# wuji3/visiondk

Hardware: NVIDIA H100
Metric: embeddings/sec (ConvNeXt-B 224^2 faceX ArcFace train step) (higher is better)
Workload: dtype bf16

## Files before the change

visiondk_b200/csrc/convnext.cu:

```cuda
#include "vdk_host.h"
#include "vdk_ptx.cuh"

#include <cstdlib>
#include "convnext_internal.h"

namespace vdk {

__device__ __forceinline__ float warp_sum(float v) {
#pragma unroll
  for (int off = 16; off > 0; off >>= 1) v += __shfl_xor_sync(0xffffffffu, v, off);
  return v;
}

__global__ void __launch_bounds__(256) stem_patchify_kernel(const float* __restrict__ x, int B, int H, int W,
                                                            __nv_bfloat16* __restrict__ out) {
  const int PH = H / 4, PW = W / 4;
  const int64_t total = static_cast<int64_t>(B) * PH * PW * 12;
  for (int64_t t = static_cast<int64_t>(blockIdx.x) * blockDim.x + threadIdx.x; t < total;
       t += static_cast<int64_t>(gridDim.x) * blockDim.x) {
    const int ck = static_cast<int>(t % 12);
    const int64_t patch = t / 12;
    const int c = ck >> 2, kh = ck & 3;
    const int pw = static_cast<int>(patch % PW);
    const int ph = static_cast<int>((patch / PW) % PH);
// ... 246 lines not shown
  const bool active = has_c && warp < TH && oy0 + warp < H;
  float2 acc[kDwTW][2];
#pragma unroll
  for (int p = 0; p < kDwTW; ++p) {
    acc[p][0] = make_float2(bc.x, bc.y);
    acc[p][1] = make_float2(bc.z, bc.w);
  }
  mbar_wait(bar, 0);
  if (active) {
    const uint8_t* tbase = smem + cl * 2;
#pragma unroll 1
    for (int dy = 0; dy < 7; ++dy) {
      float2 wlo[7], whi[7];
      const float* wrow = wsm + dy * (7 * chunk) + cl;
#pragma unroll
      for (int dx = 0; dx < 7; ++dx) {
        const float4 t = *reinterpret_cast<const float4*>(wrow + dx * chunk);
        wlo[dx] = make_float2(t.x, t.y);
        whi[dx] = make_float2(t.z, t.w);
      }
      const uint8_t* rowp = tbase + (warp + dy) * (box_w * pix_stride);
#pragma unroll
      for (int ix = 0; ix < box_w; ++ix) {
        const uint2 t = *reinterpret_cast<const uint2*>(rowp + ix * pix_stride);
        const float2 a = make_float2(__uint_as_float(t.x << 16), __uint_as_float(t.x & 0xffff0000u));
        const float2 c = make_float2(__uint_as_float(t.y << 16), __uint_as_float(t.y & 0xffff0000u));
#pragma unroll
        for (int p = 0; p < kDwTW; ++p) {
          const int dx = ix - p;
          if (dx >= 0 && dx < 7) {
            acc[p][0] = ffma2(a, wlo[dx], acc[p][0]);
            acc[p][1] = ffma2(c, whi[dx], acc[p][1]);
          }
        }
      }
    }
  }
  if (MODE == 1) {
    if (active) {
#pragma unroll
      for (int p = 0; p < kDwTW; ++p) {
        const int ox = ox0 + p;
        if (ox >= W) continue;
        const int64_t off = ((static_cast<int64_t>(b) * H + oy0 + warp) * W + ox) * C + c0;
        float o0 = acc[p][0].x, o1 = acc[p][0].y, o2 = acc[p][1].x, o3 = acc[p][1].y;
        if (addend) {
          const uint2 t = __ldg(reinterpret_cast<const uint2*>(addend + off));
          const float2 a = __bfloat1622float2(*reinterpret_cast<const __nv_bfloat162*>(&t.x));
          const float2 c = __bfloat1622float2(*reinterpret_cast<const __nv_bfloat162*>(&t.y));
          o0 += a.x; o1 += a.y; o2 += c.x; o3 += c.y;
        }
        __nv_bfloat162 lo = __floats2bfloat162_rn(o0, o1), hi = __floats2bfloat162_rn(o2, o3);
        uint2 t;
        t.x = *reinterpret_cast<uint32_t*>(&lo);
        t.y = *reinterpret_cast<uint32_t*>(&hi);
        *reinterpret_cast<uint2*>(y + off) = t;
      }
    }
    return;
  }
  float mean[kDwTW], rstd[kDwTW];
  const float inv_chunk = 1.0f / static_cast<float>(chunk), inv_c = 1.0f / static_cast<float>(C);
#pragma unroll
  for (int p = 0; p < kDwTW; ++p) {
    const float s = warp_sum(active ? (acc[p][0].x + acc[p][0].y) + (acc[p][1].x + acc[p][1].y) : 0.f);
    mean[p] = s * inv_chunk;
  }
#pragma unroll
  for (int p = 0; p < kDwTW; ++p) {
    float q = 0.f;
    if (active) {
      const float d0 = acc[p][0].x - mean[p], d1 = acc[p][0].y - mean[p];
      const float d2 = acc[p][1].x - mean[p], d3 = acc[p][1].y - mean[p];
      q = fmaf(d0, d0, fmaf(d1, d1, fmaf(d2, d2, d3 * d3)));
    }
    rstd[p] = warp_sum(q);
  }
  if (nchunks == 1) {
#pragma unroll
    for (int p = 0; p < kDwTW; ++p) rstd[p] = rsqrtf(rstd[p] * inv_c + eps);
  } else {
    float2 mine = make_float2(0.f, 0.f);
#pragma unroll
    for (int p = 0; p < kDwTW; ++p)
      if (lane == p) mine = make_float2(mean[p], rstd[p]);
    if (lane < kDwTW && warp < 7) part[warp * 8 + lane] = mine;
    cluster_arrive();
    cluster_wait();
    const float inv_n = 1.0f / static_cast<float>(nchunks);
#pragma unroll
    for (int p = 0; p < kDwTW; ++p) {
      float2 r = make_float2(0.f, 0.f);
      if (lane < nchunks) r = ld_dsmem_f2(part + warp * 8 + p, static_cast<uint32_t>(lane));
      const float m = warp_sum(r.x) * inv_n;
      const float d = r.x - m;
      const float m2 = warp_sum(lane < nchunks ? fmaf(static_cast<float>(chunk) * d, d, r.y) : 0.f);
      mean[p] = m;
      rstd[p] = rsqrtf(m2 * inv_c + eps);
    }
    cluster_arrive();
  }
  if (active) {
#pragma unroll
    for (int p = 0; p < kDwTW; ++p) {
      const int ox = ox0 + p;
      if (ox >= W) continue;
      const int64_t pix = (static_cast<int64_t>(b) * H + oy0 + warp) * W + ox;
      if (rstd_out != nullptr && lane == 0 && ck == 0) rstd_out[pix] = rstd[p];
      __nv_bfloat16* dst = y + pix * C + c0;
      __nv_bfloat162 lo = __floats2bfloat162_rn((acc[p][0].x - mean[p]) * rstd[p] * g4.x + b4.x,
                                                (acc[p][0].y - mean[p]) * rstd[p] * g4.y + b4.y);
      __nv_bfloat162 hi = __floats2bfloat162_rn((acc[p][1].x - mean[p]) * rstd[p] * g4.z + b4.z,
                                                (acc[p][1].y - mean[p]) * rstd[p] * g4.w + b4.w);
      uint2 t;
      t.x = *reinterpret_cast<uint32_t*>(&lo);
      t.y = *reinterpret_cast<uint32_t*>(&hi);
      *reinterpret_cast<uint2*>(dst) = t;
    }
  }
  if (nchunks > 1) cluster_wait();
}

template <int MODE, int CHUNK, int TH>
__global__ void __launch_bounds__((TH + 1) * 32, TH == 7 ? 2 : 1)
dwconv7_pipe_kernel(const __grid_constant__ CUtensorMap map_x, int B, int H, int W, int C, int nchunks, int n_tiles,
                    const float* __restrict__ w49, const float* __restrict__ bias, const float* __restrict__ ln_w,
                    const float* __restrict__ ln_b, float eps, __nv_bfloat16* __restrict__ y, float* __restrict__ rstd_out,
                    const __nv_bfloat16* __restrict__ addend) {
  extern __shared__ uint8_t dwp_smem_raw[];
  uint8_t* smem = dwp_smem_raw + ((128u - (smem_u32(dwp_smem_raw) & 127u)) & 127u);
  constexpr int box_w = kDwTW + 6, box_h = TH + 6;
  constexpr int tile_bytes = box_h * box_w * CHUNK * 2;
  constexpr int tile_stride = (tile_bytes + 127) & ~127;
  float* wsm = reinterpret_cast<float*>(smem + 2 * tile_stride);
  float2* part = reinterpret_cast<float2*>(wsm + 49 * CHUNK);
  uint64_t* full_bar = reinterpret_cast<uint64_t*>(part + 2 * TH * 8);
  uint64_t* empty_bar = full_bar + 2;

  const int warp = threadIdx.x >> 5, lane = threadIdx.x & 31;
  const int ck = blockIdx.x % nchunks;
  const int group = blockIdx.x / nchunks, n_groups = gridDim.x / nchunks;
  const int tiles_w = (W + kDwTW - 1) / kDwTW, tiles_h = (H + TH - 1) / TH;
  const int n_my = group < n_tiles ? (n_tiles - group + n_groups - 1) / n_groups : 0;
  const bool clustered = MODE == 0 && nchunks > 1;

  if (threadIdx.x == 0) {
    prefetch_tensormap(&map_x);
    for (int i = 0; i < 2; ++i) {
      mbar_init(&full_bar[i], 1);
      mbar_init(&empty_bar[i], TH);
    }
    fence_mbar_init();
  }
  for (int i = threadIdx.x; i < 49 * (CHUNK / 4); i += blockDim.x) {
    const int t = i / (CHUNK / 4), q = i - t * (CHUNK / 4);
    *reinterpret_cast<float4*>(wsm + t * CHUNK + q * 4) = __ldg(reinterpret_cast<const float4*>(w49 + t * C + ck * CHUNK + q * 4));
  }
  __syncthreads();

  auto tile_coords = [&](int it, int& b, int& oy0, int& ox0) {
    int t = group + it * n_groups;
    const int tw = t % tiles_w;
    t /= tiles_w;
    const int th = t % tiles_h;
    b = t / tiles_h;
    oy0 = th * TH;
    ox0 = tw * kDwTW;
  };

  if (warp == TH) {
    if (lane == 0 && n_my > 0) {
      int b, oy0, ox0;
      tile_coords(0, b, oy0, ox0);
      mbar_arrive_expect_tx(&full_bar[0], tile_bytes);
      tma_load_4d(smem, &map_x, &full_bar[0], ck * CHUNK, ox0 - 3, oy0 - 3, b);
    }
    for (int it = 0; it < n_my; ++it) {
      if (lane == 0 && it + 1 < n_my) {
        const int j = it + 1, buf = j & 1;
        mbar_wait_relaxed(&empty_bar[buf], ((j >> 1) & 1) ^ 1);
        int b, oy0, ox0;
        tile_coords(j, b, oy0, ox0);
        mbar_arrive_expect_tx(&full_bar[buf], tile_bytes);
        tma_load_4d(smem + buf * tile_stride, &map_x, &full_bar[buf], ck * CHUNK, ox0 - 3, oy0 - 3, b);
      }
      if (clustered) {
        __syncwarp();
        cluster_arrive();
        cluster_wait();
      }
    }
    if (clustered) {
      __syncwarp();
      cluster_arrive();
      cluster_wait();
    }
    return;
  }

  const int cl = lane * 4;
  const bool has_c = cl < CHUNK;
  const int c0 = ck * CHUNK + cl;
  float4 bc = make_float4(0.f, 0.f, 0.f, 0.f), g4 = bc, b4 = bc;
  if (has_c && MODE == 0) {
    bc = __ldg(reinterpret_cast<const float4*>(bias + c0));
    g4 = __ldg(reinterpret_cast<const float4*>(ln_w + c0));
    b4 = __ldg(reinterpret_cast<const float4*>(ln_b + c0));
  }
  constexpr int pix_stride = CHUNK * 2;
  const float inv_chunk = 1.0f / static_cast<float>(CHUNK), inv_c = 1.0f / static_cast<float>(C);

  auto conv_row = [&](const uint8_t* tile, float2 (&acc)[kDwTW][2]) {
#pragma unroll
    for (int p = 0; p < kDwTW; ++p) {
      acc[p][0] = make_float2(bc.x, bc.y);
      acc[p][1] = make_float2(bc.z, bc.w);
    }
    const uint8_t* tbase = tile + cl * 2;
#pragma unroll 1
    for (int dy = 0; dy < 7; ++dy) {
      float2 wlo[7], whi[7];
      const float* wrow = wsm + dy * (7 * CHUNK) + cl;
#pragma unroll
      for (int dx = 0; dx < 7; ++dx) {
        const float4 t = *reinterpret_cast<const float4*>(wrow + dx * CHUNK);
        wlo[dx] = make_float2(t.x, t.y);
        whi[dx] = make_float2(t.z, t.w);
      }
      const uint8_t* rowp = tbase + (warp + dy) * (box_w * pix_stride);
#pragma unroll
      for (int ix = 0; ix < box_w; ++ix) {
        const uint2 t = *reinterpret_cast<const uint2*>(rowp + ix * pix_stride);
        const float2 a = make_float2(__uint_as_float(t.x << 16), __uint_as_float(t.x & 0xffff0000u));
        const float2 c = make_float2(__uint_as_float(t.y << 16), __uint_as_float(t.y & 0xffff0000u));
#pragma unroll
        for (int p = 0; p < kDwTW; ++p) {
          const int dx = ix - p;
          if (dx >= 0 && dx < 7) {
            acc[p][0] = ffma2(a, wlo[dx], acc[p][0]);
            acc[p][1] = ffma2(c, whi[dx], acc[p][1]);
          }
        }
      }
    }
  };

  if (MODE == 1) {
    for (int it = 0; it < n_my; ++it) {
      const int buf = it & 1;
      int b, oy0, ox0;
      tile_coords(it, b, oy0, ox0);
      const bool active = has_c && oy0 + warp < H;
      float2 acc[kDwTW][2];
      mbar_wait(&full_bar[buf], (it >> 1) & 1);
      if (active) conv_row(smem + buf * tile_stride, acc);
      __syncwarp();
      if (lane == 0) mbar_arrive(&empty_bar[buf]);
      if (active) {
#pragma unroll
        for (int p = 0; p < kDwTW; ++p) {
          const int ox = ox0 + p;
          if (ox >= W) continue;
          const int64_t off = ((static_cast<int64_t>(b) * H + oy0 + warp) * W + ox) * C + c0;
          float o0 = acc[p][0].x, o1 = acc[p][0].y, o2 = acc[p][1].x, o3 = acc[p][1].y;
          if (addend) {
            const uint2 t = __ldg(reinterpret_cast<const uint2*>(addend + off));
            const float2 a = __bfloat1622float2(*reinterpret_cast<const __nv_bfloat162*>(&t.x));
            const float2 c = __bfloat1622float2(*reinterpret_cast<const __nv_bfloat162*>(&t.y));
            o0 += a.x; o1 += a.y; o2 += c.x; o3 += c.y;
          }
          __nv_bfloat162 lo = __floats2bfloat162_rn(o0, o1), hi = __floats2bfloat162_rn(o2, o3);
          uint2 t;
          t.x = *reinterpret_cast<uint32_t*>(&lo);
          t.y = *reinterpret_cast<uint32_t*>(&hi);
          *reinterpret_cast<uint2*>(y + off) = t;
        }
      }
    }
    return;
  }

  float2 acc[kDwTW][2];
  float mean[kDwTW], m2[kDwTW];
  int pb = 0, poy0 = 0, pox0 = 0;
  bool pactive = false;

  auto local_stats = [&](bool active, int parity) {
#pragma unroll
    for (int p = 0; p < kDwTW; ++p)
      mean[p] = warp_sum(active ? (acc[p][0].x + acc[p][0].y) + (acc[p][1].x + acc[p][1].y) : 0.f) * inv_chunk;
#pragma unroll
    for (int p = 0; p < kDwTW; ++p) {
      float q = 0.f;
      if (active) {
        const float d0 = acc[p][0].x - mean[p], d1 = acc[p][0].y - mean[p];
        const float d2 = acc[p][1].x - mean[p], d3 = acc[p][1].y - mean[p];
        q = fmaf(d0, d0, fmaf(d1, d1, fmaf(d2, d2, d3 * d3)));
      }
      m2[p] = warp_sum(q);
    }
    if (clustered) {
      float2 mine = make_float2(0.f, 0.f);
#pragma unroll
      for (int p = 0; p < kDwTW; ++p)
        if (lane == p) mine = make_float2(mean[p], m2[p]);
      if (lane < kDwTW) part[(parity * TH + warp) * 8 + lane] = mine;
    }
  };

  auto finish = [&](int parity) {
    float rstd[kDwTW];
    if (clustered) {
      float2 r[kDwTW];
#pragma unroll
      for (int p = 0; p < kDwTW; ++p) {
        r[p] = make_float2(0.f, 0.f);
        if (lane < nchunks) r[p] = ld_dsmem_f2(part + (parity * TH + warp) * 8 + p, static_cast<uint32_t>(lane));
      }
      const float inv_n = 1.0f / static_cast<float>(nchunks);
#pragma unroll
      for (int p = 0; p < kDwTW; ++p) {
        const float m = warp_sum(r[p].x) * inv_n;
        const float d = r[p].x - m;
        const float q = warp_sum(lane < nchunks ? fmaf(static_cast<float>(CHUNK) * d, d, r[p].y) : 0.f);
        mean[p] = m;
        rstd[p] = rsqrtf(q * inv_c + eps);
      }
    } else {
#pragma unroll
      for (int p = 0; p < kDwTW; ++p) rstd[p] = rsqrtf(m2[p] * inv_c + eps);
    }
    if (pactive) {
#pragma unroll
      for (int p = 0; p < kDwTW; ++p) {
        const int ox = pox0 + p;
        if (ox >= W) continue;
        const int64_t pix = (static_cast<int64_t>(pb) * H + poy0 + warp) * W + ox;
        if (rstd_out != nullptr && lane == 0 && ck == 0) rstd_out[pix] = rstd[p];
        __nv_bfloat16* dst = y + pix * C + c0;
        __nv_bfloat162 lo = __floats2bfloat162_rn((acc[p][0].x - mean[p]) * rstd[p] * g4.x + b4.x,
                                                  (acc[p][0].y - mean[p]) * rstd[p] * g4.y + b4.y);
        __nv_bfloat162 hi = __floats2bfloat162_rn((acc[p][1].x - mean[p]) * rstd[p] * g4.z + b4.z,
                                                  (acc[p][1].y - mean[p]) * rstd[p] * g4.w + b4.w);
        uint2 t;
        t.x = *reinterpret_cast<uint32_t*>(&lo);
        t.y = *reinterpret_cast<uint32_t*>(&hi);
        *reinterpret_cast<uint2*>(dst) = t;
      }
    }
  };

  for (int it = 0; it < n_my; ++it) {
    const int buf = it & 1;
    int b, oy0, ox0;
    tile_coords(it, b, oy0, ox0);
    const bool active = has_c && oy0 + warp < H;
    float2 nxt[kDwTW][2];
    mbar_wait(&full_bar[buf], (it >> 1) & 1);
    if (active) conv_row(smem + buf * tile_stride, nxt);
    __syncwarp();
    if (lane == 0) mbar_arrive(&empty_bar[buf]);
    if (it > 0) {
      if (clustered) cluster_wait();
      finish((it - 1) & 1);
    }
#pragma unroll
    for (int p = 0; p < kDwTW; ++p) {
      acc[p][0] = nxt[p][0];
      acc[p][1] = nxt[p][1];
    }
    pb = b; poy0 = oy0; pox0 = ox0; pactive = active;
    local_stats(active, buf);
    if (clustered) cluster_arrive();
  }
  if (n_my > 0) {
    if (clustered) cluster_wait();
    finish((n_my - 1) & 1);
  }
  if (clustered) {
    cluster_arrive();
    cluster_wait();
  }
}

template <int LPP>
__global__ void __launch_bounds__(256)
ln_patchify_kernel(const __nv_bfloat16* __restrict__ x, int B, int H, int W, int C, const float* __restrict__ ln_w,
                   const float* __restrict__ ln_b, float eps, int patch , __nv_bfloat16* __restrict__ out,
                   float* __restrict__ rstd_out) {
  constexpr int kPPW = 32 / LPP;
  constexpr int kMaxIter = 8;
  const int lane = threadIdx.x & 31;
  const int sub = lane % LPP;
  const int64_t warp_id = (static_cast<int64_t>(blockIdx.x) * blockDim.x + threadIdx.x) >> 5;
  const int64_t pix = warp_id * kPPW + lane / LPP;
  const int64_t npix = static_cast<int64_t>(B) * H * W;
  const bool ok = pix < npix;
  const __nv_bfloat16* src = x + (ok ? pix : 0) * C;
  const int iters = (C + LPP * 8 - 1) / (LPP * 8);
  float v[kMaxIter][8];
  float s = 0.f;
#pragma unroll
  for (int i = 0; i < kMaxIter; ++i) {
    if (i < iters) {
      const int c = (sub + i * LPP) * 8;
      uint4 t = make_uint4(0, 0, 0, 0);
      if (ok && c < C) t = *reinterpret_cast<const uint4*>(src + c);
      const float2 a0 = __bfloat1622float2(*reinterpret_cast<const __nv_bfloat162*>(&t.x));
      const float2 a1 = __bfloat1622float2(*reinterpret_cast<const __nv_bfloat162*>(&t.y));
      const float2 a2 = __bfloat1622float2(*reinterpret_cast<const __nv_bfloat162*>(&t.z));
      const float2 a3 = __bfloat1622float2(*reinterpret_cast<const __nv_bfloat162*>(&t.w));
      v[i][0] = a0.x; v[i][1] = a0.y; v[i][2] = a1.x; v[i][3] = a1.y;
      v[i][4] = a2.x; v[i][5] = a2.y; v[i][6] = a3.x; v[i][7] = a3.y;
#pragma unroll
      for (int j = 0; j < 8; ++j) s += v[i][j];
    }
  }
#pragma unroll
  for (int off = LPP / 2; off > 0; off >>= 1) s += __shfl_xor_sync(0xffffffffu, s, off);
  const float mean = s / static_cast<float>(C);
  float q = 0.f;
#pragma unroll
  for (int i = 0; i < kMaxIter; ++i) {
    if (i < iters && (sub + i * LPP) * 8 < C) {
#pragma unroll
      for (int j = 0; j < 8; ++j) {
        const float d = v[i][j] - mean;
        q = fmaf(d, d, q);
      }
    }
  }
#pragma unroll
  for (int off = LPP / 2; off > 0; off >>= 1) q += __shfl_xor_sync(0xffffffffu, q, off);
  const float rstd = rsqrtf(q / static_cast<float>(C) + eps);
  if (!ok) return;
  if (rstd_out != nullptr && sub == 0) rstd_out[pix] = rstd;
  int64_t orow;
  int ocol0;
  if (patch == 2) {
    const int xw = static_cast<int>(pix % W);
    const int yh = static_cast<int>((pix / W) % H);
    const int b = static_cast<int>(pix / (static_cast<int64_t>(W) * H));
    orow = (static_cast<int64_t>(b) * (H / 2) + (yh >> 1)) * (W / 2) + (xw >> 1);
    ocol0 = ((yh & 1) * 2 + (xw & 1)) * C;
  } else {
    orow = pix;
    ocol0 = 0;
  }
  __nv_bfloat16* dst = out + orow * (static_cast<int64_t>(C) * patch * patch) + ocol0;
#pragma unroll
  for (int i = 0; i < kMaxIter; ++i) {
    const int c = (sub + i * LPP) * 8;
    if (i < iters && c < C) {
      const float4 g0 = __ldg(reinterpret_cast<const float4*>(ln_w + c)), g1 = __ldg(reinterpret_cast<const float4*>(ln_w + c + 4));
      const float4 b0 = __ldg(reinterpret_cast<const float4*>(ln_b + c)), b1 = __ldg(reinterpret_cast<const float4*>(ln_b + c + 4));
      __nv_bfloat162 o0 = __floats2bfloat162_rn((v[i][0] - mean) * rstd * g0.x + b0.x, (v[i][1] - mean) * rstd * g0.y + b0.y);
      __nv_bfloat162 o1 = __floats2bfloat162_rn((v[i][2] - mean) * rstd * g0.z + b0.z, (v[i][3] - mean) * rstd * g0.w + b0.w);
      __nv_bfloat162 o2 = __floats2bfloat162_rn((v[i][4] - mean) * rstd * g1.x + b1.x, (v[i][5] - mean) * rstd * g1.y + b1.y);
      __nv_bfloat162 o3 = __floats2bfloat162_rn((v[i][6] - mean) * rstd * g1.z + b1.z, (v[i][7] - mean) * rstd * g1.w + b1.w);
      uint4 t;
      t.x = *reinterpret_cast<uint32_t*>(&o0); t.y = *reinterpret_cast<uint32_t*>(&o1);
      t.z = *reinterpret_cast<uint32_t*>(&o2); t.w = *reinterpret_cast<uint32_t*>(&o3);
      *reinterpret_cast<uint4*>(dst + c) = t;
    }
  }
}

int launch_ln_patchify(const __nv_bfloat16* x, int B, int H, int W, int C, const float* ln_w, const float* ln_b, float eps,
                       int patch, __nv_bfloat16* out, float* rstd_out, cudaStream_t s) {
  VDK_REQUIRE(C % 8 == 0 && C <= 2048, "layernorm_patchify: C must be a multiple of 8, <= 2048 (got %d)", C);
  const int64_t npix = static_cast<int64_t>(B) * H * W;
  const int vecs = C / 8;
  if (vecs <= 8) {
    const int64_t warps = (npix + 3) / 4;
    ln_patchify_kernel<8><<<static_cast<unsigned>((warps * 32 + 255) / 256), 256, 0, s>>>(x, B, H, W, C, ln_w, ln_b, eps, patch, out, rstd_out);
  } else if (vecs <= 16) {
    const int64_t warps = (npix + 1) / 2;
    ln_patchify_kernel<16><<<static_cast<unsigned>((warps * 32 + 255) / 256), 256, 0, s>>>(x, B, H, W, C, ln_w, ln_b, eps, patch, out, rstd_out);
  } else {
    ln_patchify_kernel<32><<<static_cast<unsigned>((npix * 32 + 255) / 256), 256, 0, s>>>(x, B, H, W, C, ln_w, ln_b, eps, patch, out, rstd_out);
  }
  VDK_CUDA_OK(cudaGetLastError());
  return VDK_OK;
}

__global__ void __launch_bounds__(256)
neck_finalize_kernel(const float* __restrict__ acc, int n_slabs, size_t slab_stride, int B, int F,
                     const float* __restrict__ bias, int l2norm, float* __restrict__ out) {
  const int lane = threadIdx.x & 31;
  const int row = (blockIdx.x * blockDim.x + threadIdx.x) >> 5;
  if (row >= B) return;
  double ss = 0.0;
  for (int i = lane; i < F; i += 32) {
    float v = bias[i];
    for (int sl = 0; sl < n_slabs; ++sl) v += acc[sl * slab_stride + static_cast<size_t>(row) * F + i];
    out[static_cast<size_t>(row) * F + i] = v;
    ss = fma(static_cast<double>(v), static_cast<double>(v), ss);
  }
#pragma unroll
  for (int off = 16; off > 0; off >>= 1) ss += __shfl_xor_sync(0xffffffffu, ss, off);
  const float denom = l2norm ? fmaxf(static_cast<float>(sqrt(ss)), 1e-12f) : 1.0f;
  if (l2norm)
    for (int i = lane; i < F; i += 32) out[static_cast<size_t>(row) * F + i] = __fdiv_rn(out[static_cast<size_t>(row) * F + i], denom);
}

int launch_neck_finalize(const float* slabs, int n_slabs, size_t slab_stride, int B, int F, const float* bias, int l2norm,
                         float* out, cudaStream_t s) {
  neck_finalize_kernel<<<(B * 32 + 255) / 256, 256, 0, s>>>(slabs, n_slabs, slab_stride, B, F, bias, l2norm, out);
  VDK_CUDA_OK(cudaGetLastError());
  return VDK_OK;
}

int launch_neck(const __nv_bfloat16* feats, int batch, int Kn, int F, const void* neck_w, const float* neck_b, int l2_normalize,
                float* scratch, size_t scratch_bytes, float* embeddings, cudaStream_t s) {
  const int tiles = ((batch + 127) / 128) * ((F + 255) / 256);
  const size_t slab = static_cast<size_t>(batch) * F;
  int split = std::max(1, (2 * sm_count()) / std::max(1, tiles));
  split = static_cast<int>(std::min<size_t>(split, scratch_bytes / (slab * sizeof(float))));
  split = vdk_gemm_effective_splits(Kn, std::max(1, split));
  {
    vdk_gemm_desc g{};
    g.A = feats; g.B = neck_w; g.D = scratch;
    g.M = batch; g.N = F; g.K = Kn; g.lda = Kn; g.ldb = Kn; g.ldd = F;
    g.in_dtype = VDK_DTYPE_BF16; g.out_dtype = VDK_DTYPE_FP32; g.epilogue = VDK_EPI_NONE;
    g.split_k = split;
    g.split_stride = split > 1 ? static_cast<long long>(slab) : 0;
    const int rc = gemm_run(g, s);
    if (rc != VDK_OK) return rc;
  }
  neck_finalize_kernel<<<(batch * 32 + 255) / 256, 256, 0, s>>>(scratch, split, slab, batch, F, neck_b, l2_normalize, embeddings);
  VDK_CUDA_OK(cudaGetLastError());
  return VDK_OK;
}

static int check_net(const vdk_convnext_net* n) {
  VDK_REQUIRE(n, "vdk_convnext: null network");
  VDK_REQUIRE(n->image_size > 0 && n->image_size % 32 == 0, "vdk_convnext: image_size must be a multiple of 32");
  VDK_REQUIRE(n->feat_dim > 0 && n->feat_dim % 8 == 0, "vdk_convnext: feat_dim must be a multiple of 8");
  int nb = 0;
  for (int s = 0; s < 4; ++s) {
    VDK_REQUIRE(n->dims[s] > 0 && n->dims[s] % 8 == 0 && n->dims[s] <= 2048, "vdk_convnext: dims must be multiples of 8, <= 2048");
    VDK_REQUIRE(n->depths[s] >= 0, "vdk_convnext: bad depth");
    nb += n->depths[s];
  }
  VDK_REQUIRE(nb <= VDK_CONVNEXT_MAX_BLOCKS, "vdk_convnext: too many blocks (%d)", nb);
  VDK_REQUIRE(n->dims[0] <= 256, "vdk_convnext: stem width must be <= 256 (LayerNorm epilogue tile)");
  return VDK_OK;
}

}

using namespace vdk;

template <int TW, int MODE>
static int launch_dwconv_tw(const CUtensorMap& mx, int batch, int H, int W, int C, int TH, int box_c, const float* w49,
                            const float* bias, const float* ln_w, const float* ln_b, float eps, __nv_bfloat16* y,
                            float* rstd_out, const __nv_bfloat16* addend, cudaStream_t s) {
  const int tpg = ((C / 4) + 31) / 32 * 32;
  const int groups = std::max(1, std::min(512 / tpg, TH));
  const int n_chunks = C / box_c;
  const int smem = n_chunks * (((TH + 6) * (TW + 6) * box_c * 2 + 127) & ~127) + 16 * TW * 16 * 4 + 16 + 128;
  auto kern = dwconv7_ln_kernel<TW, MODE>;
  VDK_CUDA_OK(cudaFuncSetAttribute(kern, cudaFuncAttributeMaxDynamicSharedMemorySize, 227 * 1024));
  const unsigned grid = static_cast<unsigned>(batch) * ((H + TH - 1) / TH) * ((W + TW - 1) / TW);
  kern<<<grid, groups * tpg, smem, s>>>(mx, batch, H, W, C, TH, box_c, tpg, w49, bias, ln_w, ln_b, eps, y, rstd_out, addend);
  VDK_CUDA_OK(cudaGetLastError());
  return VDK_OK;
}


template <int MODE, int CHUNK, int TH>
static int launch_dwconv7_pipe_t(const __nv_bfloat16* x, int batch, int H, int W, int C, const float* w49, const float* bias,
                                 const float* ln_w, const float* ln_b, float eps, __nv_bfloat16* y, float* rstd_out,
                                 const __nv_bfloat16* addend, cudaStream_t s) {
  const int nchunks = C / CHUNK;
  constexpr int tile_stride = ((TH + 6) * (kDwTW + 6) * CHUNK * 2 + 127) & ~127;
  constexpr int smem = 2 * tile_stride + 49 * CHUNK * 4 + 2 * TH * 8 * 8 + 4 * 8 + 128;
  static_assert(smem <= 227 * 1024, "dwconv7_pipe shared memory budget");
  CUtensorMap mx;
  int rc = make_tma_nhwc_16bit(&mx, x, batch, H, W, C, TH + 6, kDwTW + 6, CHUNK);
  if (rc != VDK_OK) return rc;
  auto kern = dwconv7_pipe_kernel<MODE, CHUNK, TH>;
  const int cluster = (MODE == 0) ? nchunks : 1;
  struct Fit { int clusters; };
  static Fit fit[17] = {};
  cudaLaunchConfig_t cfg{};
  cfg.blockDim = dim3((TH + 1) * 32);
  cfg.dynamicSmemBytes = smem;
  cfg.stream = s;
  cudaLaunchAttribute attr[1];
  attr[0].id = cudaLaunchAttributeClusterDimension;
  attr[0].val.clusterDim.x = cluster;
  attr[0].val.clusterDim.y = 1;
  attr[0].val.clusterDim.z = 1;
  cfg.attrs = attr;
  cfg.numAttrs = 1;
  if (fit[cluster].clusters == 0) {
    VDK_CUDA_OK(cudaFuncSetAttribute(kern, cudaFuncAttributeMaxDynamicSharedMemorySize, smem));
    if (cluster > 8) VDK_CUDA_OK(cudaFuncSetAttribute(kern, cudaFuncAttributeNonPortableClusterSizeAllowed, 1));
    cfg.gridDim = dim3(cluster * sm_count());
    int n = 0;
    if (cudaOccupancyMaxActiveClusters(&n, kern, &cfg) != cudaSuccess || n <= 0) {
      cudaGetLastError();
      fit[cluster].clusters = -1;
    } else {
      fit[cluster].clusters = n;
    }
  }
  if (fit[cluster].clusters < 0) return VDK_ERR_WORKSPACE;
  const int n_tiles = batch * ((H + TH - 1) / TH) * ((W + kDwTW - 1) / kDwTW);
  const int groups = std::min(n_tiles, fit[cluster].clusters);
  cfg.gridDim = dim3(static_cast<unsigned>(groups) * nchunks);
  if (MODE == 1) {
    const int slots = fit[cluster].clusters;
    const int g = std::max(1, std::min(n_tiles, slots / nchunks));
    cfg.gridDim = dim3(static_cast<unsigned>(g) * nchunks);
  }
  VDK_CUDA_OK(cudaLaunchKernelEx(&cfg, kern, mx, batch, H, W, C, nchunks, n_tiles, w49, bias, ln_w, ln_b, eps, y, rstd_out, addend));
  return VDK_OK;
}

static int launch_dwconv7_pipe(int mode, const __nv_bfloat16* x, int batch, int H, int W, int C, int chunk, const float* w49,
                               const float* bias, const float* ln_w, const float* ln_b, float eps, __nv_bfloat16* y, float* rstd_out,
                               const __nv_bfloat16* addend, cudaStream_t s) {
  const bool tall = H > 7;
#define VDK_DWP(MODEV, CHV)                                                                                                           \
  return tall ? launch_dwconv7_pipe_t<MODEV, CHV, 14>(x, batch, H, W, C, w49, bias, ln_w, ln_b, eps, y, rstd_out, addend, s)          \
              : launch_dwconv7_pipe_t<MODEV, CHV, 7>(x, batch, H, W, C, w49, bias, ln_w, ln_b, eps, y, rstd_out, addend, s)
  if (mode == 0) {
    if (chunk == 128) { VDK_DWP(0, 128); }
    if (chunk == 96) { VDK_DWP(0, 96); }
    VDK_DWP(0, 64);
  }
  if (chunk == 128) { VDK_DWP(1, 128); }
  if (chunk == 96) { VDK_DWP(1, 96); }
  VDK_DWP(1, 64);
#undef VDK_DWP
}

int vdk::launch_dwconv7(int mode, const __nv_bfloat16* x, int batch, int H, int W, int C, const float* w49, const float* bias,
                          const float* ln_w, const float* ln_b, float eps, __nv_bfloat16* y, float* rstd_out,
                          const __nv_bfloat16* addend, cudaStream_t s) {
  VDK_REQUIRE(C % 8 == 0 && C <= 2048, "dwconv7: C must be a multiple of 8, <= 2048 (got %d)", C);
  const double dw_elems = static_cast<double>(batch) * H * W * C;
  ProfScope prof(kProfDepthwise, 2.0 * 49.0 * dw_elems, 2.0 * dw_elems * (addend ? 3.0 : 2.0), s);
  {
    int chunk = 0;
    if (C % 128 == 0) chunk = 128;
    else if (C % 96 == 0) chunk = 96;
    else if (C % 64 == 0) chunk = 64;
    static const bool use_pipe = [] {
      const char* e = getenv("VDK_DWCONV_PIPE");
      return e ? atoi(e) != 0 : true;
    }();
    if (use_pipe && chunk > 0 && C / chunk <= 16) {
      const int rc = launch_dwconv7_pipe(mode, x, batch, H, W, C, chunk, w49, bias, ln_w, ln_b, eps, y, rstd_out, addend, s);
      if (rc != VDK_ERR_WORKSPACE) return rc;
    }
    if (chunk > 0 && C / chunk <= 16) {
      const int nchunks = C / chunk;
      const int TH = std::min(7, H);
      CUtensorMap mx;
      int rc = make_tma_nhwc_16bit(&mx, x, batch, H, W, C, TH + 6, kDwTW + 6, chunk);
      if (rc != VDK_OK) return rc;
      const int smem = (((TH + 6) * (kDwTW + 6) * chunk * 2 + 127) & ~127) + 49 * chunk * 4 + 7 * 8 * 8 + 16 + 128;
      const unsigned grid = static_cast<unsigned>(batch) * ((H + TH - 1) / TH) * ((W + kDwTW - 1) / kDwTW) * nchunks;
      cudaLaunchConfig_t cfg{};
      cfg.gridDim = dim3(grid);
      cfg.blockDim = dim3(32 * TH);
      cfg.dynamicSmemBytes = smem;
      cfg.stream = s;
      cudaLaunchAttribute attr[1];
      attr[0].id = cudaLaunchAttributeClusterDimension;
      attr[0].val.clusterDim.x = (mode == 0) ? nchunks : 1;
      attr[0].val.clusterDim.y = 1;
      attr[0].val.clusterDim.z = 1;
      cfg.attrs = attr;
      cfg.numAttrs = 1;
#define VDK_DWC(MODEV, CHV)                                                                                              \
  do {                                                                                                                   \
    auto kern = dwconv7_chunk_kernel<MODEV, CHV>;                                                                        \
    VDK_CUDA_OK(cudaFuncSetAttribute(kern, cudaFuncAttributeMaxDynamicSharedMemorySize, 80 * 1024));                     \
    if (MODEV == 0 && nchunks > 8) VDK_CUDA_OK(cudaFuncSetAttribute(kern, cudaFuncAttributeNonPortableClusterSizeAllowed, 1)); \
    VDK_CUDA_OK(cudaLaunchKernelEx(&cfg, kern, mx, batch, H, W, C, TH, nchunks, w49, bias, ln_w, ln_b, eps, y, rstd_out, addend)); \
  } while (0)
      if (mode == 0) {
        if (chunk == 128) VDK_DWC(0, 128);
        else if (chunk == 96) VDK_DWC(0, 96);
        else VDK_DWC(0, 64);
      } else {
        if (chunk == 128) VDK_DWC(1, 128);
        else if (chunk == 96) VDK_DWC(1, 96);
        else VDK_DWC(1, 64);
      }
#undef VDK_DWC
      return VDK_OK;
    }
  }
  int box_c = std::min(C, 256);
  while (C % box_c != 0 || box_c % 8 != 0) --box_c;
  int T = 7;
  while (T > 2 && (T + 6) * (T + 6) * C * 2 > 200 * 1024) T = (T == 7) ? 4 : 2;
  VDK_REQUIRE((T + 6) * (T + 6) * C * 2 <= 200 * 1024, "dwconv7: C too large for the shared-memory halo (%d)", C);
  const int TH = std::min(T, H);
  CUtensorMap mx;
  int rc = make_tma_nhwc_16bit(&mx, x, batch, H, W, C, TH + 6, T + 6, box_c);
  if (rc != VDK_OK) return rc;
#define VDK_DW(TWV)                                                                                                    \
  return mode == 0 ? launch_dwconv_tw<TWV, 0>(mx, batch, H, W, C, TH, box_c, w49, bias, ln_w, ln_b, eps, y, rstd_out, addend, s) \
                   : launch_dwconv_tw<TWV, 1>(mx, batch, H, W, C, TH, box_c, w49, bias, ln_w, ln_b, eps, y, rstd_out, addend, s)
  if (T == 7) { VDK_DW(7); }
  if (T == 4) { VDK_DW(4); }
  VDK_DW(2);
#undef VDK_DW
}

static int launch_dwconv7_ln(const __nv_bfloat16* x, int batch, int H, int W, int C, const float* w49, const float* bias,
                             const float* ln_w, const float* ln_b, float eps, __nv_bfloat16* y, cudaStream_t s) {
  return launch_dwconv7(0, x, batch, H, W, C, w49, bias, ln_w, ln_b, eps, y, nullptr, nullptr, s);
}

extern "C" int vdk_dwconv7_ln(const void* x, int batch, int H, int W, int C, const float* w49, const float* bias,
                              const float* ln_w, const float* ln_b, float eps, void* y, void* stream) {
  VDK_REQUIRE(x && y && w49 && bias && ln_w && ln_b, "vdk_dwconv7_ln: null operand");
  VDK_REQUIRE(batch > 0 && H > 0 && W > 0 && C > 0 && C % 8 == 0, "vdk_dwconv7_ln: bad shape (C must be a multiple of 8)");
  return launch_dwconv7_ln(reinterpret_cast<const __nv_bfloat16*>(x), batch, H, W, C, w49, bias, ln_w, ln_b, eps,
                           reinterpret_cast<__nv_bfloat16*>(y), reinterpret_cast<cudaStream_t>(stream));
}

extern "C" int vdk_layernorm_patchify(const void* x, int batch, int H, int W, int C, const float* ln_w,
                                      const float* ln_b, float eps, int patch, void* out, void* stream) {
  VDK_REQUIRE(x && out && ln_w && ln_b, "vdk_layernorm_patchify: null operand");
  VDK_REQUIRE(batch > 0 && H > 0 && W > 0 && C > 0 && C % 8 == 0 && C <= 2048, "vdk_layernorm_patchify: bad shape");
  VDK_REQUIRE(patch == 1 || (patch == 2 && H % 2 == 0 && W % 2 == 0), "vdk_layernorm_patchify: patch must be 1 or 2");
  return launch_ln_patchify(reinterpret_cast<const __nv_bfloat16*>(x), batch, H, W, C, ln_w, ln_b, eps, patch,
                            reinterpret_cast<__nv_bfloat16*>(out), nullptr, reinterpret_cast<cudaStream_t>(stream));
}

extern "C" size_t vdk_convnext_workspace_bytes(const vdk_convnext_net* net, int batch) {
  if (!net || batch <= 0) return 0;
  const size_t hw0 = static_cast<size_t>(net->image_size / 4) * (net->image_size / 4);
  size_t max_mc = 0, max_m4c = 0;
  size_t hw = hw0;
  for (int s = 0; s < 4; ++s) {
    if (s > 0) hw /= 4;
    const size_t m = static_cast<size_t>(batch) * hw;
    max_mc = std::max(max_mc, m * net->dims[s]);
    max_m4c = std::max(max_m4c, m * net->dims[s] * 4);
  }
  const size_t patches = static_cast<size_t>(batch) * hw0 * 48;
  return up256(max_mc * 2) * 2 + up256(std::max(max_m4c, patches) * 2) + up256(static_cast<size_t>(batch) * net->feat_dim * 4) + 1024;
}

extern "C" int vdk_convnext_forward(const vdk_convnext_net* net, const float* images, int batch, int l2_normalize,
                                    float* embeddings, void* workspace, size_t workspace_bytes, void* stream) {
  int rc = check_net(net);
  if (rc != VDK_OK) return rc;
  VDK_REQUIRE(images && embeddings && batch > 0, "vdk_convnext_forward: null image/embedding buffer");
  VDK_REQUIRE(workspace && workspace_bytes >= vdk_convnext_workspace_bytes(net, batch),
              "vdk_convnext_forward: workspace too small");
  VDK_REQUIRE((reinterpret_cast<uintptr_t>(workspace) & 255) == 0 && (reinterpret_cast<uintptr_t>(images) & 15) == 0,
              "vdk_convnext_forward: workspace must be 256-byte and images 16-byte aligned");
  cudaStream_t s = reinterpret_cast<cudaStream_t>(stream);
  const int S = net->image_size;
  const size_t hw0 = static_cast<size_t>(S / 4) * (S / 4);
  size_t max_mc = 0, max_m4c = 0, hwt = hw0;
  for (int st = 0; st < 4; ++st) {
    if (st > 0) hwt /= 4;
    max_mc = std::max(max_mc, static_cast<size_t>(batch) * hwt * net->dims[st]);
    max_m4c = std::max(max_m4c, static_cast<size_t>(batch) * hwt * net->dims[st] * 4);
// ... 60 lines not shown
```

visiondk_b200/csrc/convnext_train.cu:

```cuda
#include "vdk_host.h"
#include "vdk_ptx.cuh"
#include "convnext_internal.h"
#include "train_gemm.h"

#include <vector>

namespace vdk {

static size_t al(size_t v) { return (v + 255) & ~static_cast<size_t>(255); }

static bool ln_bwd_fuses(int C) { return C == 128 || C == 256 || C == 512 || C == 1024; }

struct StageDims {
  int H, W, C;
  size_t M;
};

struct TrainLayout {
  StageDims st[4];
  int depth[4];
  int n_blocks;
  size_t p0, z0, rstd0;
  size_t xs[4][VDK_CONVNEXT_MAX_BLOCKS + 1];
  size_t y[VDK_CONVNEXT_MAX_BLOCKS], rstd[VDK_CONVNEXT_MAX_BLOCKS];
  size_t hpre[VDK_CONVNEXT_MAX_BLOCKS], hpost[VDK_CONVNEXT_MAX_BLOCKS];
  size_t patch[4], prstd[4];
  size_t f, frstd, fn, bn2_mean, bn2_rstd, z, zslab, bn1_mean, bn1_rstd;
  size_t dxa, dxb, dy, dconv, G, sdo, dw49, gwc, gwneck, dz, dzb, dfn, wslab;
  size_t total;
};

static void make_layout(const vdk_convnext_net* net, int batch, TrainLayout* L) {
  size_t off = 0;
  auto take = [&](size_t bytes) { size_t o = off; off += al(bytes); return o; };
  int H = net->image_size / 4, W = H;
  L->n_blocks = 0;
  for (int s = 0; s < 4; ++s) {
    if (s > 0) { H /= 2; W /= 2; }
    L->st[s] = {H, W, net->dims[s], static_cast<size_t>(batch) * H * W};
    L->depth[s] = net->depths[s];
    L->n_blocks += net->depths[s];
  }
  const size_t M0 = L->st[0].M;
  L->p0 = take(M0 * 48 * 2);
  L->z0 = take(M0 * net->dims[0] * 2);
  L->rstd0 = take(M0 * 4);
  int k = 0;
  size_t max_mc = 0, max_cc4 = 0;
  for (int s = 0; s < 4; ++s) {
    const size_t M = L->st[s].M, C = L->st[s].C;
    max_mc = std::max(max_mc, M * C);
    max_cc4 = std::max(max_cc4, C * 4 * C);
    if (s > 0) {
      L->patch[s] = take(M * 4 * L->st[s - 1].C * 2);
      L->prstd[s] = take(L->st[s - 1].M * 4);
      max_cc4 = std::max(max_cc4, C * 4 * static_cast<size_t>(L->st[s - 1].C));
    }
    for (int j = 0; j <= L->depth[s]; ++j) L->xs[s][j] = take(M * C * 2);
    for (int j = 0; j < L->depth[s]; ++j, ++k) {
      L->y[k] = take(M * C * 2);
      L->rstd[k] = take(M * 4);
      L->hpre[k] = take(M * 4 * C * 2);
      L->hpost[k] = take(M * 4 * C * 2);
    }
  }
  const size_t M3 = L->st[3].M, C3 = L->st[3].C, F = net->feat_dim, Kn = (M3 / batch) * C3;
  L->f = take(M3 * C3 * 2);
  L->frstd = take(M3 * 4);
  L->fn = take(M3 * C3 * 2);
  L->bn2_mean = take(C3 * 4);
  L->bn2_rstd = take(C3 * 4);
  L->z = take(static_cast<size_t>(batch) * F * 4);
  L->zslab = take(static_cast<size_t>(batch) * F * 4 * 160);
  L->bn1_mean = take(F * 4);
  L->bn1_rstd = take(F * 4);
  L->dxa = take(max_mc * 2);
  L->dxb = take(max_mc * 2);
  L->dy = take(std::max(max_mc * 2, static_cast<size_t>(2) * 4096 * sm_count() * 4));
  L->dconv = take(max_mc * 2);
  L->G = take(max_cc4 * 4);
  L->sdo = take(static_cast<size_t>(L->n_blocks) * 2048 * 4);
  L->dw49 = take(static_cast<size_t>(L->n_blocks) * 49 * 2048 * 4);
  L->gwc = take(max_cc4 * 4);
  L->gwneck = take(F * Kn * 4);
  L->dz = take(static_cast<size_t>(batch) * F * 4);
  L->dzb = take(static_cast<size_t>(batch) * F * 2);
  L->dfn = take(M3 * C3 * 2);
  size_t slab = wgrad_slab_bytes(net->dims[0], 48, M0);
  for (int s = 0; s < 4; ++s) {
    const int C = L->st[s].C;
    slab = std::max(slab, wgrad_slab_bytes(C, 4 * C, L->st[s].M));
    slab = std::max(slab, wgrad_slab_bytes(4 * C, C, L->st[s].M));
    if (s > 0) slab = std::max(slab, wgrad_slab_bytes(C, 4 * L->st[s - 1].C, L->st[s].M));
  }
  L->wslab = take(slab);
  L->total = off + 256;
}

__global__ void slab_reduce_bias_kernel(const float* __restrict__ slabs, int n_slabs, size_t stride, const float* __restrict__ bias,
                                        int rows, int cols, float* __restrict__ out) {
  const int i = blockIdx.x * blockDim.x + threadIdx.x;
  if (i >= rows * cols) return;
  float v = bias ? bias[i % cols] : 0.f;
  for (int s = 0; s < n_slabs; ++s) v += slabs[s * stride + i];
  out[i] = v;
}
int launch_slab_reduce_bias(const float* slabs, int n_slabs, size_t stride, const float* bias, int rows, int cols, float* out,
                            cudaStream_t s) {
  slab_reduce_bias_kernel<<<(rows * cols + 255) / 256, 256, 0, s>>>(slabs, n_slabs, stride, bias, rows, cols, out);
  VDK_CUDA_OK(cudaGetLastError());
  return VDK_OK;
}
__global__ void __launch_bounds__(256)
slab_reduce_kernel(const float* __restrict__ slabs, int n_slabs, size_t stride, int64_t n4, float* __restrict__ dst,
                   int accumulate) {
  __shared__ float4 part[8][32];
  const int col = threadIdx.x & 31, grp = threadIdx.x >> 5;
  const int64_t i = static_cast<int64_t>(blockIdx.x) * 32 + col;
  float4 acc = make_float4(0.f, 0.f, 0.f, 0.f);
  if (i < n4) {
#pragma unroll 4
    for (int s = grp; s < n_slabs; s += 8) {
      const float4 v = __ldg(reinterpret_cast<const float4*>(slabs + static_cast<size_t>(s) * stride) + i);
      acc.x += v.x; acc.y += v.y; acc.z += v.z; acc.w += v.w;
    }
  }
  part[grp][col] = acc;
  __syncthreads();
  if (grp == 0 && i < n4) {
    float4 t = part[0][col];
#pragma unroll
    for (int g = 1; g < 8; ++g) {
      const float4 v = part[g][col];
      t.x += v.x; t.y += v.y; t.z += v.z; t.w += v.w;
    }
    float4* o = reinterpret_cast<float4*>(dst) + i;
    if (accumulate) {
      const float4 d = *o;
      t.x += d.x; t.y += d.y; t.z += d.z; t.w += d.w;
    }
    *o = t;
  }
}
int launch_slab_reduce(const float* slabs, int n_slabs, size_t stride, int64_t n4, float* dst, int accumulate, cudaStream_t s) {
  slab_reduce_kernel<<<static_cast<unsigned>((n4 + 31) / 32), 256, 0, s>>>(slabs, n_slabs, stride, n4, dst, accumulate);
  VDK_CUDA_OK(cudaGetLastError());
  return VDK_OK;
}
__global__ void col_sum_f32_small_kernel(const float* __restrict__ x, int rows, int cols, float* __restrict__ out) {
  const int c = blockIdx.x * blockDim.x + threadIdx.x;
  if (c >= cols) return;
  float s = 0.f;
  for (int r = 0; r < rows; ++r) s += x[static_cast<size_t>(r) * cols + c];
  out[c] += s;
}
int launch_col_sum_f32_small(const float* x, int rows, int cols, float* out, cudaStream_t s) {
  col_sum_f32_small_kernel<<<(cols + 255) / 256, 256, 0, s>>>(x, rows, cols, out);
  VDK_CUDA_OK(cudaGetLastError());
  return VDK_OK;
}
__global__ void stem_patchify_train_kernel(const float* __restrict__ x, int B, int H, int W, __nv_bfloat16* __restrict__ out) {
  const int PH = H / 4, PW = W / 4;
  const int64_t total = static_cast<int64_t>(B) * PH * PW * 12;
  for (int64_t t = static_cast<int64_t>(blockIdx.x) * blockDim.x + threadIdx.x; t < total;
       t += static_cast<int64_t>(gridDim.x) * blockDim.x) {
    const int ck = static_cast<int>(t % 12);
    const int64_t patch = t / 12;
    const int c = ck >> 2, kh = ck & 3;
    const int pw = static_cast<int>(patch % PW);
    const int ph = static_cast<int>((patch / PW) % PH);
    const int b = static_cast<int>(patch / (static_cast<int64_t>(PW) * PH));
    const float4 v = *reinterpret_cast<const float4*>(x + ((static_cast<int64_t>(b) * 3 + c) * H + (ph * 4 + kh)) * W + pw * 4);
    __nv_bfloat162 lo = __floats2bfloat162_rn(v.x, v.y), hi = __floats2bfloat162_rn(v.z, v.w);
    uint2 o;
    o.x = *reinterpret_cast<uint32_t*>(&lo);
    o.y = *reinterpret_cast<uint32_t*>(&hi);
    *reinterpret_cast<uint2*>(out + patch * 48 + ck * 4) = o;
  }
}

}

using namespace vdk;

extern "C" size_t vdk_convnext_train_workspace_bytes(const vdk_convnext_net* net, int batch) {
  if (!net || batch <= 0) return 0;
  TrainLayout L;
  make_layout(net, batch, &L);
  return L.total;
}

constexpr int kPackTab = 32;
struct PackTab {
  const float* src[kPackTab];
  void* dst[kPackTab];
  void* dst2[kPackTab];
  const float* scale[kPackTab];
};

__global__ void __launch_bounds__(256)
pack_cast_kernel(PackTab t, int64_t n, int cols) {
  const float* __restrict__ src = t.src[blockIdx.y];
  __nv_bfloat16* __restrict__ dst = reinterpret_cast<__nv_bfloat16*>(t.dst[blockIdx.y]);
  __nv_bfloat16* __restrict__ dst2 = reinterpret_cast<__nv_bfloat16*>(t.dst2[blockIdx.y]);
  const float* __restrict__ sc = t.scale[blockIdx.y];
  for (int64_t i = (static_cast<int64_t>(blockIdx.x) * blockDim.x + threadIdx.x) * 4; i < n;
       i += static_cast<int64_t>(gridDim.x) * blockDim.x * 4) {
    const float4 v = __ldg(reinterpret_cast<const float4*>(src + i));
    if (dst2 != nullptr) {
      __nv_bfloat162 lo = __floats2bfloat162_rn(v.x, v.y), hi = __floats2bfloat162_rn(v.z, v.w);
      uint2 o;
      o.x = *reinterpret_cast<uint32_t*>(&lo);
      o.y = *reinterpret_cast<uint32_t*>(&hi);
      *reinterpret_cast<uint2*>(dst2 + i) = o;
    }
    const float m = sc ? sc[i / cols] : 1.f;
    __nv_bfloat162 lo = __floats2bfloat162_rn(v.x * m, v.y * m), hi = __floats2bfloat162_rn(v.z * m, v.w * m);
    uint2 o;
    o.x = *reinterpret_cast<uint32_t*>(&lo);
    o.y = *reinterpret_cast<uint32_t*>(&hi);
    *reinterpret_cast<uint2*>(dst + i) = o;
  }
}
__global__ void __launch_bounds__(256)
pack_taps_kernel(PackTab t, int C) {
  const float* __restrict__ src = t.src[blockIdx.y];
  float* __restrict__ dst = reinterpret_cast<float*>(t.dst[blockIdx.y]);
  float* __restrict__ dst2 = reinterpret_cast<float*>(t.dst2[blockIdx.y]);
  const int i = blockIdx.x * blockDim.x + threadIdx.x;
  if (i >= 49 * C) return;
  const int tap = i / C, c = i - tap * C;
  const float v = src[c * 49 + tap];
  if (dst != nullptr) dst[i] = v;
  if (dst2 != nullptr) dst2[(48 - tap) * C + c] = v;
}

__global__ void __launch_bounds__(256)
unpack_taps_grad_kernel(PackTab t, int C) {
  const float* __restrict__ src = t.src[blockIdx.y];
  float* __restrict__ dst = reinterpret_cast<float*>(t.dst[blockIdx.y]);
  const int i = blockIdx.x * blockDim.x + threadIdx.x;
  if (i >= 49 * C) return;
  const int tap = i / C, c = i - tap * C;
  dst[c * 49 + tap] += src[i];
}

static int pack_impl(const vdk_convnext_tensors* p, const vdk_convnext_net* net, bool taps_and_weights, bool flip, cudaStream_t s) {
  auto bf = [](const void* q) { return const_cast<void*>(q); };
  int k0 = 0;
  for (int st = 0; st < 4; ++st) {
    const int C = net->dims[st], depth = net->depths[st];
    for (int j0 = 0; j0 < depth; j0 += kPackTab) {
      const int nb = std::min(kPackTab, depth - j0);
      PackTab fc1{}, fc2{}, taps{};
      bool any_flip = false;
      for (int j = 0; j < nb; ++j) {
        const vdk_convnext_block_tensors* b = &p->blocks[k0 + j0 + j];
        const vdk_convnext_block* o = &net->blocks[k0 + j0 + j];
        fc1.src[j] = b->fc1_w; fc1.dst[j] = bf(o->fc1_w);
        fc2.src[j] = b->fc2_w;
        if (o->fc2_wg) { fc2.dst[j] = bf(o->fc2_wg); fc2.dst2[j] = bf(o->fc2_w); fc2.scale[j] = b->gamma; }
        else { fc2.dst[j] = bf(o->fc2_w); }
        taps.src[j] = b->dw_w;
        taps.dst[j] = taps_and_weights ? bf(o->dw_w) : nullptr;
        taps.dst2[j] = (flip && o->dw_w_flip) ? bf(o->dw_w_flip) : nullptr;
        any_flip = any_flip || taps.dst2[j] != nullptr;
      }
      const int64_t n = static_cast<int64_t>(4) * C * C;
      const unsigned gx = static_cast<unsigned>(std::max<int64_t>(1, std::min<int64_t>((n / 4 + 255) / 256, 256)));
      if (taps_and_weights) {
        pack_cast_kernel<<<dim3(gx, nb), 256, 0, s>>>(fc1, n, 4 * C);
        pack_cast_kernel<<<dim3(gx, nb), 256, 0, s>>>(fc2, n, 4 * C);
      }
      if (taps_and_weights || any_flip) pack_taps_kernel<<<dim3((49 * C + 255) / 256, nb), 256, 0, s>>>(taps, C);
    }
    k0 += depth;
  }
  VDK_CUDA_OK(cudaGetLastError());
  return VDK_OK;
}

extern "C" int vdk_convnext_pack(const vdk_convnext_tensors* p, vdk_convnext_net* net, void* stream) {
  VDK_REQUIRE(p && net, "vdk_convnext_pack: null argument");
  cudaStream_t s = reinterpret_cast<cudaStream_t>(stream);
  const int C0 = net->dims[0];
  auto bf = [](const void* q) { return reinterpret_cast<__nv_bfloat16*>(const_cast<void*>(q)); };
  for (int st = 0; st < 4; ++st)
    VDK_REQUIRE(net->dims[st] % 4 == 0, "vdk_convnext_pack: channel counts must be multiples of 4");
  RC(launch_cast_bf16(p->stem_w, static_cast<int64_t>(C0) * 48, bf(net->stem_w), s));
  for (int st = 1; st < 4; ++st) {
    RC(launch_permute021(p->down[st].conv_w, net->dims[st], net->dims[st - 1], 4, nullptr, bf(net->down[st].conv_w), nullptr, 0, s));
  }
  RC(pack_impl(p, net, true, true, s));
  const int C3 = net->dims[3], hw = (net->image_size / 32) * (net->image_size / 32);
  RC(launch_permute021(p->lin_w, net->feat_dim, C3, hw, nullptr, bf(net->neck_w), nullptr, 0, s));
  return VDK_OK;
}

extern "C" int vdk_convnext_train_forward(const vdk_convnext_net* net, const vdk_convnext_tensors* p, const float* images,
                                          int batch, float bn_momentum, float* out_feats, void* workspace,
                                          size_t workspace_bytes, void* stream) {
  VDK_REQUIRE(net && p && images && out_feats && batch > 1, "vdk_convnext_train_forward: bad arguments (batch must be > 1)");
  TrainLayout L;
  make_layout(net, batch, &L);
  VDK_REQUIRE(workspace && workspace_bytes >= L.total && (reinterpret_cast<uintptr_t>(workspace) & 255) == 0,
              "vdk_convnext_train_forward: workspace too small or misaligned");
  cudaStream_t s = reinterpret_cast<cudaStream_t>(stream);
  uint8_t* ws = reinterpret_cast<uint8_t*>(workspace);
  auto B16 = [&](size_t off) { return reinterpret_cast<__nv_bfloat16*>(ws + off); };
  auto F32 = [&](size_t off) { return reinterpret_cast<float*>(ws + off); };
  const Gemm G{s};
  const int S = net->image_size;

  {
    const int M0 = static_cast<int>(L.st[0].M), C0 = L.st[0].C;
    const int64_t total = static_cast<int64_t>(M0) * 12;
    stem_patchify_train_kernel<<<static_cast<int>(std::min<int64_t>((total + 255) / 256, 132 * 16)), 256, 0, s>>>(images, batch, S, S,
                                                                                                             B16(L.p0));
    VDK_CUDA_OK(cudaGetLastError());
    RC(G.run(B16(L.p0), net->stem_w, B16(L.z0), M0, C0, 48, 48, 48, C0, VDK_EPI_NONE, net->stem_b, nullptr, nullptr, 0,
             VDK_DTYPE_BF16, 1, 0, 0, 0));
    RC(launch_ln_patchify(B16(L.z0), batch, L.st[0].H, L.st[0].W, C0, net->stem_ln_w, net->stem_ln_b, 1e-6f, 1, B16(L.xs[0][0]),
                          F32(L.rstd0), s));
  }
  int k = 0;
  for (int st = 0; st < 4; ++st) {
    const int H = L.st[st].H, W = L.st[st].W, C = L.st[st].C, M = static_cast<int>(L.st[st].M);
    if (st > 0) {
      const vdk_convnext_down* d = &net->down[st];
      const int Cin = L.st[st - 1].C;
      RC(launch_ln_patchify(B16(L.xs[st - 1][L.depth[st - 1]]), batch, L.st[st - 1].H, L.st[st - 1].W, Cin, d->ln_w, d->ln_b, 1e-6f,
                            2, B16(L.patch[st]), F32(L.prstd[st]), s));
      RC(G.run(B16(L.patch[st]), d->conv_w, B16(L.xs[st][0]), M, C, 4 * Cin, 4 * Cin, 4 * Cin, C, VDK_EPI_NONE, d->conv_b, nullptr,
               nullptr, 0, VDK_DTYPE_BF16, 1, 0, 0, 0));
    }
    for (int j = 0; j < L.depth[st]; ++j, ++k) {
      const vdk_convnext_block* b = &net->blocks[k];
      RC(launch_dwconv7(0, B16(L.xs[st][j]), batch, H, W, C, b->dw_w, b->dw_b, b->ln_w, b->ln_b, 1e-6f, B16(L.y[k]), F32(L.rstd[k]),
                        nullptr, s));
      RC(G.run(B16(L.y[k]), b->fc1_w, B16(L.hpost[k]), M, 4 * C, C, C, C, 4 * C, VDK_EPI_GELU, b->fc1_b, nullptr, nullptr, 0,
               VDK_DTYPE_BF16, 1, 0, 0, 0, B16(L.hpre[k])));
      RC(G.run(B16(L.hpost[k]), b->fc2_w, B16(L.xs[st][j + 1]), M, C, 4 * C, 4 * C, 4 * C, C, VDK_EPI_SCALE_RESIDUAL, b->fc2_b,
               b->gamma, B16(L.xs[st][j]), C, VDK_DTYPE_BF16, 1, 0, 0, 0));
    }
  }
  {
    const int H = L.st[3].H, W = L.st[3].W, C3 = L.st[3].C, M3 = static_cast<int>(L.st[3].M), F = net->feat_dim;
    const int Kn = H * W * C3;
    RC(launch_ln_patchify(B16(L.xs[3][L.depth[3]]), batch, H, W, C3, net->head_ln_w, net->head_ln_b, 1e-6f, 1, B16(L.f),
                          F32(L.frstd), s));
    RC(launch_bn_fwd_bf16(B16(L.f), M3, C3, p->bn2_w, p->bn2_b, 1e-5f, bn_momentum, B16(L.fn), F32(L.bn2_mean), F32(L.bn2_rstd),
                          p->bn2_running_mean, p->bn2_running_var, s));
    const int tiles = ((batch + 127) / 128) * ((F + 255) / 256);
    int split = std::max(1, std::min(160, (2 * sm_count()) / std::max(1, tiles)));
    split = vdk_gemm_effective_splits(Kn, split);
    const size_t slab = static_cast<size_t>(batch) * F;
    RC(G.run(B16(L.fn), net->neck_w, F32(L.zslab), batch, F, Kn, Kn, Kn, F, VDK_EPI_NONE, nullptr, nullptr, nullptr, 0,
             VDK_DTYPE_FP32, split, split > 1 ? static_cast<long long>(slab) : 0, 0, 0));
    RC(launch_slab_reduce_bias(F32(L.zslab), split, slab, p->lin_b, batch, F, F32(L.z), s));
    RC(launch_bn_fwd_f32(F32(L.z), batch, F, p->bn1_w, p->bn1_b, 1e-5f, bn_momentum, out_feats, F32(L.bn1_mean), F32(L.bn1_rstd),
                         p->bn1_running_mean, p->bn1_running_var, s));
  }
  return VDK_OK;
}

extern "C" int vdk_convnext_train_backward_units(const vdk_convnext_net* net) {
  if (!net) return 0;
  int n = 1 + 4;
  for (int st = 0; st < 4; ++st) n += net->depths[st];
  return n;
}

static int backward_range(const vdk_convnext_net* net, const vdk_convnext_tensors* p, const vdk_convnext_tensors* g,
                          const float* d_feats, int batch, void* workspace, size_t workspace_bytes, void* stream, int u_begin,
                          int u_end) {
  VDK_REQUIRE(net && p && g && d_feats && batch > 1, "vdk_convnext_train_backward: bad arguments");
  VDK_REQUIRE(u_begin >= 0 && u_begin < u_end && u_end <= vdk_convnext_train_backward_units(net),
              "vdk_convnext_train_backward: bad unit range [%d, %d)", u_begin, u_end);
  int u = 0;
  auto active = [&](int unit) { return unit >= u_begin && unit < u_end; };
  TrainLayout L;
  make_layout(net, batch, &L);
  VDK_REQUIRE(workspace && workspace_bytes >= L.total, "vdk_convnext_train_backward: workspace too small");
  cudaStream_t s = reinterpret_cast<cudaStream_t>(stream);
  uint8_t* ws = reinterpret_cast<uint8_t*>(workspace);
  auto B16 = [&](size_t off) { return reinterpret_cast<__nv_bfloat16*>(ws + off); };
  auto F32 = [&](size_t off) { return reinterpret_cast<float*>(ws + off); };
  const Gemm G{s};
  const int F = net->feat_dim;

  const int H3 = L.st[3].H, W3 = L.st[3].W, C3 = L.st[3].C, M3 = static_cast<int>(L.st[3].M), Kn = H3 * W3 * C3;
  if (active(u++)) {
    VDK_CUDA_OK(cudaMemsetAsync(F32(L.sdo), 0, static_cast<size_t>(L.n_blocks) * 2048 * 4, s));
    VDK_CUDA_OK(cudaMemsetAsync(F32(L.dw49), 0, static_cast<size_t>(L.n_blocks) * 49 * 2048 * 4, s));
    RC(launch_bn_bwd_f32(d_feats, F32(L.z), batch, F, p->bn1_w, F32(L.bn1_mean), F32(L.bn1_rstd), F32(L.dz), g->bn1_w, g->bn1_b, s));
    RC(launch_col_sum_f32_small(F32(L.dz), batch, F, g->lin_b, s));
    RC(launch_cast_bf16(F32(L.dz), static_cast<int64_t>(batch) * F, B16(L.dzb), s));
    RC(G.run(B16(L.dzb), B16(L.fn), F32(L.gwneck), F, Kn, batch, F, Kn, Kn, VDK_EPI_NONE, nullptr, nullptr, nullptr, 0,
             VDK_DTYPE_FP32, 1, 0, 1, 1));
    RC(launch_permute021(F32(L.gwneck), F, H3 * W3, C3, nullptr, nullptr, g->lin_w, 1, s));
    RC(G.run(B16(L.dzb), net->neck_w, B16(L.dfn), batch, Kn, F, F, Kn, Kn, VDK_EPI_NONE, nullptr, nullptr, nullptr, 0,
             VDK_DTYPE_BF16, 1, 0, 0, 1));
    RC(launch_bn_bwd_bf16(B16(L.dfn), B16(L.f), M3, C3, p->bn2_w, F32(L.bn2_mean), F32(L.bn2_rstd), B16(L.dy), g->bn2_w, g->bn2_b, s));
    RC(launch_ln_bwd(B16(L.dy), B16(L.f), F32(L.frstd), batch, H3, W3, C3, net->head_ln_w, net->head_ln_b, 1, B16(L.dxa), nullptr,
                     g->head_ln_w, g->head_ln_b, s));
  }
  size_t dx = L.dxa, dx_other = L.dxb;
  int k = L.n_blocks;
  for (int st = 3; st >= 0; --st) {
    const int H = L.st[st].H, W = L.st[st].W, C = L.st[st].C, M = static_cast<int>(L.st[st].M);
    int k_done_lo = -1, k_done_hi = -1;
    for (int j = L.depth[st] - 1; j >= 0; --j) {
      --k;
      if (!active(u++)) {
        std::swap(dx, dx_other);
        continue;
      }
      if (k_done_hi < 0) k_done_hi = k;
      k_done_lo = k;
      const vdk_convnext_block* b = &net->blocks[k];
      const vdk_convnext_block_tensors* pb = &p->blocks[k];
      const vdk_convnext_block_tensors* gb = &g->blocks[k];
      float* sdo = F32(L.sdo) + static_cast<size_t>(k) * 2048;
      RC(G.wgrad(B16(dx), B16(L.hpost[k]), F32(L.G), C, 4 * C, M, C, 4 * C, F32(L.wslab), false, sdo));
      RC(launch_layerscale_finalize(F32(L.G), pb->fc2_w, pb->fc2_b, pb->gamma, sdo, C, 4 * C, gb->fc2_w, gb->gamma, gb->fc2_b, s));
      RC(G.run(B16(dx), b->fc2_wg, B16(L.hpost[k]), M, 4 * C, C, C, 4 * C, 4 * C, VDK_EPI_MUL_GELU_GRAD, nullptr, nullptr,
               B16(L.hpre[k]), 4 * C, VDK_DTYPE_BF16, 1, 0, 0, 1));
      __nv_bfloat16* dh = B16(L.hpost[k]);
      RC(G.wgrad(dh, B16(L.y[k]), gb->fc1_w, 4 * C, C, M, 4 * C, C, F32(L.wslab), true, gb->fc1_b));
      if (ln_bwd_fuses(C)) {
        RC(G.ln_bwd(dh, b->fc1_w, B16(L.dconv), M, C, 4 * C, B16(L.y[k]), F32(L.rstd[k]), b->ln_w, b->ln_b, C, 0, gb->ln_w, gb->ln_b,
                    F32(L.dy)));
      } else {
        RC(G.run(dh, b->fc1_w, B16(L.dy), M, C, 4 * C, 4 * C, C, C, VDK_EPI_NONE, nullptr, nullptr, nullptr, 0, VDK_DTYPE_BF16, 1, 0, 0, 1));
        RC(launch_ln_bwd(B16(L.dy), B16(L.y[k]), F32(L.rstd[k]), batch, H, W, C, b->ln_w, b->ln_b, 1, B16(L.dconv), nullptr, gb->ln_w,
                         gb->ln_b, s));
      }
      RC(launch_dwconv7_wgrad(B16(L.xs[st][j]), B16(L.dconv), batch, H, W, C, F32(L.dw49) + static_cast<size_t>(k) * 49 * 2048, gb->dw_b, s));
      RC(launch_dwconv7(1, B16(L.dconv), batch, H, W, C, b->dw_w_flip, nullptr, nullptr, nullptr, 0.f, B16(dx_other), nullptr,
                        B16(dx), s));
      std::swap(dx, dx_other);
    }
    for (int k0 = k_done_lo; k_done_lo >= 0 && k0 <= k_done_hi; k0 += kPackTab) {
      const int nb = std::min(kPackTab, k_done_hi - k0 + 1);
      PackTab tab{};
      for (int j = 0; j < nb; ++j) {
        tab.src[j] = F32(L.dw49) + static_cast<size_t>(k0 + j) * 49 * 2048;
        tab.dst[j] = g->blocks[k0 + j].dw_w;
      }
      unpack_taps_grad_kernel<<<dim3((49 * C + 255) / 256, nb), 256, 0, s>>>(tab, C);
    }
    VDK_CUDA_OK(cudaGetLastError());
    if (st > 0 && !active(u++)) {
      std::swap(dx, dx_other);
    } else if (st > 0) {
      const vdk_convnext_down* d = &net->down[st];
      const vdk_convnext_down_tensors* gd = &g->down[st];
      const int Cin = L.st[st - 1].C;
      RC(G.wgrad(B16(dx), B16(L.patch[st]), F32(L.gwc), C, 4 * Cin, M, C, 4 * Cin, F32(L.wslab), false, gd->conv_b));
      RC(launch_permute021(F32(L.gwc), C, 4, Cin, nullptr, nullptr, gd->conv_w, 1, s));
      if (ln_bwd_fuses(Cin)) {
        RC(G.ln_bwd(B16(dx), d->conv_w, B16(dx_other), M, 4 * Cin, C, B16(L.patch[st]), F32(L.prstd[st]), d->ln_w, d->ln_b, Cin,
                    L.st[st].W, gd->ln_w, gd->ln_b, F32(L.dy)));
      } else {
        RC(G.run(B16(dx), d->conv_w, B16(L.dy), M, 4 * Cin, C, C, 4 * Cin, 4 * Cin, VDK_EPI_NONE, nullptr, nullptr, nullptr, 0,
                 VDK_DTYPE_BF16, 1, 0, 0, 1));
        RC(launch_ln_bwd(B16(L.dy), B16(L.patch[st]), F32(L.prstd[st]), batch, L.st[st - 1].H, L.st[st - 1].W, Cin, d->ln_w, d->ln_b,
                         2, B16(dx_other), nullptr, gd->ln_w, gd->ln_b, s));
      }
      std::swap(dx, dx_other);
    }
  }
  if (active(u++)) {
    const int M0 = static_cast<int>(L.st[0].M), C0 = L.st[0].C;
    RC(launch_ln_bwd(B16(dx), B16(L.xs[0][0]), F32(L.rstd0), batch, L.st[0].H, L.st[0].W, C0, net->stem_ln_w, net->stem_ln_b, 1,
                     B16(L.dy), nullptr, g->stem_ln_w, g->stem_ln_b, s));
    RC(G.wgrad(B16(L.dy), B16(L.p0), g->stem_w, C0, 48, M0, C0, 48, F32(L.wslab), true, g->stem_b));
  }
  return VDK_OK;
}

extern "C" int vdk_convnext_train_backward(const vdk_convnext_net* net, const vdk_convnext_tensors* p,
                                           const vdk_convnext_tensors* g, const float* d_feats, int batch, void* workspace,
                                           size_t workspace_bytes, void* stream) {
  VDK_REQUIRE(net, "vdk_convnext_train_backward: null net");
  return backward_range(net, p, g, d_feats, batch, workspace, workspace_bytes, stream, 0, vdk_convnext_train_backward_units(net));
}

extern "C" int vdk_convnext_train_backward_range(const vdk_convnext_net* net, const vdk_convnext_tensors* p,
                                                 const vdk_convnext_tensors* g, const float* d_feats, int batch, void* workspace,
                                                 size_t workspace_bytes, void* stream, int unit_begin, int unit_end) {
  VDK_REQUIRE(net, "vdk_convnext_train_backward_range: null net");
  return backward_range(net, p, g, d_feats, batch, workspace, workspace_bytes, stream, unit_begin, unit_end);
}
```

visiondk_b200/csrc/gemm.cu:

```cuda
#include "vdk_host.h"
#include "vdk_ptx.cuh"

#include <algorithm>
#include <cstdlib>

#include "train_gemm.h"

namespace vdk {

constexpr int kBM = 128;
constexpr int kBK = 64;
constexpr int kGemmThreads = 384;
constexpr int kBoxBytes = 64 * 128;
constexpr int kGemmPlain = 0;
constexpr int kConvDense = 1;
constexpr int kConvIm2col = 2;
constexpr int kConvGrouped = 3;
constexpr int kConvExDense = 4;
constexpr int kConvExIm2col = 5;
constexpr int kConvGroupedEx = 6;
constexpr int kGemmLnBwd = 7;

struct GemmParams {
  int M, N, K;
// ... 255 lines not shown
        t2[h] = fmaf(g1, h1, t2[h]);
        v[2 * jj] = h == 0 ? d.x * h0 : fmaf(d.x, h0, v[2 * jj]);
        v[2 * jj + 1] = h == 0 ? d.y * h1 : fmaf(d.y, h1, v[2 * jj + 1]);
      }
    }
    const int gi = sc * 64 / G;
#pragma unroll
    for (int gg = 0; gg < kGroups; ++gg)
      if (gg == gi)
#pragma unroll
        for (int h = 0; h < 2; ++h) {
          s1[gg][h] += t1[h];
          s2[gg][h] += t2[h];
        }
    halve_columns(v, lane);
    colp[sc][0] += v[0];
    colp[sc][1] += v[1];
#pragma unroll
    for (int jj = 0; jj < 8; ++jj)
#pragma unroll
      for (int e = 0; e < 2; ++e) v[2 * jj + e] = acc[4 * (sc * 8 + jj) + e] + acc[4 * (sc * 8 + jj) + 2 + e];
    halve_columns(v, lane);
    colp[sc][2] += v[0];
    colp[sc][3] += v[1];
  }
  const float inv_g = 1.0f / static_cast<float>(G);
#pragma unroll
  for (int gi = 0; gi < kGroups; ++gi) {
    if (gi * G >= BN) break;
#pragma unroll
    for (int h = 0; h < 2; ++h) {
      s1[gi][h] += __shfl_xor_sync(0xffffffffu, s1[gi][h], 1);
      s1[gi][h] += __shfl_xor_sync(0xffffffffu, s1[gi][h], 2);
      s2[gi][h] += __shfl_xor_sync(0xffffffffu, s2[gi][h], 1);
      s2[gi][h] += __shfl_xor_sync(0xffffffffu, s2[gi][h], 2);
    }
  }
  if (p.ln_cluster > 1) {
    const uint32_t rank = cluster_ctarank();
    if (leader) mbar_arrive_expect_tx(xbar, p.ln_cluster * 64 * 8);
    if ((lane & 3) == 0)
      for (int r = 0; r < p.ln_cluster; ++r)
#pragma unroll
        for (int h = 0; h < 2; ++h)
          st_async_f2(smem_u32(xch + (rank * 64 + frow + 8 * h) * 8), smem_u32(xbar), r, s1[0][h], s2[0][h]);
    mbar_wait<true>(xbar, xphase);
#pragma unroll
    for (int h = 0; h < 2; ++h) {
      float a = 0.f, b = 0.f;
      for (int r = 0; r < p.ln_cluster; ++r) {
        const float2 t = *reinterpret_cast<const float2*>(xch + (r * 64 + frow + 8 * h) * 8);
        a += t.x;
        b += t.y;
      }
      s1[0][h] = a;
      s2[0][h] = b;
    }
  }
#pragma unroll
  for (int gi = 0; gi < kGroups; ++gi)
#pragma unroll
    for (int h = 0; h < 2; ++h) {
      s1[gi][h] *= inv_g;
      s2[gi][h] *= inv_g;
    }
  __nv_bfloat16* dst = reinterpret_cast<__nv_bfloat16*>(p.D);
#pragma unroll
  for (int sc = 0; sc < BN / 64; ++sc) {
    uint8_t* boxp = ring + sc * kBoxBytes;
    const uint32_t box = smem_u32(boxp);
    const int gi = sc * 64 / G;
    float m1[2], m2[2], r[2];
#pragma unroll
    for (int h = 0; h < 2; ++h) {
      m1[h] = s1[0][h]; m2[h] = s2[0][h]; r[h] = rs[0][h];
#pragma unroll
      for (int gg = 1; gg < kGroups; ++gg)
        if (gg == gi) { m1[h] = s1[gg][h]; m2[h] = s2[gg][h]; r[h] = rs[gg][h]; }
    }
#pragma unroll
    for (int q = 0; q < 4; ++q) {
      const uint32_t addr = box + box_off(mrow, 2 * q + mcb);
      uint32_t rin[4], rq[4];
      ldmatrix_x4(rin, addr);
#pragma unroll
      for (int i = 0; i < 4; ++i) {
        const int j = sc * 8 + 2 * q + (i >> 1), h = i & 1, c = j * 8 + fcol;
        const float2 yv = unpack2(rin[i], VDK_DTYPE_BF16);
        const float2 w = *reinterpret_cast<const float2*>(par + c);
        const float2 iw = *reinterpret_cast<const float2*>(par + BN + c);
        const float2 b = *reinterpret_cast<const float2*>(par + 2 * BN + c);
        const float h0 = (yv.x - b.x) * iw.x, h1 = (yv.y - b.y) * iw.y;
        const float o0 = r[h] * (acc[4 * j + 2 * h] * w.x - m1[h] - h0 * m2[h]);
        const float o1 = r[h] * (acc[4 * j + 2 * h + 1] * w.y - m1[h] - h1 * m2[h]);
        rq[i] = pack2(o0, o1, VDK_DTYPE_BF16);
      }
      stmatrix_x4(addr, rq);
    }
    __syncwarp();
#pragma unroll
    for (int it = 0; it < 4; ++it) {
      const int row = wl * 16 + it * 4 + (lane >> 3), chunk = lane & 7, m = wrow0 + row;
      if (m < p.M) {
        const int n = n0 + sc * 64 + chunk * 8, qg = n / G;
        const long long off = p.ln_wo == 0 ? static_cast<long long>(m) * p.ldd + n : ln_pixel(p, m, qg) * G + (n - qg * G);
        *reinterpret_cast<uint4*>(dst + off) = *reinterpret_cast<const uint4*>(boxp + box_off(row, chunk));
      }
    }
  }
}

template <int BN, bool kBf16, int kTA, int kTB, int kMode>
__global__ void __launch_bounds__(kGemmThreads, 1)
gemm_tn_kernel(const __grid_constant__ CUtensorMap map_a, const __grid_constant__ CUtensorMap map_b,
               const __grid_constant__ CUtensorMap map_d, const __grid_constant__ CUtensorMap map_aux,
               const __grid_constant__ CUtensorMap map_r, const GemmParams p) {
  using Cfg = GemmCfg<BN>;
  constexpr int kStages = Cfg::kStages;
  constexpr int kRing = Cfg::kRing;
  extern __shared__ uint8_t smem_raw[];
  uint8_t* smem = smem_raw + ((1024u - (smem_u32(smem_raw) & 1023u)) & 1023u);
  uint8_t* ring_all = smem + kStages * Cfg::kStageBytes;
  float* par_all = reinterpret_cast<float*>(ring_all + Cfg::kRingBytes);
  uint64_t* full_bar = reinterpret_cast<uint64_t*>(par_all + 2 * Cfg::kParFloats);
  uint64_t* empty_bar = full_bar + kStages;
  uint64_t* res_bar = empty_bar + kStages;
  constexpr bool kColSums = kTA && kMode == kGemmPlain;
  const bool col_sums = kColSums && p.partial_out && p.split_stride > 0 && p.col_sums != nullptr;
  constexpr bool kConvEx = kMode == kConvExDense || kMode == kConvExIm2col;


  if (threadIdx.x == 0) {
    prefetch_tensormap(&map_a);
    prefetch_tensormap(&map_b);
    prefetch_tensormap(&map_d);
    if (p.aux != nullptr) prefetch_tensormap(&map_aux);
    if (kMode == kGemmLnBwd || p.epilogue == VDK_EPI_SCALE_RESIDUAL || p.epilogue == VDK_EPI_MUL_GELU_GRAD ||
        (kMode != kGemmPlain && p.epilogue == VDK_EPI_RESIDUAL_RELU) || (kConvEx && p.epilogue == VDK_EPI_SILU_RESIDUAL))
      prefetch_tensormap(&map_r);
    for (int i = 0; i < kStages; ++i) {
      mbar_init(&full_bar[i], 1);
      mbar_init(&empty_bar[i], col_sums ? 10 : 8);
    }
    mbar_init(&res_bar[0], 1);
    mbar_init(&res_bar[1], 1);
    if constexpr (kMode == kGemmLnBwd)
      for (int i = 0; i < 4; ++i) mbar_init(reinterpret_cast<uint64_t*>(reinterpret_cast<uint8_t*>(res_bar + 2) + kLnXchBytes) + i, 1);
    fence_mbar_init();
  }
  __syncthreads();
  if constexpr (kMode == kGemmLnBwd) {
    if (p.ln_cluster > 1) cluster_sync_all();
  }

  if (threadIdx.x < 128) {
    asm volatile("setmaxnreg.dec.sync.aligned.u32 40;");
    const int num_m = (p.M + kBM - 1) / kBM;
    const int num_n = (p.N + BN - 1) / BN;
    const int num_kb_total = (p.K + kBK - 1) / kBK;
    const int kb_per_split = (num_kb_total + p.split_k - 1) / p.split_k;
    const int num_tiles = num_m * num_n * p.split_k;
    if (threadIdx.x == 0) {
      int stage = 0;
      uint32_t phase = 0;
      for (int tile = blockIdx.x; tile < num_tiles; tile += gridDim.x) {
        const int mn = tile % (num_m * num_n), split = tile / (num_m * num_n);
        const int m0 = (mn / num_n) * kBM;
        const int n0 = (mn % num_n) * BN;
        const int kb0 = split * kb_per_split;
        const int kb1 = min(kb0 + kb_per_split, num_kb_total);
        int cw = 0, ch = 0, cn = 0;
        if constexpr (kMode == kConvIm2col || kMode == kConvGrouped || kMode == kConvGroupedEx) {
          cn = m0 / p.cv_howo;
          const int r = m0 - cn * p.cv_howo, ho = r / p.cv_wo;
          ch = ho * p.cv_stride - p.cv_pad;
          cw = (r - ho * p.cv_wo) * p.cv_stride - p.cv_pad;
        } else if constexpr (kMode == kConvExIm2col) {
          cn = m0 / p.cv_howo;
          const int r = m0 - cn * p.cv_howo, ho = r / p.cv_wo;
          ch = ho * p.cv_stride - (p.cv_pad & 0xff);
          cw = (r - ho * p.cv_wo) * p.cv_stride - (p.cv_pad >> 8);
        }
        for (int kb = kb0; kb < kb1; ++kb) {
          mbar_wait_relaxed<true>(&empty_bar[stage], phase ^ 1);
          uint8_t* sa = smem + stage * Cfg::kStageBytes;
          uint8_t* sb = sa + Cfg::kStageA;
          mbar_arrive_expect_tx(&full_bar[stage], Cfg::kStageBytes);
          if constexpr (kMode == kConvIm2col || kMode == kConvExIm2col) {
            const int tap = kb / p.cv_cpb, c0 = (kb - tap * p.cv_cpb) * kBK, dy = tap / p.cv_kw;
            tma_load_im2col_4d(sa, &map_a, &full_bar[stage], c0, cw, ch, cn, static_cast<uint16_t>(tap - dy * p.cv_kw),
                               static_cast<uint16_t>(dy), kEvictNormal);
          } else if constexpr (kMode == kConvGrouped) {
            const int tap = kb >> 1, c0 = n0 + (kb & 1) * kBK, dy = tap / p.cv_kw;
            tma_load_im2col_4d(sa, &map_a, &full_bar[stage], c0, cw, ch, cn, static_cast<uint16_t>(tap - dy * p.cv_kw),
                               static_cast<uint16_t>(dy), kEvictNormal);
          } else if constexpr (kMode == kConvGroupedEx) {
            const int tap = kb / p.cv_cpb, dy = tap / p.cv_kw;
            const int c0 = ((n0 / p.cv_cg_out * p.cv_cg_in) & ~7) + (kb - tap * p.cv_cpb) * kBK;
            tma_load_im2col_4d(sa, &map_a, &full_bar[stage], c0, cw, ch, cn, static_cast<uint16_t>(tap - dy * p.cv_kw),
                               static_cast<uint16_t>(dy), kEvictNormal);
          } else if (kTA) {
#pragma unroll
            for (int j = 0; j < kBM / 64; ++j) tma_load_2d(sa + j * 8192, &map_a, &full_bar[stage], m0 + j * 64, kb * kBK, kEvictNormal);
          } else {
            tma_load_2d(sa, &map_a, &full_bar[stage], kb * kBK, m0, kEvictNormal);
          }
          if (kTB) {
#pragma unroll
            for (int j = 0; j < BN / 64; ++j) tma_load_2d(sb + j * 8192, &map_b, &full_bar[stage], n0 + j * 64, kb * kBK, kEvictLast);
          } else {
            tma_load_2d(sb, &map_b, &full_bar[stage], kb * kBK, n0, kEvictLast);
          }
          if (++stage == kStages) {
            stage = 0;
            phase ^= 1;
          }
        }
      }
    } else if (col_sums && threadIdx.x >= 32 && threadIdx.x < 96) {
      const int j = (threadIdx.x >> 5) - 1, lane = threadIdx.x & 31;
      const int piece = lane & 15, r0 = lane >> 4;
      uint32_t off[4];
#pragma unroll
      for (int q = 0; q < 4; ++q)
        off[q] = j * 8192 + r0 * 128 + q * 256 + (((((piece >> 1) ^ r0) << 4)) ^ (q << 5)) + (piece & 1) * 8;
      int stage = 0;
      uint32_t phase = 0;
      for (int tile = blockIdx.x; tile < num_tiles; tile += gridDim.x) {
        const int mn = tile % (num_m * num_n), split = tile / (num_m * num_n);
        const int m0 = (mn / num_n) * kBM;
        const bool mine = (mn % num_n) == 0;
        const int kb0 = split * kb_per_split;
        const int kb1 = min(kb0 + kb_per_split, num_kb_total);
        float s[4] = {0.f, 0.f, 0.f, 0.f};
        for (int kb = kb0; kb < kb1; ++kb) {
          mbar_wait<true>(&full_bar[stage], phase);
          if (mine) {
            const uint8_t* sa = smem + stage * Cfg::kStageBytes;
#pragma unroll
            for (int i0 = 0; i0 < 32; i0 += 4) {
              uint2 v[4];
#pragma unroll
              for (int q = 0; q < 4; ++q) v[q] = *reinterpret_cast<const uint2*>(sa + off[q] + i0 * 256);
#pragma unroll
              for (int q = 0; q < 4; ++q) {
                const uint32_t w[2] = {v[q].x, v[q].y};
#pragma unroll
                for (int e = 0; e < 2; ++e) {
                  if constexpr (kBf16) {
                    s[2 * e] += __uint_as_float(w[e] << 16);
                    s[2 * e + 1] += __uint_as_float(w[e] & 0xffff0000u);
                  } else {
                    const float2 f = unpack2(w[e], VDK_DTYPE_FP16);
                    s[2 * e] += f.x;
                    s[2 * e + 1] += f.y;
                  }
                }
              }
            }
          }
          __syncwarp();
          if (lane == 0) mbar_arrive(&empty_bar[stage]);
          if (++stage == kStages) {
            stage = 0;
            phase ^= 1;
          }
        }
        if (mine) {
#pragma unroll
          for (int e = 0; e < 4; ++e) s[e] += __shfl_xor_sync(0xffffffffu, s[e], 16);
          const int m = m0 + j * 64 + piece * 4;
          if (lane < 16 && m < p.M)
            *reinterpret_cast<float4*>(p.col_sums + static_cast<size_t>(split) * p.M + m) = make_float4(s[0], s[1], s[2], s[3]);
        }
      }
    }
  } else {
    asm volatile("setmaxnreg.inc.sync.aligned.u32 232;");
    const int num_m = (p.M + kBM - 1) / kBM;
    const int num_n = (p.N + BN - 1) / BN;
    const int num_kb_total = (p.K + kBK - 1) / kBK;
    const int kb_per_split = (num_kb_total + p.split_k - 1) / p.split_k;
    const int num_tiles = num_m * num_n * p.split_k;
    const int ct = threadIdx.x - 128;
    const int cg = ct >> 7;
    const int wl = (ct >> 5) & 3, lane = ct & 31;
    const int fcol = (lane & 3) * 2;
    const int frow = wl * 16 + (lane >> 2);
    const int mrow = wl * 16 + ((lane >> 3) & 1) * 8 + (lane & 7);
    const int mcb = lane >> 4;
    const bool leader = (ct & 127) == 0;
    const uint32_t bar_id = 2 + cg;
    uint8_t* ring = ring_all + cg * kRing * kBoxBytes;
    float* par = par_all + cg * Cfg::kParFloats;
    const bool f32 = p.out_dtype == VDK_DTYPE_FP32;
    const int box_cols = f32 ? 32 : 64;
    const bool has_res = kMode == kGemmLnBwd || p.epilogue == VDK_EPI_SCALE_RESIDUAL || p.epilogue == VDK_EPI_MUL_GELU_GRAD ||
                         (kMode != kGemmPlain && p.epilogue == VDK_EPI_RESIDUAL_RELU) ||
                         (kConvEx && p.epilogue == VDK_EPI_SILU_RESIDUAL);
    const bool reduce = p.partial_out && p.split_stride == 0;
    int slot = 0;
    uint32_t res_phase = 0;
    int stage = 0;
    uint32_t phase = 0;
    float acc[BN / 2];
    float colp[BN / 64][4] = {};
// ... 103 lines not shown
          sum += __shfl_xor_sync(0xffffffffu, sum, 1);
          sum += __shfl_xor_sync(0xffffffffu, sum, 2);
          const float mean = sum / static_cast<float>(p.N);
          float sq = 0.f;
#pragma unroll
          for (int j = 0; j < BN / 8; ++j) {
            if (j * 8 >= p.N) break;
            const float d0 = acc[4 * j + 2 * r] - mean;
            sq = fmaf(d0, d0, sq);
            const float d1 = acc[4 * j + 2 * r + 1] - mean;
            sq = fmaf(d1, d1, sq);
          }
          sq += __shfl_xor_sync(0xffffffffu, sq, 1);
          sq += __shfl_xor_sync(0xffffffffu, sq, 2);
          ln_mean[r] = mean;
          ln_rstd[r] = rsqrtf(sq / static_cast<float>(p.N) + p.ln_eps);
        }
      }
      if (npre > 0) {
        mbar_wait<true>(&res_bar[cg], res_phase);
        res_phase ^= 1;
      }
      const int dz = (p.partial_out && p.split_stride > 0) ? split : 0;
      int box_i = 0;
#pragma unroll
      for (int sc = 0; sc < BN / 64; ++sc) {
        if (n0 + sc * 64 >= p.N) continue;
        if (f32) {
#pragma unroll
          for (int hb = 0; hb < 2; ++hb) {
            const int bcol = n0 + sc * 64 + hb * 32;
            if (bcol >= p.N) continue;
            uint8_t* box = ring + slot * kBoxBytes;
            if (has_res && box_i >= npre) {
              if (leader) {
                mbar_arrive_expect_tx(&res_bar[cg], kBoxBytes);
                tma_load_3d(box, &map_r, &res_bar[cg], bcol, wrow0, 0);
              }
              mbar_wait<true>(&res_bar[cg], res_phase);
              res_phase ^= 1;
            }
#pragma unroll
            for (int q = 0; q < 4; ++q) {
              const int j = sc * 8 + hb * 4 + q;
#pragma unroll
              for (int h = 0; h < 2; ++h) {
                const int r = frow + 8 * h;
                float2* dst = reinterpret_cast<float2*>(box + box_off(r, 2 * q + (fcol >> 2)) + (fcol & 2) * 4);
                float x0 = acc[4 * j + 2 * h], x1 = acc[4 * j + 2 * h + 1];
                if (!p.partial_out) epi_pair<BN, kMode>(p, x0, x1, par, j * 8 + fcol, ln_mean[h], ln_rstd[h], has_res ? *dst : make_float2(0.f, 0.f));
                *dst = make_float2(x0, x1);
              }
            }
            epi_publish<kRing>(&map_d, box, slot, leader, bar_id, bcol, wrow0, dz, reduce);
            ++box_i;
          }
        } else {
          const int bcol = n0 + sc * 64;
          uint8_t* box = ring + slot * kBoxBytes;
          if (p.aux != nullptr) {
#pragma unroll
            for (int q = 0; q < 4; ++q) {
              uint32_t rq[4];
#pragma unroll
              for (int i = 0; i < 4; ++i) {
                const int j = sc * 8 + 2 * q + (i >> 1), h = i & 1;
                float& x0 = acc[4 * j + 2 * h];
                float& x1 = acc[4 * j + 2 * h + 1];
                if (p.bias != nullptr) {
                  const float2 b = *reinterpret_cast<const float2*>(par + j * 8 + fcol);
                  x0 += b.x;
                  x1 += b.y;
                }
                rq[i] = pack2(x0, x1, p.out_dtype);
                const float2 a = unpack2(rq[i], p.out_dtype);
                x0 = a.x;
                x1 = a.y;
              }
              stmatrix_x4(smem_u32(box) + box_off(mrow, 2 * q + mcb), rq);
            }
            epi_publish<kRing>(&map_aux, box, slot, leader, bar_id, bcol, wrow0, 0, false);
            box = ring + slot * kBoxBytes;
#pragma unroll
            for (int q = 0; q < 4; ++q) {
              uint32_t rq[4];
#pragma unroll
              for (int i = 0; i < 4; ++i) {
                const int j = sc * 8 + 2 * q + (i >> 1), h = i & 1;
                float x0 = acc[4 * j + 2 * h], x1 = acc[4 * j + 2 * h + 1];
                gelu_pair(x0, x1);
                rq[i] = pack2(x0, x1, p.out_dtype);
              }
              stmatrix_x4(smem_u32(box) + box_off(mrow, 2 * q + mcb), rq);
            }
          } else {
#pragma unroll
            for (int q = 0; q < 4; ++q) {
              const uint32_t addr = smem_u32(box) + box_off(mrow, 2 * q + mcb);
              uint32_t rin[4] = {0u, 0u, 0u, 0u}, rq[4];
              if (has_res) ldmatrix_x4(rin, addr);
#pragma unroll
              for (int i = 0; i < 4; ++i) {
                const int j = sc * 8 + 2 * q + (i >> 1), h = i & 1;
                float x0 = acc[4 * j + 2 * h], x1 = acc[4 * j + 2 * h + 1];
                epi_pair<BN, kMode>(p, x0, x1, par, j * 8 + fcol, ln_mean[h], ln_rstd[h], unpack2(rin[i], p.out_dtype));
                rq[i] = pack2(x0, x1, p.out_dtype);
              }
              stmatrix_x4(addr, rq);
            }
          }
          epi_publish<kRing>(&map_d, box, slot, leader, bar_id, bcol, wrow0, 0, false);
          ++box_i;
        }
      }
    }
    if (leader) tma_store_wait<0>();
    if constexpr (kMode == kGemmLnBwd) {
      named_bar_sync(4, 256);
      float* part = reinterpret_cast<float*>(smem);
      const int warp = ct >> 5, jj = ((lane >> 4) & 1) * 4 + ((lane >> 3) & 1) * 2 + ((lane >> 2) & 1);
#pragma unroll
      for (int sc = 0; sc < BN / 64; ++sc)
#pragma unroll
        for (int i = 0; i < 4; ++i) part[(warp * 2 + (i >> 1)) * BN + sc * 64 + jj * 8 + fcol + (i & 1)] = colp[sc][i];
      named_bar_sync(4, 256);
      const int n0 = (blockIdx.x % num_n) * BN;
      float* row = p.ln_slab + static_cast<size_t>(blockIdx.x / num_n) * 2 * p.N;
      for (int t = ct; t < 2 * BN; t += 256) {
        const int q = t / BN, c = t - q * BN;
        float sum = 0.f;
#pragma unroll
        for (int w8 = 0; w8 < 8; ++w8) sum += part[(w8 * 2 + q) * BN + c];
        const int n = n0 + c, grp = n / p.ln_group;
        row[(grp * 2 + q) * p.ln_group + n - grp * p.ln_group] = sum;
      }
    }
  }
  if constexpr (kMode == kGemmLnBwd) {
    if (p.ln_cluster > 1) cluster_sync_all();
  }
}

template <int BN, bool kBf16, int kTA, int kTB, int kMode = kGemmPlain>
static int launch_gemm(const CUtensorMap* maps, const GemmParams& p, cudaStream_t stream) {
  constexpr int kSmem = GemmCfg<BN>::kSmemBytes;
  auto kern = gemm_tn_kernel<BN, kBf16, kTA, kTB, kMode>;
  static bool attr_set = false;
  if (!attr_set) {
    VDK_CUDA_OK(cudaFuncSetAttribute(kern, cudaFuncAttributeMaxDynamicSharedMemorySize, kSmem));
    attr_set = true;
  }
  const int num_tiles = ((p.M + kBM - 1) / kBM) * ((p.N + BN - 1) / BN) * p.split_k;
  const int grid = num_tiles < sm_count() ? num_tiles : sm_count();
  kern<<<grid, kGemmThreads, kSmem, stream>>>(maps[0], maps[1], maps[2], maps[3], maps[4], p);
  VDK_CUDA_OK(cudaGetLastError());
  return VDK_OK;
}

template <int BN, bool kBf16>
static int launch_gemm_major(const CUtensorMap* maps, const GemmParams& p, bool ta, bool tb, cudaStream_t s) {
  if (ta) return tb ? launch_gemm<BN, kBf16, 1, 1>(maps, p, s) : launch_gemm<BN, kBf16, 1, 0>(maps, p, s);
  return tb ? launch_gemm<BN, kBf16, 0, 1>(maps, p, s) : launch_gemm<BN, kBf16, 0, 0>(maps, p, s);
}

}

namespace vdk {

template <int BN>
static int launch_gemm_ln_bwd(const CUtensorMap* maps, const GemmParams& p, int cluster, cudaStream_t s, int* grid_out) {
  constexpr int kSmem = GemmCfg<BN>::kSmemBytes + kLnSmemBytes;
  static_assert(kSmem <= 227 * 1024, "LN-backward GEMM shared memory budget");
  auto kern = gemm_tn_kernel<BN, true, 0, 1, kGemmLnBwd>;
  static int fit[5] = {};
  cudaLaunchConfig_t cfg{};
  cfg.blockDim = dim3(kGemmThreads);
  cfg.dynamicSmemBytes = kSmem;
  cfg.stream = s;
  cudaLaunchAttribute attr[1];
  attr[0].id = cudaLaunchAttributeClusterDimension;
  attr[0].val.clusterDim.x = cluster;
  attr[0].val.clusterDim.y = 1;
  attr[0].val.clusterDim.z = 1;
  cfg.attrs = attr;
  cfg.numAttrs = 1;
  if (fit[cluster] == 0) {
    VDK_CUDA_OK(cudaFuncSetAttribute(kern, cudaFuncAttributeMaxDynamicSharedMemorySize, kSmem));
    int n = sm_count() / cluster;
    if (cluster > 1) {
      cfg.gridDim = dim3(cluster * sm_count());
      VDK_CUDA_OK(cudaOccupancyMaxActiveClusters(&n, kern, &cfg));
    }
    VDK_REQUIRE(n > 0, "vdk_gemm: no cluster of %d LN-backward GEMM CTAs fits on the device", cluster);
    fit[cluster] = n * cluster;
  }
  const int num_n = p.N / BN, num_tiles = ((p.M + kBM - 1) / kBM) * num_n;
  const int grid = std::min(num_tiles, fit[cluster] - fit[cluster] % num_n);
  cfg.gridDim = dim3(grid);
  VDK_CUDA_OK(cudaLaunchKernelEx(&cfg, kern, maps[0], maps[1], maps[2], maps[3], maps[4], p));
  *grid_out = grid;
  return VDK_OK;
}

static int gemm_ln_bwd_run(const vdk_gemm_desc& g, cudaStream_t s) {
  const int G = g.ln_group;
  VDK_REQUIRE(g.in_dtype == VDK_DTYPE_BF16 && g.out_dtype == VDK_DTYPE_BF16 && !g.trans_a && g.trans_b && g.split_k <= 1 &&
                  !g.bias && !g.aux_out && !g.a_col_sums,
              "vdk_gemm: LN_BWD needs bf16 in and out, trans_b only, no split-K, bias or auxiliary output");
  VDK_REQUIRE(g.gamma && g.beta && g.residual && g.ln_rstd && g.ln_dgamma && g.ln_dbeta && g.ln_slab,
              "vdk_gemm: LN_BWD needs gamma, beta, the saved output (residual), ln_rstd, ln_dgamma, ln_dbeta and ln_slab");
  const int BN = (g.N % 256 == 0) ? 256 : 128;
  VDK_REQUIRE(G > 0 && G % 128 == 0 && g.N % G == 0 && (BN % G == 0 || (G % BN == 0 && G / BN <= 4 && G / BN != 3)),
              "vdk_gemm: LN_BWD group %d must be 128, 256, 512 or 1024 and divide N=%d (tile width %d)", G, g.N, BN);
  VDK_REQUIRE(g.lda >= g.K && g.lda % 8 == 0 && g.ldb >= g.N && g.ldb % 8 == 0 && g.ldd >= g.N && g.ldd % 8 == 0 &&
                  (reinterpret_cast<uintptr_t>(g.D) & 15) == 0,
              "vdk_gemm: LN_BWD pitches must cover the rows and keep them 16-byte aligned");
  VDK_REQUIRE(g.ln_wo >= 0 && (g.ln_wo == 0 || (g.N == 4 * G && g.M % g.ln_wo == 0)),
              "vdk_gemm: LN_BWD patch rows need N = 4 ln_group and M a multiple of ln_wo");
  VDK_REQUIRE(g.ldr >= g.N && g.ldr % 8 == 0 && (reinterpret_cast<uintptr_t>(g.residual) & 15) == 0 &&
                  (reinterpret_cast<uintptr_t>(g.ln_slab) & 15) == 0,
              "vdk_gemm: LN_BWD saved-output rows and ln_slab must be 16-byte aligned");
  CUtensorMap maps[5];
  int rc = make_tma_2d_16bit(&maps[0], g.A, (uint64_t)g.M, (uint64_t)g.K, (uint64_t)g.lda, kBM, kBK);
  if (rc != VDK_OK) return rc;
  rc = make_tma_2d_16bit(&maps[1], g.B, (uint64_t)g.K, (uint64_t)g.N, (uint64_t)g.ldb, kBK, 64);
  if (rc != VDK_OK) return rc;
  rc = make_tma_epilogue_map(&maps[4], g.residual, 2, (uint64_t)g.M, (uint64_t)g.N, (uint64_t)g.ldr, 1, 0);
  if (rc != VDK_OK) return rc;
  maps[2] = maps[4];
  maps[3] = maps[4];
  GemmParams p{};
  p.M = g.M; p.N = g.N; p.K = g.K; p.D = g.D; p.ldd = g.ldd;
  p.gamma = g.gamma; p.beta = g.beta; p.residual = g.residual; p.ldr = g.ldr;
  p.out_dtype = VDK_DTYPE_BF16; p.epilogue = VDK_EPI_LN_BWD; p.split_k = 1;
  p.ln_slab = g.ln_slab; p.ln_rstd = g.ln_rstd; p.ln_group = G; p.ln_wo = g.ln_wo;
  p.ln_cluster = G > BN ? G / BN : 1;
  int grid = 0;
  {
    ProfScope prof(kProfGemm, 2.0 * g.M * g.N * g.K,
                   2.0 * (static_cast<double>(g.M) * g.K + static_cast<double>(g.N) * g.K) + 4.0 * g.M * g.N + 4.0 * g.M * (g.N / G), s);
    rc = BN == 256 ? launch_gemm_ln_bwd<256>(maps, p, p.ln_cluster, s, &grid) : launch_gemm_ln_bwd<128>(maps, p, p.ln_cluster, s, &grid);
    if (rc != VDK_OK) return rc;
  }
  const int n_part = grid / (g.N / BN) * (g.N / G);
  rc = launch_slab_reduce(g.ln_slab, n_part, static_cast<size_t>(2) * G, G / 4, g.ln_dgamma, 1, s);
  if (rc != VDK_OK) return rc;
  return launch_slab_reduce(g.ln_slab + G, n_part, static_cast<size_t>(2) * G, G / 4, g.ln_dbeta, 1, s);
}

int gemm_run(const vdk_gemm_desc& g, cudaStream_t s) {
  VDK_REQUIRE(g.A && g.B && g.D, "vdk_gemm: null operand");
  VDK_REQUIRE(g.M > 0 && g.N > 0 && g.K > 0, "vdk_gemm: empty problem M=%d N=%d K=%d", g.M, g.N, g.K);
  VDK_REQUIRE(g.in_dtype == VDK_DTYPE_BF16 || g.in_dtype == VDK_DTYPE_FP16, "vdk_gemm: in_dtype must be bf16/fp16");
  VDK_REQUIRE(g.out_dtype >= VDK_DTYPE_BF16 && g.out_dtype <= VDK_DTYPE_FP32, "vdk_gemm: bad out_dtype");
  VDK_REQUIRE(g.N % 8 == 0, "vdk_gemm: N must be a multiple of 8 (N=%d)", g.N);
  VDK_REQUIRE(g.lda >= (g.trans_a ? g.M : g.K) && g.ldb >= (g.trans_b ? g.N : g.K) && g.ldd >= g.N && g.lda % 8 == 0 &&
                  g.ldb % 8 == 0,
              "vdk_gemm: bad pitches");
  if (g.trans_a) VDK_REQUIRE(g.M % 8 == 0, "vdk_gemm: trans_a needs M to be a multiple of 8");
  const int dalign = g.out_dtype == VDK_DTYPE_FP32 ? 4 : 8;
  VDK_REQUIRE(g.ldd % dalign == 0, "vdk_gemm: ldd must keep rows 16-byte aligned");
  VDK_REQUIRE((reinterpret_cast<uintptr_t>(g.D) & 15) == 0, "vdk_gemm: D must be 16-byte aligned");
  if (g.epilogue == VDK_EPI_LN_BWD) return gemm_ln_bwd_run(g, s);
  VDK_REQUIRE(g.epilogue >= VDK_EPI_NONE && g.epilogue <= VDK_EPI_MUL_GELU_GRAD, "vdk_gemm: bad epilogue");
  if (g.epilogue == VDK_EPI_MUL_GELU_GRAD) {
    VDK_REQUIRE(g.residual && g.out_dtype != VDK_DTYPE_FP32 && g.split_k <= 1 && !g.bias,
                "vdk_gemm: MUL_GELU_GRAD needs the saved pre-activation in `residual`, a 16-bit output and no bias");
    VDK_REQUIRE(g.ldr >= g.N && g.ldr % 8 == 0 && (reinterpret_cast<uintptr_t>(g.residual) & 15) == 0,
                "vdk_gemm: pre-activation rows must be 16-byte aligned");
  }
  if (g.epilogue == VDK_EPI_SCALE_RESIDUAL) {
    VDK_REQUIRE(g.gamma && g.residual, "vdk_gemm: SCALE_RESIDUAL needs gamma and residual");
    VDK_REQUIRE(g.ldr >= g.N && g.ldr % dalign == 0 && (reinterpret_cast<uintptr_t>(g.residual) & 15) == 0,
                "vdk_gemm: residual must be 16-byte aligned rows");
  }
  if (g.epilogue == VDK_EPI_LAYERNORM) {
    VDK_REQUIRE(g.gamma && g.beta, "vdk_gemm: LAYERNORM needs gamma (weight) and beta (bias)");
    VDK_REQUIRE(g.N <= 256, "vdk_gemm: LAYERNORM epilogue needs the whole row in one tile (N <= 256, got %d)", g.N);
    VDK_REQUIRE((reinterpret_cast<uintptr_t>(g.beta) & 15) == 0, "vdk_gemm: beta must be 16-byte aligned");
  }
  if (g.bias) VDK_REQUIRE((reinterpret_cast<uintptr_t>(g.bias) & 15) == 0, "vdk_gemm: bias must be 16-byte aligned");
  if (g.gamma) VDK_REQUIRE((reinterpret_cast<uintptr_t>(g.gamma) & 15) == 0, "vdk_gemm: gamma must be 16-byte aligned");
  int split = g.split_k < 1 ? 1 : g.split_k;
  {
    const int kbt = (g.K + kBK - 1) / kBK;
    if (split > kbt) split = kbt;
    const int per = (kbt + split - 1) / split;
    split = (kbt + per - 1) / per;
  }
  if (g.split_stride != 0)
    VDK_REQUIRE(g.split_stride >= (long long)g.M * g.ldd && g.split_stride % 4 == 0, "vdk_gemm: split_stride must cover one [M,ldd] slab");
  if (g.split_k > 1)
    VDK_REQUIRE(g.out_dtype == VDK_DTYPE_FP32 && g.epilogue == VDK_EPI_NONE && !g.bias,
                "vdk_gemm: split_k > 1 needs fp32 output, no bias and no epilogue (partials are atomically added)");
  if (g.a_col_sums)
    VDK_REQUIRE(g.trans_a && g.split_k > 1 && g.split_stride != 0 && (reinterpret_cast<uintptr_t>(g.a_col_sums) & 15) == 0,
                "vdk_gemm: a_col_sums needs trans_a, split_k > 1 with split_stride > 0, and 16-byte alignment");

  bool wide = (g.N % 256 == 0) || g.N > 512;
  if (g.epilogue == VDK_EPI_LAYERNORM) wide = g.N > 128;
  const int BN = wide ? 256 : 128;
  CUtensorMap maps[5];
  CUtensorMap &ma = maps[0], &mb = maps[1], &md = maps[2], &maux = maps[3], &mr = maps[4];
  int rc = g.trans_a ? make_tma_2d_16bit(&ma, g.A, (uint64_t)g.K, (uint64_t)g.M, (uint64_t)g.lda, kBK, 64)
                     : make_tma_2d_16bit(&ma, g.A, (uint64_t)g.M, (uint64_t)g.K, (uint64_t)g.lda, kBM, kBK);
  if (rc != VDK_OK) return rc;
  rc = g.trans_b ? make_tma_2d_16bit(&mb, g.B, (uint64_t)g.K, (uint64_t)g.N, (uint64_t)g.ldb, kBK, 64)
                 : make_tma_2d_16bit(&mb, g.B, (uint64_t)g.N, (uint64_t)g.K, (uint64_t)g.ldb, BN, kBK);
  if (rc != VDK_OK) return rc;
  if (g.aux_out != nullptr) {
    VDK_REQUIRE(g.out_dtype != VDK_DTYPE_FP32 && g.split_k <= 1 && g.epilogue == VDK_EPI_GELU,
                "vdk_gemm: aux_out needs the GELU epilogue and a 16-bit output");
    VDK_REQUIRE((reinterpret_cast<uintptr_t>(g.aux_out) & 15) == 0, "vdk_gemm: aux_out must be 16-byte aligned");
  }
  const int osize = g.out_dtype == VDK_DTYPE_FP32 ? 4 : 2;
  const bool slabs = g.split_k > 1 && g.split_stride != 0;
  rc = make_tma_epilogue_map(&md, g.D, osize, (uint64_t)g.M, (uint64_t)g.N, (uint64_t)g.ldd, slabs ? (uint64_t)split : 1,
                             slabs ? (uint64_t)g.split_stride : 0);
  if (rc != VDK_OK) return rc;
  maux = md;
  mr = md;
  if (g.aux_out != nullptr) {
    rc = make_tma_epilogue_map(&maux, g.aux_out, 2, (uint64_t)g.M, (uint64_t)g.N, (uint64_t)g.ldd, 1, 0);
    if (rc != VDK_OK) return rc;
  }
  if (g.epilogue == VDK_EPI_SCALE_RESIDUAL || g.epilogue == VDK_EPI_MUL_GELU_GRAD) {
    rc = make_tma_epilogue_map(&mr, g.residual, osize, (uint64_t)g.M, (uint64_t)g.N, (uint64_t)g.ldr, 1, 0);
    if (rc != VDK_OK) return rc;
  }
  GemmParams p{g.M, g.N, g.K, g.D, g.ldd, g.bias, g.gamma, g.beta, g.residual, g.ldr, g.out_dtype, g.epilogue,
               g.ln_eps, split, g.split_k > 1 ? (long long)g.split_stride : 0ll, g.aux_out, (g.split_k > 1) ? 1 : 0};
  if (g.a_col_sums) p.col_sums = g.a_col_sums;
  const bool bf = g.in_dtype == VDK_DTYPE_BF16;
  const double osz = g.out_dtype == VDK_DTYPE_FP32 ? 4.0 : 2.0;
  ProfScope prof(kProfGemm, 2.0 * g.M * g.N * g.K,
                 2.0 * (static_cast<double>(g.M) * g.K + static_cast<double>(g.N) * g.K) + osz * g.M * g.N * (g.split_k > 1 ? split : 1) +
                     (g.aux_out ? 2.0 * g.M * g.N : 0.0) + (g.residual ? osz * g.M * g.N : 0.0),
                 s);
  const bool ta = g.trans_a != 0, tb = g.trans_b != 0;
  if (wide) return bf ? launch_gemm_major<256, true>(maps, p, ta, tb, s) : launch_gemm_major<256, false>(maps, p, ta, tb, s);
  return bf ? launch_gemm_major<128, true>(maps, p, ta, tb, s) : launch_gemm_major<128, false>(maps, p, ta, tb, s);
}

struct ConvArgs {
  const void* x;
  const void* w;
  const float* bias;
  const void* residual;
  void* y;
  int B, H, W, Cin, Cout, kernel, stride, epilogue;
  int pad_h[2], pad_w[2];
  bool ex;
};

static int conv_launch(const ConvArgs& c, cudaStream_t s) {
  const int Ho = (c.H + c.pad_h[0] + c.pad_h[1] - c.kernel) / c.stride + 1;
  const int Wo = (c.W + c.pad_w[0] + c.pad_w[1] - c.kernel) / c.stride + 1;
  const bool dense = c.kernel == 1 && c.stride == 1 && (c.pad_h[0] | c.pad_h[1] | c.pad_w[0] | c.pad_w[1]) == 0;
  const int Cinp = dense ? c.Cin : (c.Cin + kBK - 1) / kBK * kBK;
  const long long M = static_cast<long long>(c.B) * Ho * Wo;
  const long long K = static_cast<long long>(c.kernel) * c.kernel * Cinp;
  VDK_REQUIRE(M < (1ll << 31) && K < (1ll << 31), "vdk_conv2d: problem too large (M=%lld K=%lld)", M, K);
  const bool wide = (c.Cout % 256 == 0) || c.Cout > 512;
  CUtensorMap maps[5];
  int rc = dense ? make_tma_2d_16bit(&maps[0], c.x, (uint64_t)M, (uint64_t)c.Cin, (uint64_t)c.Cin, kBM, kBK)
         : c.ex  ? make_tma_im2col_16bit_pads(&maps[0], c.x, c.B, c.H, c.W, c.Cin, c.kernel, c.stride, c.pad_h, c.pad_w)
                 : make_tma_im2col_16bit(&maps[0], c.x, c.B, c.H, c.W, c.Cin, c.kernel, c.stride, c.pad_h[0]);
  if (rc != VDK_OK) return rc;
  rc = make_tma_2d_16bit(&maps[1], c.w, (uint64_t)c.Cout, (uint64_t)K, (uint64_t)K, wide ? 256 : 128, kBK);
  if (rc != VDK_OK) return rc;
  rc = make_tma_epilogue_map(&maps[2], c.y, 2, (uint64_t)M, (uint64_t)c.Cout, (uint64_t)c.Cout, 1, 0);
  if (rc != VDK_OK) return rc;
  maps[3] = maps[2];
  maps[4] = maps[2];
  if (c.residual != nullptr) {
    rc = make_tma_epilogue_map(&maps[4], c.residual, 2, (uint64_t)M, (uint64_t)c.Cout, (uint64_t)c.Cout, 1, 0);
    if (rc != VDK_OK) return rc;
  }
  GemmParams p{};
  p.M = static_cast<int>(M); p.N = c.Cout; p.K = static_cast<int>(K);
  p.D = c.y; p.ldd = c.Cout; p.bias = c.bias; p.residual = c.residual; p.ldr = c.Cout;
  p.out_dtype = VDK_DTYPE_BF16; p.epilogue = c.epilogue; p.split_k = 1;
  p.cv_cpb = Cinp / kBK; p.cv_kw = c.kernel; p.cv_stride = c.stride;
  p.cv_pad = c.ex ? (c.pad_h[0] | c.pad_w[0] << 8) : c.pad_h[0];
  p.cv_wo = Wo; p.cv_howo = Ho * Wo;
  ProfScope prof(kProfGemm, 2.0 * M * c.Cout * K,
                 2.0 * (static_cast<double>(c.B) * c.H * c.W * c.Cin + static_cast<double>(c.Cout) * K + M * c.Cout) +
                     (c.residual ? 2.0 * M * c.Cout : 0.0),
                 s);
  if (c.ex) {
    if (dense) return wide ? launch_gemm<256, true, 0, 0, kConvExDense>(maps, p, s) : launch_gemm<128, true, 0, 0, kConvExDense>(maps, p, s);
    return wide ? launch_gemm<256, true, 0, 0, kConvExIm2col>(maps, p, s) : launch_gemm<128, true, 0, 0, kConvExIm2col>(maps, p, s);
  }
  if (dense) return wide ? launch_gemm<256, true, 0, 0, kConvDense>(maps, p, s) : launch_gemm<128, true, 0, 0, kConvDense>(maps, p, s);
  return wide ? launch_gemm<256, true, 0, 0, kConvIm2col>(maps, p, s) : launch_gemm<128, true, 0, 0, kConvIm2col>(maps, p, s);
}

int conv_run(const vdk_conv_desc& c, cudaStream_t s) {
  VDK_REQUIRE(c.x && c.w && c.y, "vdk_conv2d: null operand");
  VDK_REQUIRE(c.B > 0 && c.H > 0 && c.W > 0, "vdk_conv2d: empty input B=%d H=%d W=%d", c.B, c.H, c.W);
// ... 201 lines not shown
```

visiondk_b200/csrc/train_gemm.h:

```cpp
#pragma once
#include <algorithm>

#include "vdk_host.h"

namespace vdk {

int launch_slab_reduce(const float* slabs, int n_slabs, size_t stride, int64_t n4, float* dst, int accumulate, cudaStream_t s);
int launch_slab_reduce_bias(const float* slabs, int n_slabs, size_t stride, const float* bias, int rows, int cols, float* out,
                            cudaStream_t s);
int launch_col_sum_f32_small(const float* x, int rows, int cols, float* out, cudaStream_t s);

inline int wgrad_splits(int M, int N, size_t K) {
  const int tiles = ((M + 127) / 128) * ((N + 255) / 256);
  const int want = std::max(2, (2 * sm_count()) / std::max(1, tiles));
  return vdk_gemm_effective_splits(static_cast<int>(K), want);
}
inline size_t wgrad_slab_bytes(int M, int N, size_t K) {
  return static_cast<size_t>(std::max(2, wgrad_splits(M, N, K))) * M * (static_cast<size_t>(N) + 1) * 4;
}

struct Gemm {
  cudaStream_t s;
  int run(const void* A, const void* B, void* D, int M, int N, int K, int lda, int ldb, int ldd, int epi, const float* bias,
          const float* gamma, const void* res, int ldr, int out_dtype, int split, long long stride, int ta, int tb,
          void* aux_out = nullptr, float* a_col_sums = nullptr) const {
    vdk_gemm_desc g{};
    g.A = A; g.B = B; g.D = D;
    g.M = M; g.N = N; g.K = K; g.lda = lda; g.ldb = ldb; g.ldd = ldd;
    g.in_dtype = VDK_DTYPE_BF16; g.out_dtype = out_dtype; g.epilogue = epi;
    g.bias = bias; g.gamma = gamma; g.residual = res; g.ldr = ldr;
    g.ln_eps = 1e-6f; g.split_k = split; g.split_stride = stride; g.trans_a = ta; g.trans_b = tb; g.aux_out = aux_out;
    g.a_col_sums = a_col_sums;
    return gemm_run(g, s);
  }
  int ln_bwd(const void* A, const void* B, void* D, int M, int N, int K, const void* y, const float* rstd, const float* ln_w,
             const float* ln_b, int group, int wo, float* dgamma, float* dbeta, float* slab) const {
    vdk_gemm_desc g{};
    g.A = A; g.B = B; g.D = D;
    g.M = M; g.N = N; g.K = K; g.lda = K; g.ldb = N; g.ldd = N;
    g.in_dtype = VDK_DTYPE_BF16; g.out_dtype = VDK_DTYPE_BF16; g.epilogue = VDK_EPI_LN_BWD;
    g.gamma = ln_w; g.beta = ln_b; g.residual = y; g.ldr = N;
    g.split_k = 1; g.trans_b = 1;
    g.ln_rstd = rstd; g.ln_dgamma = dgamma; g.ln_dbeta = dbeta; g.ln_slab = slab; g.ln_group = group; g.ln_wo = wo;
    return gemm_run(g, s);
  }
  int wgrad(const void* A, const void* B, float* D, int M, int N, int K, int lda, int ldb, float* slabs, bool accumulate,
            float* bias_grad = nullptr) const {
    VDK_REQUIRE((static_cast<size_t>(M) * N) % 4 == 0, "wgrad: M*N must be a multiple of 4");
    const int split = wgrad_splits(M, N, static_cast<size_t>(K));
    const size_t stride = static_cast<size_t>(M) * N;
    float* col_slabs = bias_grad ? slabs + static_cast<size_t>(split) * stride : nullptr;
    int rc = run(A, B, slabs, M, N, K, lda, ldb, N, VDK_EPI_NONE, nullptr, nullptr, nullptr, 0, VDK_DTYPE_FP32, std::max(2, split),
                 static_cast<long long>(stride), 1, 1, nullptr, col_slabs);
    if (rc != VDK_OK) return rc;
    rc = launch_slab_reduce(slabs, split, stride, static_cast<int64_t>(stride / 4), D, accumulate ? 1 : 0, s);
    if (rc != VDK_OK || !bias_grad) return rc;
    return launch_slab_reduce(col_slabs, split, static_cast<size_t>(M), M / 4, bias_grad, 1, s);
  }
};

#define RC(expr)                   \
  do {                             \
    int _rc = (expr);              \
    if (_rc != VDK_OK) return _rc; \
  } while (0)

}
```

visiondk_b200/csrc/train_ops.cu:

```cuda
#include "vdk_host.h"
#include "vdk_ptx.cuh"
#include "convnext_internal.h"

namespace vdk {

__device__ __forceinline__ float wsum(float v) {
#pragma unroll
  for (int off = 16; off > 0; off >>= 1) v += __shfl_xor_sync(0xffffffffu, v, off);
  return v;
}

__device__ __forceinline__ void unpack8(const uint4& t, float (&v)[8]) {
  const float2 a0 = __bfloat1622float2(*reinterpret_cast<const __nv_bfloat162*>(&t.x));
  const float2 a1 = __bfloat1622float2(*reinterpret_cast<const __nv_bfloat162*>(&t.y));
  const float2 a2 = __bfloat1622float2(*reinterpret_cast<const __nv_bfloat162*>(&t.z));
  const float2 a3 = __bfloat1622float2(*reinterpret_cast<const __nv_bfloat162*>(&t.w));
  v[0] = a0.x; v[1] = a0.y; v[2] = a1.x; v[3] = a1.y; v[4] = a2.x; v[5] = a2.y; v[6] = a3.x; v[7] = a3.y;
}
__device__ __forceinline__ uint4 pack8(const float (&v)[8]) {
  __nv_bfloat162 o0 = __floats2bfloat162_rn(v[0], v[1]), o1 = __floats2bfloat162_rn(v[2], v[3]);
  __nv_bfloat162 o2 = __floats2bfloat162_rn(v[4], v[5]), o3 = __floats2bfloat162_rn(v[6], v[7]);
  uint4 t;
  t.x = *reinterpret_cast<uint32_t*>(&o0); t.y = *reinterpret_cast<uint32_t*>(&o1);
  t.z = *reinterpret_cast<uint32_t*>(&o2); t.w = *reinterpret_cast<uint32_t*>(&o3);
  return t;
}


template <int LPP, int IT, int U>
__global__ void __launch_bounds__(256, IT >= 4 ? 1 : 2)
ln_bwd_kernel(const __nv_bfloat16* __restrict__ dy, const __nv_bfloat16* __restrict__ y, const float* __restrict__ rstd,
              int B, int H, int W, int C, const float* __restrict__ ln_w, const float* __restrict__ ln_b, int patch,
              __nv_bfloat16* __restrict__ dx, const __nv_bfloat16* __restrict__ addend, float* __restrict__ dgamma,
              float* __restrict__ dbeta) {
  constexpr int kPPW = 32 / LPP;
  extern __shared__ float ln_sm[];
  const int Cp = LPP * IT * 8;
  float* s_w = ln_sm;
  float* s_iw = s_w + Cp;
  float* s_b = s_iw + Cp;
  float* s_dg = s_b + Cp;
  float* s_db = s_dg + Cp;
  for (int c = threadIdx.x; c < Cp; c += 256) {
    float w = c < C ? ln_w[c] : 1.f;
    float iw = 0.f;
    if (w != 0.f) {
      if (fabsf(w) < 1e-12f) w = w < 0.f ? -1e-12f : 1e-12f;
      iw = 1.0f / w;
    }
    s_w[c] = w;
    s_iw[c] = iw;
    s_b[c] = c < C ? ln_b[c] : 0.f;
    s_dg[c] = 0.f;
    s_db[c] = 0.f;
  }
  __syncthreads();
  const int lane = threadIdx.x & 31, sub = lane % LPP;
  const int64_t npix = static_cast<int64_t>(B) * H * W;
  const int64_t nwarps = (static_cast<int64_t>(gridDim.x) * blockDim.x) >> 5;
  const int64_t warp_id = (static_cast<int64_t>(blockIdx.x) * blockDim.x + threadIdx.x) >> 5;
  const float inv_c = 1.0f / static_cast<float>(C);
  float gw[IT][8], gb[IT][8];
#pragma unroll
  for (int i = 0; i < IT; ++i)
#pragma unroll
    for (int j = 0; j < 8; ++j) { gw[i][j] = 0.f; gb[i][j] = 0.f; }

  for (int64_t base = warp_id * (kPPW * U); base < npix; base += nwarps * (kPPW * U)) {
    uint4 rdy[U][IT], ry[U][IT];
    int64_t pix[U], roff[U];
#pragma unroll
    for (int u = 0; u < U; ++u) {
      pix[u] = base + u * kPPW + lane / LPP;
      const bool ok = pix[u] < npix;
      int64_t orow = pix[u];
      int ocol0 = 0;
      if (patch == 2 && ok) {
        const int xw = static_cast<int>(pix[u] % W);
        const int yh = static_cast<int>((pix[u] / W) % H);
        const int b = static_cast<int>(pix[u] / (static_cast<int64_t>(W) * H));
        orow = (static_cast<int64_t>(b) * (H / 2) + (yh >> 1)) * (W / 2) + (xw >> 1);
        ocol0 = ((yh & 1) * 2 + (xw & 1)) * C;
      }
      roff[u] = orow * (static_cast<int64_t>(C) * patch * patch) + ocol0;
#pragma unroll
      for (int i = 0; i < IT; ++i) {
        const int c = (sub + i * LPP) * 8;
        rdy[u][i] = make_uint4(0, 0, 0, 0);
        ry[u][i] = make_uint4(0, 0, 0, 0);
        if (ok && c < C) {
          rdy[u][i] = __ldg(reinterpret_cast<const uint4*>(dy + roff[u] + c));
          ry[u][i] = __ldg(reinterpret_cast<const uint4*>(y + roff[u] + c));
        }
      }
    }
    float s1[U], s2[U];
#pragma unroll
    for (int u = 0; u < U; ++u) { s1[u] = 0.f; s2[u] = 0.f; }
#pragma unroll
    for (int i = 0; i < IT; ++i) {
      const int c = (sub + i * LPP) * 8;
      float w[8], iw[8], bb[8];
      *reinterpret_cast<float4*>(&w[0]) = *reinterpret_cast<const float4*>(s_w + c);
            *reinterpret_cast<float4*>(&w[4]) = *reinterpret_cast<const float4*>(s_w + c + 4);
      *reinterpret_cast<float4*>(&iw[0]) = *reinterpret_cast<const float4*>(s_iw + c);
            *reinterpret_cast<float4*>(&iw[4]) = *reinterpret_cast<const float4*>(s_iw + c + 4);
      *reinterpret_cast<float4*>(&bb[0]) = *reinterpret_cast<const float4*>(s_b + c);
            *reinterpret_cast<float4*>(&bb[4]) = *reinterpret_cast<const float4*>(s_b + c + 4);
#pragma unroll
      for (int u = 0; u < U; ++u) {
        const bool okc = pix[u] < npix && c < C;
        float vdy[8], vy[8];
        unpack8(rdy[u][i], vdy);
        unpack8(ry[u][i], vy);
#pragma unroll
        for (int j = 0; j < 8; ++j) {
          const float h = okc ? (vy[j] - bb[j]) * iw[j] : 0.f;
          const float g = vdy[j] * w[j];
          s1[u] += g;
          s2[u] = fmaf(g, h, s2[u]);
          gw[i][j] = fmaf(vdy[j], h, gw[i][j]);
          gb[i][j] += vdy[j];
        }
      }
    }
#pragma unroll
    for (int u = 0; u < U; ++u) {
#pragma unroll
      for (int off = LPP / 2; off > 0; off >>= 1) {
        s1[u] += __shfl_xor_sync(0xffffffffu, s1[u], off);
        s2[u] += __shfl_xor_sync(0xffffffffu, s2[u], off);
      }
    }
#pragma unroll
    for (int u = 0; u < U; ++u) {
      if (pix[u] < npix) {
        const float rs = rstd[pix[u]];
        const float m1 = s1[u] * inv_c, m2 = s2[u] * inv_c;
#pragma unroll
        for (int i = 0; i < IT; ++i) {
          const int c = (sub + i * LPP) * 8;
          if (c < C) {
            float w[8], iw[8], bb[8];
            *reinterpret_cast<float4*>(&w[0]) = *reinterpret_cast<const float4*>(s_w + c);
            *reinterpret_cast<float4*>(&w[4]) = *reinterpret_cast<const float4*>(s_w + c + 4);
            *reinterpret_cast<float4*>(&iw[0]) = *reinterpret_cast<const float4*>(s_iw + c);
            *reinterpret_cast<float4*>(&iw[4]) = *reinterpret_cast<const float4*>(s_iw + c + 4);
            *reinterpret_cast<float4*>(&bb[0]) = *reinterpret_cast<const float4*>(s_b + c);
            *reinterpret_cast<float4*>(&bb[4]) = *reinterpret_cast<const float4*>(s_b + c + 4);
            float vdy[8], vy[8], o[8];
            if constexpr (IT > 4) {
              asm volatile("" : "+r"(rdy[u][i].x), "+r"(rdy[u][i].y), "+r"(rdy[u][i].z), "+r"(rdy[u][i].w));
              asm volatile("" : "+r"(ry[u][i].x), "+r"(ry[u][i].y), "+r"(ry[u][i].z), "+r"(ry[u][i].w));
            }
            unpack8(rdy[u][i], vdy);
            unpack8(ry[u][i], vy);
#pragma unroll
            for (int j = 0; j < 8; ++j) {
              const float h = (vy[j] - bb[j]) * iw[j];
              o[j] = rs * (vdy[j] * w[j] - m1 - h * m2);
            }
            if (addend) {
              float a[8];
              unpack8(__ldg(reinterpret_cast<const uint4*>(addend + pix[u] * C + c)), a);
#pragma unroll
              for (int j = 0; j < 8; ++j) o[j] += a[j];
            }
            *reinterpret_cast<uint4*>(dx + pix[u] * C + c) = pack8(o);
          }
        }
      }
    }
  }
#pragma unroll
  for (int i = 0; i < IT; ++i) {
    const int c = (sub + i * LPP) * 8;
#pragma unroll
    for (int j = 0; j < 8; ++j) {
      float a = gw[i][j], b2 = gb[i][j];
#pragma unroll
      for (int off = LPP; off < 32; off <<= 1) {
        a += __shfl_xor_sync(0xffffffffu, a, off);
        b2 += __shfl_xor_sync(0xffffffffu, b2, off);
      }
      if (lane < LPP) {
        atomicAdd(s_dg + c + j, a);
        atomicAdd(s_db + c + j, b2);
      }
    }
  }
  __syncthreads();
  for (int c = threadIdx.x; c < C; c += 256) {
    atomicAdd(dgamma + c, s_dg[c]);
    atomicAdd(dbeta + c, s_db[c]);
  }
}

template <int LPP, int IT, int U>
static void ln_bwd_launch(const __nv_bfloat16* dy, const __nv_bfloat16* y, const float* rstd, int B, int H, int W, int C,
                          const float* ln_w, const float* ln_b, int patch, __nv_bfloat16* dx, const __nv_bfloat16* addend,
                          float* dgamma, float* dbeta, cudaStream_t s) {
  const int64_t npix = static_cast<int64_t>(B) * H * W;
  const int64_t pix_per_block_trip = 8 * (32 / LPP) * U;
  const int blocks = static_cast<int>(std::max<int64_t>(1, std::min<int64_t>((npix + pix_per_block_trip - 1) / pix_per_block_trip,
                                                                              sm_count() * (IT >= 4 ? 1 : 2))));
  const size_t smem = static_cast<size_t>(LPP) * IT * 8 * 5 * sizeof(float);
  ln_bwd_kernel<LPP, IT, U><<<blocks, 256, smem, s>>>(dy, y, rstd, B, H, W, C, ln_w, ln_b, patch, dx, addend, dgamma, dbeta);
}

int launch_ln_bwd(const __nv_bfloat16* dy, const __nv_bfloat16* y, const float* rstd, int B, int H, int W, int C,
                  const float* ln_w, const float* ln_b, int patch, __nv_bfloat16* dx, const __nv_bfloat16* addend,
                  float* dgamma, float* dbeta, cudaStream_t s) {
  VDK_REQUIRE(C % 8 == 0 && C <= 1536, "ln_bwd: C must be a multiple of 8, <= 1536 (got %d)", C);
  const int vecs = C / 8;
  if (vecs <= 8) ln_bwd_launch<8, 1, 4>(dy, y, rstd, B, H, W, C, ln_w, ln_b, patch, dx, addend, dgamma, dbeta, s);
  else if (vecs <= 16) ln_bwd_launch<16, 1, 4>(dy, y, rstd, B, H, W, C, ln_w, ln_b, patch, dx, addend, dgamma, dbeta, s);
  else if (vecs <= 32) ln_bwd_launch<32, 1, 4>(dy, y, rstd, B, H, W, C, ln_w, ln_b, patch, dx, addend, dgamma, dbeta, s);
  else if (vecs <= 64) ln_bwd_launch<32, 2, 2>(dy, y, rstd, B, H, W, C, ln_w, ln_b, patch, dx, addend, dgamma, dbeta, s);
  else if (vecs <= 96) ln_bwd_launch<32, 3, 1>(dy, y, rstd, B, H, W, C, ln_w, ln_b, patch, dx, addend, dgamma, dbeta, s);
  else if (vecs <= 128) ln_bwd_launch<32, 4, 1>(dy, y, rstd, B, H, W, C, ln_w, ln_b, patch, dx, addend, dgamma, dbeta, s);
  else ln_bwd_launch<32, 6, 1>(dy, y, rstd, B, H, W, C, ln_w, ln_b, patch, dx, addend, dgamma, dbeta, s);
  VDK_CUDA_OK(cudaGetLastError());
  return VDK_OK;
}

constexpr int kWgT = 14;
constexpr int kWgC = 64;
constexpr int kWgR = 7;

template <int TT>
__global__ void __launch_bounds__(224)
dwconv7_wgrad_kernel(const __grid_constant__ CUtensorMap map_x, const __grid_constant__ CUtensorMap map_g, int B, int H,
                     int W, int C, int T_rt, int ipc, float* __restrict__ dw49, float* __restrict__ dbias) {
  extern __shared__ uint8_t wg_raw[];
  uint8_t* smem = wg_raw + ((128u - (smem_u32(wg_raw) & 127u)) & 127u);
  const int T = TT > 0 ? TT : T_rt;
  const int halo = T + 6;
  const int nh = (T + kWgR - 1) / kWgR;
  const int planes = 7 * nh;
  const int x_bytes = halo * halo * kWgC * 2, g_bytes = T * T * kWgC * 2;
  const int red_bytes = (planes * 7 + nh) * kWgC * 4;
  const int first = ((x_bytes > red_bytes ? x_bytes : red_bytes) + 127) & ~127;
  uint8_t* sx = smem;
  float* red = reinterpret_cast<float*>(smem);
  uint8_t* sg = smem + first;
  uint64_t* bar = reinterpret_cast<uint64_t*>(sg + ((g_bytes + 127) & ~127));

  const int tiles_w = (W + T - 1) / T, tiles_h = (H + T - 1) / T;
  const int n_cc = (C + kWgC - 1) / kWgC;
  int bid = blockIdx.x;
  const int cc = bid % n_cc; bid /= n_cc;
  const int tw = bid % tiles_w; bid /= tiles_w;
  const int th = bid % tiles_h;
  const int b0 = (bid / tiles_h) * ipc;
  const int b1 = min(B, b0 + ipc);
  const int oy0 = th * T, ox0 = tw * T;

  if (threadIdx.x == 0) {
    prefetch_tensormap(&map_x);
    prefetch_tensormap(&map_g);
    mbar_init(bar, 1);
    fence_mbar_init();
  }
  __syncthreads();

  const int quad = threadIdx.x & 15, plane = threadIdx.x >> 4;
  const bool active = plane < planes;
  const int hh = plane / 7, dy = plane - hh * 7;
  const int px0 = hh * kWgR;
  float2 acc[7][2];
#pragma unroll
  for (int dx = 0; dx < 7; ++dx) {
    acc[dx][0] = make_float2(0.f, 0.f);
    acc[dx][1] = make_float2(0.f, 0.f);
  }
  float bsum[4] = {0.f, 0.f, 0.f, 0.f};

  uint32_t phase = 0;
  for (int b = b0; b < b1; ++b) {
    if (threadIdx.x == 0) {
      mbar_arrive_expect_tx(bar, x_bytes + g_bytes);
      tma_load_4d(sx, &map_x, bar, cc * kWgC, ox0 - 3, oy0 - 3, b);
      tma_load_4d(sg, &map_g, bar, cc * kWgC, ox0, oy0, b);
    }
    mbar_wait(bar, phase);
    phase ^= 1u;
    if (active) {
#pragma unroll 1
      for (int py = 0; py < T; ++py) {
        float2 g[kWgR][2], x[kWgR + 6][2];
        const uint8_t* gr = sg + ((py * T + px0) * kWgC + quad * 4) * 2;
#pragma unroll
        for (int r = 0; r < kWgR; ++r) {
          uint2 t = make_uint2(0u, 0u);
          if (TT > 0 || px0 + r < T) t = *reinterpret_cast<const uint2*>(gr + r * kWgC * 2);
          g[r][0] = make_float2(__uint_as_float(t.x << 16), __uint_as_float(t.x & 0xffff0000u));
          g[r][1] = make_float2(__uint_as_float(t.y << 16), __uint_as_float(t.y & 0xffff0000u));
        }
        const uint8_t* xr = sx + (((py + dy) * halo + px0) * kWgC + quad * 4) * 2;
#pragma unroll
        for (int i = 0; i < kWgR + 6; ++i) {
          uint2 t = make_uint2(0u, 0u);
          if (TT > 0 || px0 + i < halo) t = *reinterpret_cast<const uint2*>(xr + i * kWgC * 2);
          x[i][0] = make_float2(__uint_as_float(t.x << 16), __uint_as_float(t.x & 0xffff0000u));
          x[i][1] = make_float2(__uint_as_float(t.y << 16), __uint_as_float(t.y & 0xffff0000u));
        }
        if (dy == 0) {
#pragma unroll
          for (int r = 0; r < kWgR; ++r) {
            bsum[0] += g[r][0].x; bsum[1] += g[r][0].y; bsum[2] += g[r][1].x; bsum[3] += g[r][1].y;
          }
        }
#pragma unroll
        for (int r = 0; r < kWgR; ++r)
#pragma unroll
          for (int dx = 0; dx < 7; ++dx) {
            acc[dx][0] = ffma2(g[r][0], x[r + dx][0], acc[dx][0]);
            acc[dx][1] = ffma2(g[r][1], x[r + dx][1], acc[dx][1]);
          }
      }
    }
    __syncthreads();
  }

  if (active) {
#pragma unroll
    for (int dx = 0; dx < 7; ++dx)
      *reinterpret_cast<float4*>(red + (plane * 7 + dx) * kWgC + quad * 4) =
          make_float4(acc[dx][0].x, acc[dx][0].y, acc[dx][1].x, acc[dx][1].y);
    if (dy == 0) {
#pragma unroll
      for (int c = 0; c < 4; ++c) red[(planes * 7 + hh) * kWgC + quad * 4 + c] = bsum[c];
    }
  }
  __syncthreads();
  for (int o = threadIdx.x; o < 50 * kWgC; o += blockDim.x) {
    const int slot = o / kWgC, ch = o - slot * kWgC;
    if (cc * kWgC + ch >= C) continue;
    float s = 0.f;
    if (slot < 49) {
      const int sdy = slot / 7, sdx = slot - sdy * 7;
      for (int h2 = 0; h2 < nh; ++h2) s += red[((h2 * 7 + sdy) * 7 + sdx) * kWgC + ch];
      atomicAdd(dw49 + slot * C + cc * kWgC + ch, s);
    } else {
      for (int h2 = 0; h2 < nh; ++h2) s += red[(planes * 7 + h2) * kWgC + ch];
      atomicAdd(dbias + cc * kWgC + ch, s);
    }
  }
}

int launch_dwconv7_wgrad(const __nv_bfloat16* x, const __nv_bfloat16* dconv, int B, int H, int W, int C, float* dw49,
                         float* dbias, cudaStream_t s) {
  const double wg_elems = static_cast<double>(B) * H * W * C;
  ProfScope prof(kProfDepthwise, 2.0 * 49.0 * wg_elems, 2.0 * 2.0 * wg_elems, s);

  VDK_REQUIRE(C % 8 == 0, "dwconv7_wgrad: C must be a multiple of 8 (got %d)", C);
  const int T = std::min(kWgT, std::max(H, W));
  CUtensorMap mx, mg;
  int rc = make_tma_nhwc_16bit(&mx, x, B, H, W, C, T + 6, T + 6, kWgC);
  if (rc != VDK_OK) return rc;
  rc = make_tma_nhwc_16bit(&mg, dconv, B, H, W, C, T, T, kWgC);
  if (rc != VDK_OK) return rc;
  const int halo = T + 6, nh = (T + kWgR - 1) / kWgR, planes = 7 * nh;
  const int x_bytes = halo * halo * kWgC * 2, red_bytes = (planes * 7 + nh) * kWgC * 4;
  const int smem = ((std::max(x_bytes, red_bytes) + 127) & ~127) + ((T * T * kWgC * 2 + 127) & ~127) + 16 + 128;
  VDK_CUDA_OK(cudaFuncSetAttribute(dwconv7_wgrad_kernel<14>, cudaFuncAttributeMaxDynamicSharedMemorySize, 160 * 1024));
  VDK_CUDA_OK(cudaFuncSetAttribute(dwconv7_wgrad_kernel<7>, cudaFuncAttributeMaxDynamicSharedMemorySize, 160 * 1024));
  VDK_CUDA_OK(cudaFuncSetAttribute(dwconv7_wgrad_kernel<0>, cudaFuncAttributeMaxDynamicSharedMemorySize, 160 * 1024));
  const int64_t per_image = static_cast<int64_t>((H + T - 1) / T) * ((W + T - 1) / T) * ((C + kWgC - 1) / kWgC);
  const int ipc = static_cast<int>(std::max<int64_t>(1, std::min<int64_t>(16, (per_image * B) / (sm_count() * 4))));
  const unsigned grid = static_cast<unsigned>(((B + ipc - 1) / ipc) * per_image);
  const int threads = ((16 * planes + 31) / 32) * 32;
  if (T == 14) dwconv7_wgrad_kernel<14><<<grid, threads, smem, s>>>(mx, mg, B, H, W, C, T, ipc, dw49, dbias);
  else if (T == 7) dwconv7_wgrad_kernel<7><<<grid, threads, smem, s>>>(mx, mg, B, H, W, C, T, ipc, dw49, dbias);
  else dwconv7_wgrad_kernel<0><<<grid, threads, smem, s>>>(mx, mg, B, H, W, C, T, ipc, dw49, dbias);
  VDK_CUDA_OK(cudaGetLastError());
  return VDK_OK;
}

template <typename TIn, typename TOut>
__global__ void __launch_bounds__(256)
bn_train_fwd_kernel(const TIn* __restrict__ x, int R, int C, const float* __restrict__ weight, const float* __restrict__ bias,
                    float eps, float momentum, TOut* __restrict__ y, float* __restrict__ save_mean,
                    float* __restrict__ save_rstd, float* __restrict__ running_mean, float* __restrict__ running_var) {
  __shared__ float red[8][33];
  __shared__ float s_mean[32], s_rstd[32];
  const int lane = threadIdx.x & 31, warp = threadIdx.x >> 5;
  const int c = blockIdx.x * 32 + lane;
  const bool ok = c < C;
  float s = 0.f;
  if (ok) for (int r = warp; r < R; r += 8) s += static_cast<float>(x[static_cast<int64_t>(r) * C + c]);
  red[warp][lane] = s;
  __syncthreads();
  if (warp == 0) {
    float t = 0.f;
#pragma unroll
    for (int w = 0; w < 8; ++w) t += red[w][lane];
    s_mean[lane] = t / static_cast<float>(R);
  }
  __syncthreads();
  const float mean = s_mean[lane];
  float q = 0.f;
  if (ok) for (int r = warp; r < R; r += 8) {
    const float d = static_cast<float>(x[static_cast<int64_t>(r) * C + c]) - mean;
    q = fmaf(d, d, q);
  }
  red[warp][lane] = q;
  __syncthreads();
  if (warp == 0) {
    float t = 0.f;
#pragma unroll
    for (int w = 0; w < 8; ++w) t += red[w][lane];
    const float var = t / static_cast<float>(R);
    s_rstd[lane] = rsqrtf(var + eps);
    if (ok) {
      save_mean[c] = mean;
      save_rstd[c] = s_rstd[lane];
      if (running_mean) {
        running_mean[c] = (1.f - momentum) * running_mean[c] + momentum * mean;
        const float unb = R > 1 ? t / static_cast<float>(R - 1) : var;
        running_var[c] = (1.f - momentum) * running_var[c] + momentum * unb;
      }
    }
  }
  __syncthreads();
  if (ok) {
    const float rs = s_rstd[lane], w = weight[c], b = bias[c];
    for (int r = warp; r < R; r += 8) {
      const float v = (static_cast<float>(x[static_cast<int64_t>(r) * C + c]) - mean) * rs * w + b;
      y[static_cast<int64_t>(r) * C + c] = static_cast<TOut>(v);
    }
  }
}

template <typename TIn, typename TGrad>
__global__ void __launch_bounds__(256)
bn_train_bwd_kernel(const TGrad* __restrict__ dy, const TIn* __restrict__ x, int R, int C, const float* __restrict__ weight,
                    const float* __restrict__ save_mean, const float* __restrict__ save_rstd, TGrad* __restrict__ dx,
                    float* __restrict__ dweight, float* __restrict__ dbias) {
  __shared__ float red[2][8][33];
  __shared__ float s_a[32], s_b[32];
  const int lane = threadIdx.x & 31, warp = threadIdx.x >> 5;
  const int c = blockIdx.x * 32 + lane;
  const bool ok = c < C;
  const float mean = ok ? save_mean[c] : 0.f, rs = ok ? save_rstd[c] : 0.f;
  float s1 = 0.f, s2 = 0.f;
  if (ok) for (int r = warp; r < R; r += 8) {
    const float g = static_cast<float>(dy[static_cast<int64_t>(r) * C + c]);
    const float xh = (static_cast<float>(x[static_cast<int64_t>(r) * C + c]) - mean) * rs;
    s1 += g;
    s2 = fmaf(g, xh, s2);
  }
  red[0][warp][lane] = s1;
  red[1][warp][lane] = s2;
  __syncthreads();
  if (warp == 0) {
    float a = 0.f, b = 0.f;
#pragma unroll
    for (int w = 0; w < 8; ++w) {
      a += red[0][w][lane];
      b += red[1][w][lane];
    }
    s_a[lane] = a;
    s_b[lane] = b;
    if (ok) {
      dbias[c] += a;
      dweight[c] += b;
    }
  }
  __syncthreads();
  if (ok) {
    const float w = weight[c], m1 = s_a[lane] / static_cast<float>(R), m2 = s_b[lane] / static_cast<float>(R);
    for (int r = warp; r < R; r += 8) {
      const float g = static_cast<float>(dy[static_cast<int64_t>(r) * C + c]);
      const float xh = (static_cast<float>(x[static_cast<int64_t>(r) * C + c]) - mean) * rs;
      dx[static_cast<int64_t>(r) * C + c] = static_cast<TGrad>(w * rs * (g - m1 - xh * m2));
    }
  }
}

__device__ __forceinline__ void block_sum8(float (&v)[8], float (*red)[8]) {
#pragma unroll
  for (int j = 0; j < 8; ++j) v[j] = wsum(v[j]);
  const int lane = threadIdx.x & 31, warp = threadIdx.x >> 5;
  __syncthreads();
  if (lane == 0) {
#pragma unroll
    for (int j = 0; j < 8; ++j) red[warp][j] = v[j];
  }
  __syncthreads();
#pragma unroll
  for (int j = 0; j < 8; ++j) {
    float t = 0.f;
#pragma unroll
    for (int w = 0; w < 8; ++w) t += red[w][j];
    v[j] = t;
  }
}

__global__ void __launch_bounds__(256)
bn_train_fwd_vec_kernel(const __nv_bfloat16* __restrict__ x, int R, int C, const float* __restrict__ weight,
                        const float* __restrict__ bias, float eps, float momentum, __nv_bfloat16* __restrict__ y,
                        float* __restrict__ save_mean, float* __restrict__ save_rstd, float* __restrict__ running_mean,
                        float* __restrict__ running_var) {
  __shared__ float red[8][8];
  const int c0 = blockIdx.x * 8;
  const float inv_r = 1.0f / static_cast<float>(R);
  float mean[8], q[8], v[8];
#pragma unroll
  for (int j = 0; j < 8; ++j) { mean[j] = 0.f; q[j] = 0.f; }
  for (int r = threadIdx.x; r < R; r += 256) {
    unpack8(__ldg(reinterpret_cast<const uint4*>(x + static_cast<int64_t>(r) * C + c0)), v);
#pragma unroll
    for (int j = 0; j < 8; ++j) mean[j] += v[j];
  }
  block_sum8(mean, red);
#pragma unroll
  for (int j = 0; j < 8; ++j) mean[j] *= inv_r;
  for (int r = threadIdx.x; r < R; r += 256) {
    unpack8(__ldg(reinterpret_cast<const uint4*>(x + static_cast<int64_t>(r) * C + c0)), v);
#pragma unroll
    for (int j = 0; j < 8; ++j) {
      const float d = v[j] - mean[j];
      q[j] = fmaf(d, d, q[j]);
    }
  }
  block_sum8(q, red);
  float sc[8], sh[8];
#pragma unroll
  for (int j = 0; j < 8; ++j) {
    const float var = q[j] * inv_r;
    const float rs = rsqrtf(var + eps);
    sc[j] = rs * weight[c0 + j];
    sh[j] = bias[c0 + j] - mean[j] * sc[j];
    if (threadIdx.x == 0) {
      save_mean[c0 + j] = mean[j];
      save_rstd[c0 + j] = rs;
      if (running_mean) {
        running_mean[c0 + j] = (1.f - momentum) * running_mean[c0 + j] + momentum * mean[j];
        const float unb = R > 1 ? q[j] / static_cast<float>(R - 1) : var;
        running_var[c0 + j] = (1.f - momentum) * running_var[c0 + j] + momentum * unb;
      }
    }
  }
  for (int r = threadIdx.x; r < R; r += 256) {
    unpack8(__ldg(reinterpret_cast<const uint4*>(x + static_cast<int64_t>(r) * C + c0)), v);
    float o[8];
#pragma unroll
    for (int j = 0; j < 8; ++j) o[j] = fmaf(v[j], sc[j], sh[j]);
    *reinterpret_cast<uint4*>(y + static_cast<int64_t>(r) * C + c0) = pack8(o);
  }
}

__global__ void __launch_bounds__(256)
bn_train_bwd_vec_kernel(const __nv_bfloat16* __restrict__ dy, const __nv_bfloat16* __restrict__ x, int R, int C,
                        const float* __restrict__ weight, const float* __restrict__ save_mean,
                        const float* __restrict__ save_rstd, __nv_bfloat16* __restrict__ dx, float* __restrict__ dweight,
                        float* __restrict__ dbias) {
  __shared__ float red[8][8];
  const int c0 = blockIdx.x * 8;
  float mean[8], rs[8], s1[8], s2[8], g[8], v[8];
#pragma unroll
  for (int j = 0; j < 8; ++j) {
    mean[j] = save_mean[c0 + j];
    rs[j] = save_rstd[c0 + j];
    s1[j] = 0.f;
    s2[j] = 0.f;
  }
  for (int r = threadIdx.x; r < R; r += 256) {
    unpack8(__ldg(reinterpret_cast<const uint4*>(dy + static_cast<int64_t>(r) * C + c0)), g);
    unpack8(__ldg(reinterpret_cast<const uint4*>(x + static_cast<int64_t>(r) * C + c0)), v);
#pragma unroll
    for (int j = 0; j < 8; ++j) {
      s1[j] += g[j];
      s2[j] = fmaf(g[j], (v[j] - mean[j]) * rs[j], s2[j]);
    }
  }
  block_sum8(s1, red);
  block_sum8(s2, red);
  const float inv_r = 1.0f / static_cast<float>(R);
  float a[8], m1[8], m2[8];
#pragma unroll
  for (int j = 0; j < 8; ++j) {
    if (threadIdx.x == 0) {
      dbias[c0 + j] += s1[j];
      dweight[c0 + j] += s2[j];
    }
    a[j] = weight[c0 + j] * rs[j];
    m1[j] = s1[j] * inv_r;
    m2[j] = s2[j] * inv_r;
  }
  for (int r = threadIdx.x; r < R; r += 256) {
    unpack8(__ldg(reinterpret_cast<const uint4*>(dy + static_cast<int64_t>(r) * C + c0)), g);
    unpack8(__ldg(reinterpret_cast<const uint4*>(x + static_cast<int64_t>(r) * C + c0)), v);
    float o[8];
#pragma unroll
    for (int j = 0; j < 8; ++j) o[j] = a[j] * (g[j] - m1[j] - (v[j] - mean[j]) * rs[j] * m2[j]);
    *reinterpret_cast<uint4*>(dx + static_cast<int64_t>(r) * C + c0) = pack8(o);
  }
}

__global__ void __launch_bounds__(256)
permute021_kernel(const float* __restrict__ in, int A, int Bd, int Cd, const float* __restrict__ row_scale,
                  __nv_bfloat16* __restrict__ out_bf16, float* __restrict__ out_f32, int accumulate) {
  const int64_t total = static_cast<int64_t>(A) * Bd * Cd;
  for (int64_t i = static_cast<int64_t>(blockIdx.x) * blockDim.x + threadIdx.x; i < total;
       i += static_cast<int64_t>(gridDim.x) * blockDim.x) {
    const int b = static_cast<int>(i % Bd);
    const int c = static_cast<int>((i / Bd) % Cd);
    const int a = static_cast<int>(i / (static_cast<int64_t>(Bd) * Cd));
    float v = in[(static_cast<int64_t>(a) * Bd + b) * Cd + c];
    if (row_scale) v *= row_scale[a];
    if (out_bf16) out_bf16[i] = __float2bfloat16_rn(v);
    if (out_f32) out_f32[i] = accumulate ? out_f32[i] + v : v;
  }
}

__global__ void __launch_bounds__(256)
permute021_tiled_kernel(const float* __restrict__ in, int Bd, int Cd, const float* __restrict__ row_scale,
                        __nv_bfloat16* __restrict__ out_bf16, float* __restrict__ out_f32, int accumulate) {
  __shared__ float tile[32][33];
  const int a = blockIdx.z, b0 = blockIdx.y * 32, c0 = blockIdx.x * 32;
  const int tx = threadIdx.x & 31, ty = threadIdx.x >> 5;
  const float sc = row_scale ? row_scale[a] : 1.f;
  const int64_t base = static_cast<int64_t>(a) * Bd * Cd;
#pragma unroll
  for (int r = ty; r < 32; r += 8) {
    const int b = b0 + r, c = c0 + tx;
    if (b < Bd && c < Cd) tile[r][tx] = in[base + static_cast<int64_t>(b) * Cd + c] * sc;
  }
  __syncthreads();
#pragma unroll
  for (int r = ty; r < 32; r += 8) {
    const int c = c0 + r, b = b0 + tx;
    if (b < Bd && c < Cd) {
      const int64_t o = base + static_cast<int64_t>(c) * Bd + b;
      const float v = tile[tx][r];
      if (out_bf16) out_bf16[o] = __float2bfloat16_rn(v);
      if (out_f32) out_f32[o] = accumulate ? out_f32[o] + v : v;
    }
  }
}

__global__ void __launch_bounds__(256)
layerscale_finalize_kernel(const float* __restrict__ G, const float* __restrict__ W2, const float* __restrict__ b2,
                           const float* __restrict__ gamma, const float* __restrict__ sdo, int C, int K4,
                           float* __restrict__ dW2, float* __restrict__ dgamma, float* __restrict__ db2) {
  __shared__ float red[8];
  const int c = blockIdx.x;
  const float gm = gamma[c];
  float dot = 0.f;
  for (int k = threadIdx.x; k < K4; k += 256) {
    const float g = G[static_cast<int64_t>(c) * K4 + k];
    dot = fmaf(g, W2[static_cast<int64_t>(c) * K4 + k], dot);
    dW2[static_cast<int64_t>(c) * K4 + k] += gm * g;
  }
  dot = wsum(dot);
  if ((threadIdx.x & 31) == 0) red[threadIdx.x >> 5] = dot;
  __syncthreads();
  if (threadIdx.x == 0) {
    float t = 0.f;
#pragma unroll
    for (int w = 0; w < 8; ++w) t += red[w];
    dgamma[c] += t + b2[c] * sdo[c];
    db2[c] += gm * sdo[c];
  }
}

__global__ void cast_f32_bf16_kernel(const float* __restrict__ in, int64_t n, __nv_bfloat16* __restrict__ out) {
  for (int64_t i = static_cast<int64_t>(blockIdx.x) * blockDim.x + threadIdx.x; i < n;
       i += static_cast<int64_t>(gridDim.x) * blockDim.x)
    out[i] = __float2bfloat16_rn(in[i]);
}
__global__ void add_f32_kernel(float* __restrict__ dst, const float* __restrict__ src, int64_t n) {
  for (int64_t i = static_cast<int64_t>(blockIdx.x) * blockDim.x + threadIdx.x; i < n;
       i += static_cast<int64_t>(gridDim.x) * blockDim.x)
    dst[i] += src[i];
}

static int blocks_for(int64_t n) { return static_cast<int>(std::max<int64_t>(1, std::min<int64_t>((n + 255) / 256, 132 * 16))); }

int launch_permute021(const float* in, int A, int Bd, int Cd, const float* row_scale, __nv_bfloat16* out_bf16,
                      float* out_f32, int accumulate, cudaStream_t s) {
  if (Bd >= 16 && Cd >= 16 && A <= 65535 && (Bd + 31) / 32 <= 65535) {
    const dim3 grid((Cd + 31) / 32, (Bd + 31) / 32, A);
    permute021_tiled_kernel<<<grid, 256, 0, s>>>(in, Bd, Cd, row_scale, out_bf16, out_f32, accumulate);
  } else {
    permute021_kernel<<<blocks_for(static_cast<int64_t>(A) * Bd * Cd), 256, 0, s>>>(in, A, Bd, Cd, row_scale, out_bf16, out_f32,
                                                                                   accumulate);
  }
  VDK_CUDA_OK(cudaGetLastError());
  return VDK_OK;
}
int launch_cast_bf16(const float* in, int64_t n, __nv_bfloat16* out, cudaStream_t s) {
  cast_f32_bf16_kernel<<<blocks_for(n), 256, 0, s>>>(in, n, out);
  VDK_CUDA_OK(cudaGetLastError());
  return VDK_OK;
}
int launch_layerscale_finalize(const float* G, const float* W2, const float* b2, const float* gamma, const float* sdo, int C,
                               int K4, float* dW2, float* dgamma, float* db2, cudaStream_t s) {
  layerscale_finalize_kernel<<<C, 256, 0, s>>>(G, W2, b2, gamma, sdo, C, K4, dW2, dgamma, db2);
  VDK_CUDA_OK(cudaGetLastError());
  return VDK_OK;
}
int launch_bn_fwd_bf16(const __nv_bfloat16* x, int R, int C, const float* w, const float* b, float eps, float momentum,
                       __nv_bfloat16* y, float* save_mean, float* save_rstd, float* run_mean, float* run_var, cudaStream_t s) {
  if (C % 8 == 0)
    bn_train_fwd_vec_kernel<<<C / 8, 256, 0, s>>>(x, R, C, w, b, eps, momentum, y, save_mean, save_rstd, run_mean, run_var);
  else
    bn_train_fwd_kernel<__nv_bfloat16, __nv_bfloat16><<<(C + 31) / 32, 256, 0, s>>>(x, R, C, w, b, eps, momentum, y, save_mean,
                                                                                    save_rstd, run_mean, run_var);
  VDK_CUDA_OK(cudaGetLastError());
  return VDK_OK;
}
int launch_bn_fwd_f32(const float* x, int R, int C, const float* w, const float* b, float eps, float momentum, float* y,
                      float* save_mean, float* save_rstd, float* run_mean, float* run_var, cudaStream_t s) {
  bn_train_fwd_kernel<float, float><<<(C + 31) / 32, 256, 0, s>>>(x, R, C, w, b, eps, momentum, y, save_mean, save_rstd, run_mean,
                                                                  run_var);
  VDK_CUDA_OK(cudaGetLastError());
  return VDK_OK;
}
int launch_bn_bwd_bf16(const __nv_bfloat16* dy, const __nv_bfloat16* x, int R, int C, const float* w, const float* save_mean,
                       const float* save_rstd, __nv_bfloat16* dx, float* dweight, float* dbias, cudaStream_t s) {
  if (C % 8 == 0)
    bn_train_bwd_vec_kernel<<<C / 8, 256, 0, s>>>(dy, x, R, C, w, save_mean, save_rstd, dx, dweight, dbias);
  else
    bn_train_bwd_kernel<__nv_bfloat16, __nv_bfloat16><<<(C + 31) / 32, 256, 0, s>>>(dy, x, R, C, w, save_mean, save_rstd, dx,
                                                                                    dweight, dbias);
  VDK_CUDA_OK(cudaGetLastError());
  return VDK_OK;
}
int launch_bn_bwd_f32(const float* dy, const float* x, int R, int C, const float* w, const float* save_mean,
                      const float* save_rstd, float* dx, float* dweight, float* dbias, cudaStream_t s) {
  bn_train_bwd_kernel<float, float><<<(C + 31) / 32, 256, 0, s>>>(dy, x, R, C, w, save_mean, save_rstd, dx, dweight, dbias);
  VDK_CUDA_OK(cudaGetLastError());
  return VDK_OK;
}
int launch_add_f32(float* dst, const float* src, int64_t n, cudaStream_t s) {
  add_f32_kernel<<<blocks_for(n), 256, 0, s>>>(dst, src, n);
  VDK_CUDA_OK(cudaGetLastError());
  return VDK_OK;
}

}

using namespace vdk;

extern "C" int vdk_layernorm_bwd(const void* dy, const void* y, const float* rstd, int batch, int H, int W, int C,
                                 const float* ln_w, const float* ln_b, int patch, void* dx, const void* addend, float* dgamma,
                                 float* dbeta, void* stream) {
  VDK_REQUIRE(dy && y && rstd && ln_w && ln_b && dx && dgamma && dbeta, "vdk_layernorm_bwd: null operand");
  VDK_REQUIRE(patch == 1 || (patch == 2 && H % 2 == 0 && W % 2 == 0), "vdk_layernorm_bwd: patch must be 1 or 2");
  return launch_ln_bwd(reinterpret_cast<const __nv_bfloat16*>(dy), reinterpret_cast<const __nv_bfloat16*>(y), rstd, batch, H, W, C,
                       ln_w, ln_b, patch, reinterpret_cast<__nv_bfloat16*>(dx), reinterpret_cast<const __nv_bfloat16*>(addend),
                       dgamma, dbeta, reinterpret_cast<cudaStream_t>(stream));
}

extern "C" int vdk_dwconv7(int mode, const void* x, int batch, int H, int W, int C, const float* w49, const float* bias,
                           const float* ln_w, const float* ln_b, float eps, void* y, float* rstd_out, const void* addend,
                           void* stream) {
  VDK_REQUIRE(x && y && w49 && (mode == 1 || (bias && ln_w && ln_b)), "vdk_dwconv7: null operand");
  return launch_dwconv7(mode, reinterpret_cast<const __nv_bfloat16*>(x), batch, H, W, C, w49, bias, ln_w, ln_b, eps,
                        reinterpret_cast<__nv_bfloat16*>(y), rstd_out, reinterpret_cast<const __nv_bfloat16*>(addend),
                        reinterpret_cast<cudaStream_t>(stream));
}

extern "C" int vdk_dwconv7_wgrad(const void* x, const void* dconv, int batch, int H, int W, int C, float* dw49, float* dbias,
                                 void* stream) {
  VDK_REQUIRE(x && dconv && dw49 && dbias, "vdk_dwconv7_wgrad: null operand");
  return launch_dwconv7_wgrad(reinterpret_cast<const __nv_bfloat16*>(x), reinterpret_cast<const __nv_bfloat16*>(dconv), batch, H, W,
                              C, dw49, dbias, reinterpret_cast<cudaStream_t>(stream));
}

extern "C" int vdk_batchnorm_train_fwd(const void* x, int rows, int C, int is_bf16, const float* weight, const float* bias,
                                       float eps, float momentum, void* y, float* save_mean, float* save_rstd,
                                       float* running_mean, float* running_var, void* stream) {
  VDK_REQUIRE(x && y && weight && bias && save_mean && save_rstd && rows > 1, "vdk_batchnorm_train_fwd: bad arguments");
  cudaStream_t s = reinterpret_cast<cudaStream_t>(stream);
  if (is_bf16)
    return launch_bn_fwd_bf16(reinterpret_cast<const __nv_bfloat16*>(x), rows, C, weight, bias, eps, momentum,
                              reinterpret_cast<__nv_bfloat16*>(y), save_mean, save_rstd, running_mean, running_var, s);
  return launch_bn_fwd_f32(reinterpret_cast<const float*>(x), rows, C, weight, bias, eps, momentum, reinterpret_cast<float*>(y),
                           save_mean, save_rstd, running_mean, running_var, s);
}

extern "C" int vdk_batchnorm_train_bwd(const void* dy, const void* x, int rows, int C, int is_bf16, const float* weight,
                                       const float* save_mean, const float* save_rstd, void* dx, float* dweight, float* dbias,
                                       void* stream) {
  VDK_REQUIRE(dy && x && weight && save_mean && save_rstd && dx && dweight && dbias, "vdk_batchnorm_train_bwd: null operand");
  cudaStream_t s = reinterpret_cast<cudaStream_t>(stream);
  if (is_bf16)
    return launch_bn_bwd_bf16(reinterpret_cast<const __nv_bfloat16*>(dy), reinterpret_cast<const __nv_bfloat16*>(x), rows, C, weight,
                              save_mean, save_rstd, reinterpret_cast<__nv_bfloat16*>(dx), dweight, dbias, s);
  return launch_bn_bwd_f32(reinterpret_cast<const float*>(dy), reinterpret_cast<const float*>(x), rows, C, weight, save_mean,
                           save_rstd, reinterpret_cast<float*>(dx), dweight, dbias, s);
}
```

visiondk_b200/csrc/vdk_host.h:

```cpp
#pragma once
#include <cuda.h>
#include <cuda_runtime.h>
#include <cstdint>
#include <cstdio>
#include <cstdarg>

#include "../../include/vdk_b200.h"

namespace vdk {

void set_error(const char* fmt, ...);
int fail(int code, const char* fmt, ...);

#define VDK_CUDA_OK(expr)                                                                          \
  do {                                                                                             \
    cudaError_t _e = (expr);                                                                       \
    if (_e != cudaSuccess)                                                                         \
      return ::vdk::fail(VDK_ERR_CUDA, "%s failed: %s (%s:%d)", #expr, cudaGetErrorString(_e), __FILE__, __LINE__); \
  } while (0)

#define VDK_REQUIRE(cond, ...)                                       \
  do {                                                               \
    if (!(cond)) return ::vdk::fail(VDK_ERR_INVALID, __VA_ARGS__);   \
  } while (0)

int make_tma_2d_16bit(CUtensorMap* map, const void* base, uint64_t rows, uint64_t cols, uint64_t ld,
                      uint32_t box_rows, uint32_t box_cols);

int make_tma_nhwc_16bit(CUtensorMap* map, const void* base, int B, int H, int W, int C, int box_h, int box_w, int box_c);

int make_tma_im2col_16bit(CUtensorMap* map, const void* base, int B, int H, int W, int C, int kernel, int stride, int pad);
int make_tma_im2col_16bit_pads(CUtensorMap* map, const void* base, int B, int H, int W, int C, int kernel, int stride,
                               const int pad_h[2], const int pad_w[2]);

int make_tma_qkv_16bit(CUtensorMap* map, const void* base, int D, int H, int N, int B, uint32_t box_cols, uint32_t box_rows);

int make_tma_epilogue_map(CUtensorMap* map, const void* base, int elem_bytes, uint64_t rows, uint64_t cols, uint64_t ld,
                          uint64_t depth, uint64_t depth_stride);

int sm_count();

enum ProfCategory { kProfGemm = 0, kProfDepthwise = 1, kProfAttention = 2, kProfScoreFilter = 3, kProfOther = 4, kProfCategories = 5 };
struct ProfScope {
  ProfScope(int category, double flops, double bytes, cudaStream_t stream);
  ~ProfScope();
  int slot;
  cudaStream_t stream;
};

}

namespace vdk {
int gemm_run(const vdk_gemm_desc& g, cudaStream_t stream);
int conv_run(const vdk_conv_desc& c, cudaStream_t stream);
int conv_grouped_run(const vdk_conv_desc& c, int groups, cudaStream_t stream);
int conv_ex_run(const vdk_conv_ex_desc& c, cudaStream_t stream, bool allow_relu = false);
int conv_grouped_ex_run(const vdk_conv_desc& c, int groups, cudaStream_t stream);
int conv_grouped_ex_cpb(int Cin, int Cout, int groups);
}
```

visiondk_b200/csrc/vdk_ptx.cuh:

```cuda
#pragma once
#include <cstdint>
#include <cstdio>
#include <cuda.h>
#include <cuda_runtime.h>
#include <cuda_bf16.h>
#include <cuda_fp16.h>

#include "vdk_wgmma.cuh"

namespace vdk {

__device__ __forceinline__ float hardswish(float x) { return x * fminf(fmaxf(x + 3.f, 0.f), 6.f) * (1.f / 6.f); }

__device__ __forceinline__ uint32_t smem_u32(const void* p) {
  return static_cast<uint32_t>(__cvta_generic_to_shared(p));
}

__device__ __forceinline__ uint32_t lane_id() {
  uint32_t l;
  asm volatile("mov.u32 %0, %%laneid;" : "=r"(l));
  return l;
}

__device__ __forceinline__ bool elect_one() {
// ... 19 lines not shown
}
__device__ __forceinline__ void mbar_arrive_expect_tx(uint64_t* bar, uint32_t bytes) {
  asm volatile("mbarrier.arrive.expect_tx.shared::cta.b64 _, [%0], %1;" ::"r"(smem_u32(bar)), "r"(bytes)
               : "memory");
}
__device__ __forceinline__ void mbar_arrive(uint64_t* bar) {
  asm volatile("mbarrier.arrive.shared::cta.b64 _, [%0];" ::"r"(smem_u32(bar)) : "memory");
}
__device__ __forceinline__ bool mbar_try_wait(uint64_t* bar, uint32_t parity) {
  uint32_t ok;
  asm volatile(
      "{\n\t"
      ".reg .pred P;\n\t"
      "mbarrier.try_wait.parity.shared::cta.b64 P, [%1], %2;\n\t"
      "selp.u32 %0, 1, 0, P;\n\t"
      "}\n"
      : "=r"(ok)
      : "r"(smem_u32(bar)), "r"(parity)
      : "memory");
  return ok != 0;
}

template <bool kQuiet = false>
__device__ __forceinline__ void mbar_wait(uint64_t* bar, uint32_t parity) {
  if (mbar_try_wait(bar, parity)) return;
  const long long t0 = clock64();
  while (!mbar_try_wait(bar, parity)) {
    if (clock64() - t0 > 4000000000LL) {
      if (!kQuiet) printf("vdk: mbarrier wait timed out (block %d, thread %d, parity %u)\n", (int)blockIdx.x, (int)threadIdx.x, parity);
      __trap();
    }
  }
}

template <bool kQuiet = false>
__device__ __forceinline__ void mbar_wait_relaxed(uint64_t* bar, uint32_t parity) {
  if (mbar_try_wait(bar, parity)) return;
  const long long t0 = clock64();
  int polls = 0;
  while (!mbar_try_wait(bar, parity)) {
    if (++polls > 4) __nanosleep(64);
    if (clock64() - t0 > 4000000000LL) {
      if (!kQuiet) printf("vdk: mbarrier wait timed out (block %d, thread %d, parity %u)\n", (int)blockIdx.x, (int)threadIdx.x, parity);
      __trap();
    }
  }
}

__device__ __forceinline__ void prefetch_tensormap(const CUtensorMap* m) {
  asm volatile("prefetch.tensormap [%0];" ::"l"(reinterpret_cast<uint64_t>(m)) : "memory");
}

constexpr uint64_t kEvictNormal = 0x1000000000000000ull;
constexpr uint64_t kEvictFirst = 0x12F0000000000000ull;
constexpr uint64_t kEvictLast = 0x14F0000000000000ull;

__device__ __forceinline__ void tma_load_2d(void* smem_dst, const CUtensorMap* map, uint64_t* bar, int c0,
                                            int c1, uint64_t policy) {
  asm volatile(
      "cp.async.bulk.tensor.2d.shared::cluster.global.tile.mbarrier::complete_tx::bytes.L2::cache_hint"
      " [%0], [%1, {%3, %4}], [%2], %5;"
      ::"r"(smem_u32(smem_dst)),
      "l"(reinterpret_cast<uint64_t>(map)), "r"(smem_u32(bar)), "r"(c0), "r"(c1), "l"(policy)
      : "memory");
}

__device__ __forceinline__ void tma_load_im2col_4d(void* smem_dst, const CUtensorMap* map, uint64_t* bar, int c, int w, int h,
                                                   int n, uint16_t off_w, uint16_t off_h, uint64_t policy) {
  asm volatile(
      "cp.async.bulk.tensor.4d.shared::cluster.global.im2col.mbarrier::complete_tx::bytes.L2::cache_hint"
      " [%0], [%1, {%3, %4, %5, %6}], [%2], {%7, %8}, %9;"
      ::"r"(smem_u32(smem_dst)),
      "l"(reinterpret_cast<uint64_t>(map)), "r"(smem_u32(bar)), "r"(c), "r"(w), "r"(h), "r"(n), "h"(off_w), "h"(off_h),
      "l"(policy)
      : "memory");
}

__device__ __forceinline__ void tma_load_4d(void* smem_dst, const CUtensorMap* map, uint64_t* bar, int c0, int c1,
                                            int c2, int c3) {
  asm volatile(
      "cp.async.bulk.tensor.4d.shared::cluster.global.tile.mbarrier::complete_tx::bytes"
      " [%0], [%1, {%3, %4, %5, %6}], [%2];"
      ::"r"(smem_u32(smem_dst)),
      "l"(reinterpret_cast<uint64_t>(map)), "r"(smem_u32(bar)), "r"(c0), "r"(c1), "r"(c2), "r"(c3)
      : "memory");
}

__device__ __forceinline__ void tma_load_3d(void* smem_dst, const CUtensorMap* map, uint64_t* bar, int c0, int c1, int c2) {
  asm volatile(
      "cp.async.bulk.tensor.3d.shared::cluster.global.tile.mbarrier::complete_tx::bytes"
      " [%0], [%1, {%3, %4, %5}], [%2];"
      ::"r"(smem_u32(smem_dst)),
      "l"(reinterpret_cast<uint64_t>(map)), "r"(smem_u32(bar)), "r"(c0), "r"(c1), "r"(c2)
      : "memory");
}

__device__ __forceinline__ void tma_store_2d(const CUtensorMap* map, const void* smem_src, int c0, int c1) {
  asm volatile("cp.async.bulk.tensor.2d.global.shared::cta.tile.bulk_group [%0, {%2, %3}], [%1];" ::"l"(
                   reinterpret_cast<uint64_t>(map)),
               "r"(smem_u32(smem_src)), "r"(c0), "r"(c1)
               : "memory");
}
__device__ __forceinline__ void tma_store_commit() { asm volatile("cp.async.bulk.commit_group;" ::: "memory"); }
template <int N>
__device__ __forceinline__ void tma_store_wait_read() {
  asm volatile("cp.async.bulk.wait_group.read %0;" ::"n"(N) : "memory");
}
template <int N>
__device__ __forceinline__ void tma_store_wait() {
  asm volatile("cp.async.bulk.wait_group %0;" ::"n"(N) : "memory");
}
__device__ __forceinline__ void tma_store_3d(const CUtensorMap* map, const void* smem_src, int c0, int c1, int c2) {
  asm volatile("cp.async.bulk.tensor.3d.global.shared::cta.tile.bulk_group [%0, {%2, %3, %4}], [%1];" ::"l"(
                   reinterpret_cast<uint64_t>(map)),
               "r"(smem_u32(smem_src)), "r"(c0), "r"(c1), "r"(c2)
               : "memory");
}
__device__ __forceinline__ void tma_reduce_add_3d(const CUtensorMap* map, const void* smem_src, int c0, int c1, int c2) {
  asm volatile("cp.reduce.async.bulk.tensor.3d.global.shared::cta.add.tile.bulk_group [%0, {%2, %3, %4}], [%1];" ::"l"(
                   reinterpret_cast<uint64_t>(map)),
               "r"(smem_u32(smem_src)), "r"(c0), "r"(c1), "r"(c2)
               : "memory");
}

__device__ __forceinline__ void cp_async_16_zfill(void* smem_dst, const void* src, bool valid) {
  asm volatile("cp.async.cg.shared.global [%0], [%1], 16, %2;" ::"r"(smem_u32(smem_dst)), "l"(src), "r"(valid ? 16 : 0)
               : "memory");
}
__device__ __forceinline__ void cp_async_wait_all() { asm volatile("cp.async.wait_all;" ::: "memory"); }

__device__ __forceinline__ void ldmatrix_x4(uint32_t (&r)[4], uint32_t addr) {
  asm volatile("ldmatrix.sync.aligned.m8n8.x4.shared.b16 {%0, %1, %2, %3}, [%4];"
               : "=r"(r[0]), "=r"(r[1]), "=r"(r[2]), "=r"(r[3]) : "r"(addr));
}
__device__ __forceinline__ void ldmatrix_x4_trans(uint32_t (&r)[4], uint32_t addr) {
  asm volatile("ldmatrix.sync.aligned.m8n8.x4.trans.shared.b16 {%0, %1, %2, %3}, [%4];"
               : "=r"(r[0]), "=r"(r[1]), "=r"(r[2]), "=r"(r[3]) : "r"(addr));
}
__device__ __forceinline__ void stmatrix_x4(uint32_t addr, const uint32_t (&r)[4]) {
  asm volatile("stmatrix.sync.aligned.m8n8.x4.shared.b16 [%0], {%1, %2, %3, %4};"
               ::"r"(addr), "r"(r[0]), "r"(r[1]), "r"(r[2]), "r"(r[3]) : "memory");
}

__device__ __forceinline__ uint32_t cluster_ctarank() {
  uint32_t r;
  asm volatile("mov.u32 %0, %%cluster_ctarank;" : "=r"(r));
  return r;
}
__device__ __forceinline__ void cluster_sync_all() {
  asm volatile("barrier.cluster.arrive.release.aligned;" ::: "memory");
  asm volatile("barrier.cluster.wait.acquire.aligned;" ::: "memory");
}

__device__ __forceinline__ float2 ffma2(float2 a, float2 b, float2 c) {
  return make_float2(fmaf(a.x, b.x, c.x), fmaf(a.y, b.y, c.y));
}

__device__ __forceinline__ void named_bar_sync(uint32_t id, uint32_t nthreads) {
  asm volatile("bar.sync %0, %1;" ::"r"(id), "r"(nthreads) : "memory");
}

}
```

Baseline: 2424.

## Enable programmatic dependent launch across training kernels and merge paired slab reductions

Launches most training-step kernels (GEMMs, dwconv, layernorm, reductions, casts, BN, permutes) with the programmatic stream serialization attribute, and adds a griddepcontrol.wait at the start of each kernel. The next kernel's launch and prologue (barrier init, tensormap prefetch) can then overlap the tail of the previous kernel. It also merges the two back-to-back slab reductions (dgamma/dbeta, dW/dbias) into a single launch. No kernel issues an early launch trigger, so overlap is limited to the block scheduling and setup that happens before the wait.

```diff
diff --git a/visiondk_b200/csrc/convnext.cu b/visiondk_b200/csrc/convnext.cu
--- a/visiondk_b200/csrc/convnext.cu
+++ b/visiondk_b200/csrc/convnext.cu
@@ -422,6 +422,7 @@
     }
     fence_mbar_init();
   }
+  grid_dep_wait();
   for (int i = threadIdx.x; i < 49 * (CHUNK / 4); i += blockDim.x) {
     const int t = i / (CHUNK / 4), q = i - t * (CHUNK / 4);
     *reinterpret_cast<float4*>(wsm + t * CHUNK + q * 4) = __ldg(reinterpret_cast<const float4*>(w49 + t * C + ck * CHUNK + q * 4));
@@ -658,6 +659,7 @@
 ln_patchify_kernel(const __nv_bfloat16* __restrict__ x, int B, int H, int W, int C, const float* __restrict__ ln_w,
                    const float* __restrict__ ln_b, float eps, int patch , __nv_bfloat16* __restrict__ out,
                    float* __restrict__ rstd_out) {
+  grid_dep_wait();
   constexpr int kPPW = 32 / LPP;
   constexpr int kMaxIter = 8;
   const int lane = threadIdx.x & 31;
@@ -741,16 +743,17 @@
   VDK_REQUIRE(C % 8 == 0 && C <= 2048, "layernorm_patchify: C must be a multiple of 8, <= 2048 (got %d)", C);
   const int64_t npix = static_cast<int64_t>(B) * H * W;
   const int vecs = C / 8;
+  auto kern = ln_patchify_kernel<32>;
+  int64_t warps = npix;
   if (vecs <= 8) {
-    const int64_t warps = (npix + 3) / 4;
-    ln_patchify_kernel<8><<<static_cast<unsigned>((warps * 32 + 255) / 256), 256, 0, s>>>(x, B, H, W, C, ln_w, ln_b, eps, patch, out, rstd_out);
+    kern = ln_patchify_kernel<8>;
+    warps = (npix + 3) / 4;
   } else if (vecs <= 16) {
-    const int64_t warps = (npix + 1) / 2;
-    ln_patchify_kernel<16><<<static_cast<unsigned>((warps * 32 + 255) / 256), 256, 0, s>>>(x, B, H, W, C, ln_w, ln_b, eps, patch, out, rstd_out);
-  } else {
-    ln_patchify_kernel<32><<<static_cast<unsigned>((npix * 32 + 255) / 256), 256, 0, s>>>(x, B, H, W, C, ln_w, ln_b, eps, patch, out, rstd_out);
-  }
-  VDK_CUDA_OK(cudaGetLastError());
+    kern = ln_patchify_kernel<16>;
+    warps = (npix + 1) / 2;
+  }
+  VDK_CUDA_OK(launch_pdl(kern, dim3(static_cast<unsigned>((warps * 32 + 255) / 256)), dim3(256), 0, s, x, B, H, W, C, ln_w, ln_b,
+                         eps, patch, out, rstd_out));
   return VDK_OK;
 }
 
@@ -858,11 +861,12 @@
   cfg.blockDim = dim3((TH + 1) * 32);
   cfg.dynamicSmemBytes = smem;
   cfg.stream = s;
-  cudaLaunchAttribute attr[1];
+  cudaLaunchAttribute attr[2];
   attr[0].id = cudaLaunchAttributeClusterDimension;
   attr[0].val.clusterDim.x = cluster;
   attr[0].val.clusterDim.y = 1;
   attr[0].val.clusterDim.z = 1;
+  attr[1] = pdl_attribute();
   cfg.attrs = attr;
   cfg.numAttrs = 1;
   if (fit[cluster].clusters == 0) {
@@ -886,6 +890,7 @@
     const int g = std::max(1, std::min(n_tiles, slots / nchunks));
     cfg.gridDim = dim3(static_cast<unsigned>(g) * nchunks);
   }
+  cfg.numAttrs = 2;
   VDK_CUDA_OK(cudaLaunchKernelEx(&cfg, kern, mx, batch, H, W, C, nchunks, n_tiles, w49, bias, ln_w, ln_b, eps, y, rstd_out, addend));
   return VDK_OK;
 }
diff --git a/visiondk_b200/csrc/convnext_train.cu b/visiondk_b200/csrc/convnext_train.cu
--- a/visiondk_b200/csrc/convnext_train.cu
+++ b/visiondk_b200/csrc/convnext_train.cu
@@ -99,6 +99,7 @@
 
 __global__ void slab_reduce_bias_kernel(const float* __restrict__ slabs, int n_slabs, size_t stride, const float* __restrict__ bias,
                                         int rows, int cols, float* __restrict__ out) {
+  grid_dep_wait();
   const int i = blockIdx.x * blockDim.x + threadIdx.x;
   if (i >= rows * cols) return;
   float v = bias ? bias[i % cols] : 0.f;
@@ -107,16 +108,25 @@
 }
 int launch_slab_reduce_bias(const float* slabs, int n_slabs, size_t stride, const float* bias, int rows, int cols, float* out,
                             cudaStream_t s) {
-  slab_reduce_bias_kernel<<<(rows * cols + 255) / 256, 256, 0, s>>>(slabs, n_slabs, stride, bias, rows, cols, out);
+  VDK_CUDA_OK(launch_pdl(slab_reduce_bias_kernel, dim3((rows * cols + 255) / 256), dim3(256), 0, s, slabs, n_slabs, stride,
+                         bias, rows, cols, out));
   VDK_CUDA_OK(cudaGetLastError());
   return VDK_OK;
 }
 __global__ void __launch_bounds__(256)
-slab_reduce_kernel(const float* __restrict__ slabs, int n_slabs, size_t stride, int64_t n4, float* __restrict__ dst,
-                   int accumulate) {
+slab_reduce_kernel(SlabSum a, SlabSum b) {
+  grid_dep_wait();
   __shared__ float4 part[8][32];
+  const int64_t blocks_a = (a.n4 + 31) / 32;
+  const bool in_b = blockIdx.x >= blocks_a;
+  const float* __restrict__ slabs = in_b ? b.slabs : a.slabs;
+  float* __restrict__ dst = in_b ? b.dst : a.dst;
+  const int n_slabs = in_b ? b.n_slabs : a.n_slabs;
+  const size_t stride = in_b ? b.stride : a.stride;
+  const int64_t n4 = in_b ? b.n4 : a.n4;
+  const int accumulate = in_b ? b.accumulate : a.accumulate;
   const int col = threadIdx.x & 31, grp = threadIdx.x >> 5;
-  const int64_t i = static_cast<int64_t>(blockIdx.x) * 32 + col;
+  const int64_t i = (static_cast<int64_t>(blockIdx.x) - (in_b ? blocks_a : 0)) * 32 + col;
   float4 acc = make_float4(0.f, 0.f, 0.f, 0.f);
   if (i < n4) {
 #pragma unroll 4
@@ -142,12 +152,16 @@
     *o = t;
   }
 }
+int launch_slab_reduce(const SlabSum& a, const SlabSum& b, cudaStream_t s) {
+  const int64_t blocks = (a.n4 + 31) / 32 + (b.n4 + 31) / 32;
+  VDK_CUDA_OK(launch_pdl(slab_reduce_kernel, dim3(static_cast<unsigned>(blocks)), dim3(256), 0, s, a, b));
+  return VDK_OK;
+}
 int launch_slab_reduce(const float* slabs, int n_slabs, size_t stride, int64_t n4, float* dst, int accumulate, cudaStream_t s) {
-  slab_reduce_kernel<<<static_cast<unsigned>((n4 + 31) / 32), 256, 0, s>>>(slabs, n_slabs, stride, n4, dst, accumulate);
-  VDK_CUDA_OK(cudaGetLastError());
-  return VDK_OK;
+  return launch_slab_reduce(SlabSum{slabs, n_slabs, stride, n4, dst, accumulate}, SlabSum{}, s);
 }
 __global__ void col_sum_f32_small_kernel(const float* __restrict__ x, int rows, int cols, float* __restrict__ out) {
+  grid_dep_wait();
   const int c = blockIdx.x * blockDim.x + threadIdx.x;
   if (c >= cols) return;
   float s = 0.f;
@@ -155,11 +169,12 @@
   out[c] += s;
 }
 int launch_col_sum_f32_small(const float* x, int rows, int cols, float* out, cudaStream_t s) {
-  col_sum_f32_small_kernel<<<(cols + 255) / 256, 256, 0, s>>>(x, rows, cols, out);
+  VDK_CUDA_OK(launch_pdl(col_sum_f32_small_kernel, dim3((cols + 255) / 256), dim3(256), 0, s, x, rows, cols, out));
   VDK_CUDA_OK(cudaGetLastError());
   return VDK_OK;
 }
 __global__ void stem_patchify_train_kernel(const float* __restrict__ x, int B, int H, int W, __nv_bfloat16* __restrict__ out) {
+  grid_dep_wait();
   const int PH = H / 4, PW = W / 4;
   const int64_t total = static_cast<int64_t>(B) * PH * PW * 12;
   for (int64_t t = static_cast<int64_t>(blockIdx.x) * blockDim.x + threadIdx.x; t < total;
@@ -200,6 +215,7 @@
 
 __global__ void __launch_bounds__(256)
 pack_cast_kernel(PackTab t, int64_t n, int cols) {
+  grid_dep_wait();
   const float* __restrict__ src = t.src[blockIdx.y];
   __nv_bfloat16* __restrict__ dst = reinterpret_cast<__nv_bfloat16*>(t.dst[blockIdx.y]);
   __nv_bfloat16* __restrict__ dst2 = reinterpret_cast<__nv_bfloat16*>(t.dst2[blockIdx.y]);
@@ -224,6 +240,7 @@
 }
 __global__ void __launch_bounds__(256)
 pack_taps_kernel(PackTab t, int C) {
+  grid_dep_wait();
   const float* __restrict__ src = t.src[blockIdx.y];
   float* __restrict__ dst = reinterpret_cast<float*>(t.dst[blockIdx.y]);
   float* __restrict__ dst2 = reinterpret_cast<float*>(t.dst2[blockIdx.y]);
@@ -237,6 +254,7 @@
 
 __global__ void __launch_bounds__(256)
 unpack_taps_grad_kernel(PackTab t, int C) {
+  grid_dep_wait();
   const float* __restrict__ src = t.src[blockIdx.y];
   float* __restrict__ dst = reinterpret_cast<float*>(t.dst[blockIdx.y]);
   const int i = blockIdx.x * blockDim.x + threadIdx.x;
@@ -269,10 +287,11 @@
       const int64_t n = static_cast<int64_t>(4) * C * C;
       const unsigned gx = static_cast<unsigned>(std::max<int64_t>(1, std::min<int64_t>((n / 4 + 255) / 256, 256)));
       if (taps_and_weights) {
-        pack_cast_kernel<<<dim3(gx, nb), 256, 0, s>>>(fc1, n, 4 * C);
-        pack_cast_kernel<<<dim3(gx, nb), 256, 0, s>>>(fc2, n, 4 * C);
+        VDK_CUDA_OK(launch_pdl(pack_cast_kernel, dim3(gx, nb), dim3(256), 0, s, fc1, n, 4 * C));
+        VDK_CUDA_OK(launch_pdl(pack_cast_kernel, dim3(gx, nb), dim3(256), 0, s, fc2, n, 4 * C));
       }
-      if (taps_and_weights || any_flip) pack_taps_kernel<<<dim3((49 * C + 255) / 256, nb), 256, 0, s>>>(taps, C);
+      if (taps_and_weights || any_flip) VDK_CUDA_OK(launch_pdl(pack_taps_kernel, dim3((49 * C + 255) / 256, nb), dim3(256), 0,
+                                                               s, taps, C));
     }
     k0 += depth;
   }
@@ -315,8 +334,8 @@
   {
     const int M0 = static_cast<int>(L.st[0].M), C0 = L.st[0].C;
     const int64_t total = static_cast<int64_t>(M0) * 12;
-    stem_patchify_train_kernel<<<static_cast<int>(std::min<int64_t>((total + 255) / 256, 132 * 16)), 256, 0, s>>>(images, batch, S, S,
-                                                                                                             B16(L.p0));
+    VDK_CUDA_OK(launch_pdl(stem_patchify_train_kernel, dim3(static_cast<int>(std::min<int64_t>((total + 255) / 256, 132 * 16))),
+                           dim3(256), 0, s, images, batch, S, S, B16(L.p0)));
     VDK_CUDA_OK(cudaGetLastError());
     RC(G.run(B16(L.p0), net->stem_w, B16(L.z0), M0, C0, 48, 48, 48, C0, VDK_EPI_NONE, net->stem_b, nullptr, nullptr, 0,
              VDK_DTYPE_BF16, 1, 0, 0, 0));
@@ -448,7 +467,7 @@
         tab.src[j] = F32(L.dw49) + static_cast<size_t>(k0 + j) * 49 * 2048;
         tab.dst[j] = g->blocks[k0 + j].dw_w;
       }
-      unpack_taps_grad_kernel<<<dim3((49 * C + 255) / 256, nb), 256, 0, s>>>(tab, C);
+      VDK_CUDA_OK(launch_pdl(unpack_taps_grad_kernel, dim3((49 * C + 255) / 256, nb), dim3(256), 0, s, tab, C));
     }
     VDK_CUDA_OK(cudaGetLastError());
     if (st > 0 && !active(u++)) {
diff --git a/visiondk_b200/csrc/gemm.cu b/visiondk_b200/csrc/gemm.cu
--- a/visiondk_b200/csrc/gemm.cu
+++ b/visiondk_b200/csrc/gemm.cu
@@ -431,6 +431,7 @@
   if constexpr (kMode == kGemmLnBwd) {
     if (p.ln_cluster > 1) cluster_sync_all();
   }
+  grid_dep_wait();
 
   if (threadIdx.x < 128) {
     asm volatile("setmaxnreg.dec.sync.aligned.u32 40;");
@@ -840,8 +841,7 @@
   }
   const int num_tiles = ((p.M + kBM - 1) / kBM) * ((p.N + BN - 1) / BN) * p.split_k;
   const int grid = num_tiles < sm_count() ? num_tiles : sm_count();
-  kern<<<grid, kGemmThreads, kSmem, stream>>>(maps[0], maps[1], maps[2], maps[3], maps[4], p);
-  VDK_CUDA_OK(cudaGetLastError());
+  VDK_CUDA_OK(launch_pdl(kern, dim3(grid), dim3(kGemmThreads), kSmem, stream, maps[0], maps[1], maps[2], maps[3], maps[4], p));
   return VDK_OK;
 }
 
@@ -865,11 +865,12 @@
   cfg.blockDim = dim3(kGemmThreads);
   cfg.dynamicSmemBytes = kSmem;
   cfg.stream = s;
-  cudaLaunchAttribute attr[1];
+  cudaLaunchAttribute attr[2];
   attr[0].id = cudaLaunchAttributeClusterDimension;
   attr[0].val.clusterDim.x = cluster;
   attr[0].val.clusterDim.y = 1;
   attr[0].val.clusterDim.z = 1;
+  attr[1] = pdl_attribute();
   cfg.attrs = attr;
   cfg.numAttrs = 1;
   if (fit[cluster] == 0) {
@@ -885,6 +886,7 @@
   const int num_n = p.N / BN, num_tiles = ((p.M + kBM - 1) / kBM) * num_n;
   const int grid = std::min(num_tiles, fit[cluster] - fit[cluster] % num_n);
   cfg.gridDim = dim3(grid);
+  cfg.numAttrs = 2;
   VDK_CUDA_OK(cudaLaunchKernelEx(&cfg, kern, maps[0], maps[1], maps[2], maps[3], maps[4], p));
   *grid_out = grid;
   return VDK_OK;
@@ -931,9 +933,8 @@
     if (rc != VDK_OK) return rc;
   }
   const int n_part = grid / (g.N / BN) * (g.N / G);
-  rc = launch_slab_reduce(g.ln_slab, n_part, static_cast<size_t>(2) * G, G / 4, g.ln_dgamma, 1, s);
-  if (rc != VDK_OK) return rc;
-  return launch_slab_reduce(g.ln_slab + G, n_part, static_cast<size_t>(2) * G, G / 4, g.ln_dbeta, 1, s);
+  return launch_slab_reduce(SlabSum{g.ln_slab, n_part, static_cast<size_t>(2) * G, G / 4, g.ln_dgamma, 1},
+                            SlabSum{g.ln_slab + G, n_part, static_cast<size_t>(2) * G, G / 4, g.ln_dbeta, 1}, s);
 }
 
 int gemm_run(const vdk_gemm_desc& g, cudaStream_t s) {
diff --git a/visiondk_b200/csrc/train_gemm.h b/visiondk_b200/csrc/train_gemm.h
--- a/visiondk_b200/csrc/train_gemm.h
+++ b/visiondk_b200/csrc/train_gemm.h
@@ -6,6 +6,15 @@
 namespace vdk {
 
 int launch_slab_reduce(const float* slabs, int n_slabs, size_t stride, int64_t n4, float* dst, int accumulate, cudaStream_t s);
+struct SlabSum {
+  const float* slabs;
+  int n_slabs;
+  size_t stride;
+  int64_t n4;
+  float* dst;
+  int accumulate;
+};
+int launch_slab_reduce(const SlabSum& a, const SlabSum& b, cudaStream_t s);
 int launch_slab_reduce_bias(const float* slabs, int n_slabs, size_t stride, const float* bias, int rows, int cols, float* out,
                             cudaStream_t s);
 int launch_col_sum_f32_small(const float* x, int rows, int cols, float* out, cudaStream_t s);
@@ -53,9 +62,9 @@
     int rc = run(A, B, slabs, M, N, K, lda, ldb, N, VDK_EPI_NONE, nullptr, nullptr, nullptr, 0, VDK_DTYPE_FP32, std::max(2, split),
                  static_cast<long long>(stride), 1, 1, nullptr, col_slabs);
     if (rc != VDK_OK) return rc;
-    rc = launch_slab_reduce(slabs, split, stride, static_cast<int64_t>(stride / 4), D, accumulate ? 1 : 0, s);
-    if (rc != VDK_OK || !bias_grad) return rc;
-    return launch_slab_reduce(col_slabs, split, static_cast<size_t>(M), M / 4, bias_grad, 1, s);
+    const SlabSum dw{slabs, split, stride, static_cast<int64_t>(stride / 4), D, accumulate ? 1 : 0};
+    const SlabSum db{col_slabs, split, static_cast<size_t>(M), bias_grad ? M / 4 : 0, bias_grad, 1};
+    return launch_slab_reduce(dw, db, s);
   }
 };
 
diff --git a/visiondk_b200/csrc/train_ops.cu b/visiondk_b200/csrc/train_ops.cu
--- a/visiondk_b200/csrc/train_ops.cu
+++ b/visiondk_b200/csrc/train_ops.cu
@@ -33,6 +33,7 @@
               int B, int H, int W, int C, const float* __restrict__ ln_w, const float* __restrict__ ln_b, int patch,
               __nv_bfloat16* __restrict__ dx, const __nv_bfloat16* __restrict__ addend, float* __restrict__ dgamma,
               float* __restrict__ dbeta) {
+  grid_dep_wait();
   constexpr int kPPW = 32 / LPP;
   extern __shared__ float ln_sm[];
   const int Cp = LPP * IT * 8;
@@ -197,15 +198,16 @@
 }
 
 template <int LPP, int IT, int U>
-static void ln_bwd_launch(const __nv_bfloat16* dy, const __nv_bfloat16* y, const float* rstd, int B, int H, int W, int C,
-                          const float* ln_w, const float* ln_b, int patch, __nv_bfloat16* dx, const __nv_bfloat16* addend,
-                          float* dgamma, float* dbeta, cudaStream_t s) {
+static cudaError_t ln_bwd_launch(const __nv_bfloat16* dy, const __nv_bfloat16* y, const float* rstd, int B, int H, int W,
+                                 int C, const float* ln_w, const float* ln_b, int patch, __nv_bfloat16* dx,
+                                 const __nv_bfloat16* addend, float* dgamma, float* dbeta, cudaStream_t s) {
   const int64_t npix = static_cast<int64_t>(B) * H * W;
   const int64_t pix_per_block_trip = 8 * (32 / LPP) * U;
   const int blocks = static_cast<int>(std::max<int64_t>(1, std::min<int64_t>((npix + pix_per_block_trip - 1) / pix_per_block_trip,
                                                                               sm_count() * (IT >= 4 ? 1 : 2))));
   const size_t smem = static_cast<size_t>(LPP) * IT * 8 * 5 * sizeof(float);
-  ln_bwd_kernel<LPP, IT, U><<<blocks, 256, smem, s>>>(dy, y, rstd, B, H, W, C, ln_w, ln_b, patch, dx, addend, dgamma, dbeta);
+  return launch_pdl(ln_bwd_kernel<LPP, IT, U>, dim3(blocks), dim3(256), smem, s, dy, y, rstd, B, H, W, C, ln_w, ln_b, patch, dx,
+                    addend, dgamma, dbeta);
 }
 
 int launch_ln_bwd(const __nv_bfloat16* dy, const __nv_bfloat16* y, const float* rstd, int B, int H, int W, int C,
@@ -213,14 +215,15 @@
                   float* dgamma, float* dbeta, cudaStream_t s) {
   VDK_REQUIRE(C % 8 == 0 && C <= 1536, "ln_bwd: C must be a multiple of 8, <= 1536 (got %d)", C);
   const int vecs = C / 8;
-  if (vecs <= 8) ln_bwd_launch<8, 1, 4>(dy, y, rstd, B, H, W, C, ln_w, ln_b, patch, dx, addend, dgamma, dbeta, s);
-  else if (vecs <= 16) ln_bwd_launch<16, 1, 4>(dy, y, rstd, B, H, W, C, ln_w, ln_b, patch, dx, addend, dgamma, dbeta, s);
-  else if (vecs <= 32) ln_bwd_launch<32, 1, 4>(dy, y, rstd, B, H, W, C, ln_w, ln_b, patch, dx, addend, dgamma, dbeta, s);
-  else if (vecs <= 64) ln_bwd_launch<32, 2, 2>(dy, y, rstd, B, H, W, C, ln_w, ln_b, patch, dx, addend, dgamma, dbeta, s);
-  else if (vecs <= 96) ln_bwd_launch<32, 3, 1>(dy, y, rstd, B, H, W, C, ln_w, ln_b, patch, dx, addend, dgamma, dbeta, s);
-  else if (vecs <= 128) ln_bwd_launch<32, 4, 1>(dy, y, rstd, B, H, W, C, ln_w, ln_b, patch, dx, addend, dgamma, dbeta, s);
-  else ln_bwd_launch<32, 6, 1>(dy, y, rstd, B, H, W, C, ln_w, ln_b, patch, dx, addend, dgamma, dbeta, s);
-  VDK_CUDA_OK(cudaGetLastError());
+  cudaError_t e;
+  if (vecs <= 8) e = ln_bwd_launch<8, 1, 4>(dy, y, rstd, B, H, W, C, ln_w, ln_b, patch, dx, addend, dgamma, dbeta, s);
+  else if (vecs <= 16) e = ln_bwd_launch<16, 1, 4>(dy, y, rstd, B, H, W, C, ln_w, ln_b, patch, dx, addend, dgamma, dbeta, s);
+  else if (vecs <= 32) e = ln_bwd_launch<32, 1, 4>(dy, y, rstd, B, H, W, C, ln_w, ln_b, patch, dx, addend, dgamma, dbeta, s);
+  else if (vecs <= 64) e = ln_bwd_launch<32, 2, 2>(dy, y, rstd, B, H, W, C, ln_w, ln_b, patch, dx, addend, dgamma, dbeta, s);
+  else if (vecs <= 96) e = ln_bwd_launch<32, 3, 1>(dy, y, rstd, B, H, W, C, ln_w, ln_b, patch, dx, addend, dgamma, dbeta, s);
+  else if (vecs <= 128) e = ln_bwd_launch<32, 4, 1>(dy, y, rstd, B, H, W, C, ln_w, ln_b, patch, dx, addend, dgamma, dbeta, s);
+  else e = ln_bwd_launch<32, 6, 1>(dy, y, rstd, B, H, W, C, ln_w, ln_b, patch, dx, addend, dgamma, dbeta, s);
+  VDK_CUDA_OK(e);
   return VDK_OK;
 }
 
@@ -232,6 +235,7 @@
 __global__ void __launch_bounds__(224)
 dwconv7_wgrad_kernel(const __grid_constant__ CUtensorMap map_x, const __grid_constant__ CUtensorMap map_g, int B, int H,
                      int W, int C, int T_rt, int ipc, float* __restrict__ dw49, float* __restrict__ dbias) {
+  grid_dep_wait();
   extern __shared__ uint8_t wg_raw[];
   uint8_t* smem = wg_raw + ((128u - (smem_u32(wg_raw) & 127u)) & 127u);
   const int T = TT > 0 ? TT : T_rt;
@@ -371,9 +375,12 @@
   const int ipc = static_cast<int>(std::max<int64_t>(1, std::min<int64_t>(16, (per_image * B) / (sm_count() * 4))));
   const unsigned grid = static_cast<unsigned>(((B + ipc - 1) / ipc) * per_image);
   const int threads = ((16 * planes + 31) / 32) * 32;
-  if (T == 14) dwconv7_wgrad_kernel<14><<<grid, threads, smem, s>>>(mx, mg, B, H, W, C, T, ipc, dw49, dbias);
-  else if (T == 7) dwconv7_wgrad_kernel<7><<<grid, threads, smem, s>>>(mx, mg, B, H, W, C, T, ipc, dw49, dbias);
-  else dwconv7_wgrad_kernel<0><<<grid, threads, smem, s>>>(mx, mg, B, H, W, C, T, ipc, dw49, dbias);
+  if (T == 14) VDK_CUDA_OK(launch_pdl(dwconv7_wgrad_kernel<14>, dim3(grid), dim3(threads), smem, s, mx, mg, B, H, W, C, T, ipc,
+                                      dw49, dbias));
+  else if (T == 7) VDK_CUDA_OK(launch_pdl(dwconv7_wgrad_kernel<7>, dim3(grid), dim3(threads), smem, s, mx, mg, B, H, W, C, T,
+                                          ipc, dw49, dbias));
+  else VDK_CUDA_OK(launch_pdl(dwconv7_wgrad_kernel<0>, dim3(grid), dim3(threads), smem, s, mx, mg, B, H, W, C, T, ipc, dw49,
+                              dbias));
   VDK_CUDA_OK(cudaGetLastError());
   return VDK_OK;
 }
@@ -383,6 +390,7 @@
 bn_train_fwd_kernel(const TIn* __restrict__ x, int R, int C, const float* __restrict__ weight, const float* __restrict__ bias,
                     float eps, float momentum, TOut* __restrict__ y, float* __restrict__ save_mean,
                     float* __restrict__ save_rstd, float* __restrict__ running_mean, float* __restrict__ running_var) {
+  grid_dep_wait();
   __shared__ float red[8][33];
   __shared__ float s_mean[32], s_rstd[32];
   const int lane = threadIdx.x & 31, warp = threadIdx.x >> 5;
@@ -438,6 +446,7 @@
 bn_train_bwd_kernel(const TGrad* __restrict__ dy, const TIn* __restrict__ x, int R, int C, const float* __restrict__ weight,
                     const float* __restrict__ save_mean, const float* __restrict__ save_rstd, TGrad* __restrict__ dx,
                     float* __restrict__ dweight, float* __restrict__ dbias) {
+  grid_dep_wait();
   __shared__ float red[2][8][33];
   __shared__ float s_a[32], s_b[32];
   const int lane = threadIdx.x & 31, warp = threadIdx.x >> 5;
@@ -503,6 +512,7 @@
                         const float* __restrict__ bias, float eps, float momentum, __nv_bfloat16* __restrict__ y,
                         float* __restrict__ save_mean, float* __restrict__ save_rstd, float* __restrict__ running_mean,
                         float* __restrict__ running_var) {
+  grid_dep_wait();
   __shared__ float red[8][8];
   const int c0 = blockIdx.x * 8;
   const float inv_r = 1.0f / static_cast<float>(R);
@@ -557,6 +567,7 @@
                         const float* __restrict__ weight, const float* __restrict__ save_mean,
                         const float* __restrict__ save_rstd, __nv_bfloat16* __restrict__ dx, float* __restrict__ dweight,
                         float* __restrict__ dbias) {
+  grid_dep_wait();
   __shared__ float red[8][8];
   const int c0 = blockIdx.x * 8;
   float mean[8], rs[8], s1[8], s2[8], g[8], v[8];
@@ -603,6 +614,7 @@
 __global__ void __launch_bounds__(256)
 permute021_kernel(const float* __restrict__ in, int A, int Bd, int Cd, const float* __restrict__ row_scale,
                   __nv_bfloat16* __restrict__ out_bf16, float* __restrict__ out_f32, int accumulate) {
+  grid_dep_wait();
   const int64_t total = static_cast<int64_t>(A) * Bd * Cd;
   for (int64_t i = static_cast<int64_t>(blockIdx.x) * blockDim.x + threadIdx.x; i < total;
        i += static_cast<int64_t>(gridDim.x) * blockDim.x) {
@@ -619,6 +631,7 @@
 __global__ void __launch_bounds__(256)
 permute021_tiled_kernel(const float* __restrict__ in, int Bd, int Cd, const float* __restrict__ row_scale,
                         __nv_bfloat16* __restrict__ out_bf16, float* __restrict__ out_f32, int accumulate) {
+  grid_dep_wait();
   __shared__ float tile[32][33];
   const int a = blockIdx.z, b0 = blockIdx.y * 32, c0 = blockIdx.x * 32;
   const int tx = threadIdx.x & 31, ty = threadIdx.x >> 5;
@@ -646,6 +659,7 @@
 layerscale_finalize_kernel(const float* __restrict__ G, const float* __restrict__ W2, const float* __restrict__ b2,
                            const float* __restrict__ gamma, const float* __restrict__ sdo, int C, int K4,
                            float* __restrict__ dW2, float* __restrict__ dgamma, float* __restrict__ db2) {
+  grid_dep_wait();
   __shared__ float red[8];
   const int c = blockIdx.x;
   const float gm = gamma[c];
@@ -668,11 +682,13 @@
 }
 
 __global__ void cast_f32_bf16_kernel(const float* __restrict__ in, int64_t n, __nv_bfloat16* __restrict__ out) {
+  grid_dep_wait();
   for (int64_t i = static_cast<int64_t>(blockIdx.x) * blockDim.x + threadIdx.x; i < n;
        i += static_cast<int64_t>(gridDim.x) * blockDim.x)
     out[i] = __float2bfloat16_rn(in[i]);
 }
 __global__ void add_f32_kernel(float* __restrict__ dst, const float* __restrict__ src, int64_t n) {
+  grid_dep_wait();
   for (int64_t i = static_cast<int64_t>(blockIdx.x) * blockDim.x + threadIdx.x; i < n;
        i += static_cast<int64_t>(gridDim.x) * blockDim.x)
     dst[i] += src[i];
@@ -684,60 +700,64 @@
                       float* out_f32, int accumulate, cudaStream_t s) {
   if (Bd >= 16 && Cd >= 16 && A <= 65535 && (Bd + 31) / 32 <= 65535) {
     const dim3 grid((Cd + 31) / 32, (Bd + 31) / 32, A);
-    permute021_tiled_kernel<<<grid, 256, 0, s>>>(in, Bd, Cd, row_scale, out_bf16, out_f32, accumulate);
+    VDK_CUDA_OK(launch_pdl(permute021_tiled_kernel, dim3(grid), dim3(256), 0, s, in, Bd, Cd, row_scale, out_bf16, out_f32,
+                           accumulate));
   } else {
-    permute021_kernel<<<blocks_for(static_cast<int64_t>(A) * Bd * Cd), 256, 0, s>>>(in, A, Bd, Cd, row_scale, out_bf16, out_f32,
-                                                                                   accumulate);
+    VDK_CUDA_OK(launch_pdl(permute021_kernel, dim3(blocks_for(static_cast<int64_t>(A) * Bd * Cd)), dim3(256), 0, s, in, A, Bd,
+                           Cd, row_scale, out_bf16, out_f32, accumulate));
   }
   VDK_CUDA_OK(cudaGetLastError());
   return VDK_OK;
 }
 int launch_cast_bf16(const float* in, int64_t n, __nv_bfloat16* out, cudaStream_t s) {
-  cast_f32_bf16_kernel<<<blocks_for(n), 256, 0, s>>>(in, n, out);
+  VDK_CUDA_OK(launch_pdl(cast_f32_bf16_kernel, dim3(blocks_for(n)), dim3(256), 0, s, in, n, out));
   VDK_CUDA_OK(cudaGetLastError());
   return VDK_OK;
 }
 int launch_layerscale_finalize(const float* G, const float* W2, const float* b2, const float* gamma, const float* sdo, int C,
                                int K4, float* dW2, float* dgamma, float* db2, cudaStream_t s) {
-  layerscale_finalize_kernel<<<C, 256, 0, s>>>(G, W2, b2, gamma, sdo, C, K4, dW2, dgamma, db2);
+  VDK_CUDA_OK(launch_pdl(layerscale_finalize_kernel, dim3(C), dim3(256), 0, s, G, W2, b2, gamma, sdo, C, K4, dW2, dgamma, db2));
   VDK_CUDA_OK(cudaGetLastError());
   return VDK_OK;
 }
 int launch_bn_fwd_bf16(const __nv_bfloat16* x, int R, int C, const float* w, const float* b, float eps, float momentum,
                        __nv_bfloat16* y, float* save_mean, float* save_rstd, float* run_mean, float* run_var, cudaStream_t s) {
   if (C % 8 == 0)
-    bn_train_fwd_vec_kernel<<<C / 8, 256, 0, s>>>(x, R, C, w, b, eps, momentum, y, save_mean, save_rstd, run_mean, run_var);
+    VDK_CUDA_OK(launch_pdl(bn_train_fwd_vec_kernel, dim3(C / 8), dim3(256), 0, s, x, R, C, w, b, eps, momentum, y, save_mean,
+                           save_rstd, run_mean, run_var));
   else
-    bn_train_fwd_kernel<__nv_bfloat16, __nv_bfloat16><<<(C + 31) / 32, 256, 0, s>>>(x, R, C, w, b, eps, momentum, y, save_mean,
-                                                                                    save_rstd, run_mean, run_var);
+    VDK_CUDA_OK(launch_pdl(bn_train_fwd_kernel<__nv_bfloat16, __nv_bfloat16>, dim3((C + 31) / 32), dim3(256), 0, s, x, R, C, w,
+                           b, eps, momentum, y, save_mean, save_rstd, run_mean, run_var));
   VDK_CUDA_OK(cudaGetLastError());
   return VDK_OK;
 }
 int launch_bn_fwd_f32(const float* x, int R, int C, const float* w, const float* b, float eps, float momentum, float* y,
                       float* save_mean, float* save_rstd, float* run_mean, float* run_var, cudaStream_t s) {
-  bn_train_fwd_kernel<float, float><<<(C + 31) / 32, 256, 0, s>>>(x, R, C, w, b, eps, momentum, y, save_mean, save_rstd, run_mean,
-                                                                  run_var);
+  VDK_CUDA_OK(launch_pdl(bn_train_fwd_kernel<float, float>, dim3((C + 31) / 32), dim3(256), 0, s, x, R, C, w, b, eps, momentum,
+                         y, save_mean, save_rstd, run_mean, run_var));
   VDK_CUDA_OK(cudaGetLastError());
   return VDK_OK;
 }
 int launch_bn_bwd_bf16(const __nv_bfloat16* dy, const __nv_bfloat16* x, int R, int C, const float* w, const float* save_mean,
                        const float* save_rstd, __nv_bfloat16* dx, float* dweight, float* dbias, cudaStream_t s) {
   if (C % 8 == 0)
-    bn_train_bwd_vec_kernel<<<C / 8, 256, 0, s>>>(dy, x, R, C, w, save_mean, save_rstd, dx, dweight, dbias);
+    VDK_CUDA_OK(launch_pdl(bn_train_bwd_vec_kernel, dim3(C / 8), dim3(256), 0, s, dy, x, R, C, w, save_mean, save_rstd, dx,
+                           dweight, dbias));
   else
-    bn_train_bwd_kernel<__nv_bfloat16, __nv_bfloat16><<<(C + 31) / 32, 256, 0, s>>>(dy, x, R, C, w, save_mean, save_rstd, dx,
-                                                                                    dweight, dbias);
+    VDK_CUDA_OK(launch_pdl(bn_train_bwd_kernel<__nv_bfloat16, __nv_bfloat16>, dim3((C + 31) / 32), dim3(256), 0, s, dy, x, R, C,
+                           w, save_mean, save_rstd, dx, dweight, dbias));
   VDK_CUDA_OK(cudaGetLastError());
   return VDK_OK;
 }
 int launch_bn_bwd_f32(const float* dy, const float* x, int R, int C, const float* w, const float* save_mean,
                       const float* save_rstd, float* dx, float* dweight, float* dbias, cudaStream_t s) {
-  bn_train_bwd_kernel<float, float><<<(C + 31) / 32, 256, 0, s>>>(dy, x, R, C, w, save_mean, save_rstd, dx, dweight, dbias);
+  VDK_CUDA_OK(launch_pdl(bn_train_bwd_kernel<float, float>, dim3((C + 31) / 32), dim3(256), 0, s, dy, x, R, C, w, save_mean,
+                         save_rstd, dx, dweight, dbias));
   VDK_CUDA_OK(cudaGetLastError());
   return VDK_OK;
 }
 int launch_add_f32(float* dst, const float* src, int64_t n, cudaStream_t s) {
-  add_f32_kernel<<<blocks_for(n), 256, 0, s>>>(dst, src, n);
+  VDK_CUDA_OK(launch_pdl(add_f32_kernel, dim3(blocks_for(n)), dim3(256), 0, s, dst, src, n));
   VDK_CUDA_OK(cudaGetLastError());
   return VDK_OK;
 }
diff --git a/visiondk_b200/csrc/vdk_host.h b/visiondk_b200/csrc/vdk_host.h
--- a/visiondk_b200/csrc/vdk_host.h
+++ b/visiondk_b200/csrc/vdk_host.h
@@ -40,6 +40,25 @@
 
 int sm_count();
 
+inline cudaLaunchAttribute pdl_attribute() {
+  cudaLaunchAttribute a{};
+  a.id = cudaLaunchAttributeProgrammaticStreamSerialization;
+  a.val.programmaticStreamSerializationAllowed = 1;
+  return a;
+}
+template <typename... KArgs, typename... Args>
+inline cudaError_t launch_pdl(void (*kern)(KArgs...), dim3 grid, dim3 block, size_t smem, cudaStream_t s, Args&&... args) {
+  cudaLaunchConfig_t cfg{};
+  cfg.gridDim = grid;
+  cfg.blockDim = block;
+  cfg.dynamicSmemBytes = smem;
+  cfg.stream = s;
+  cudaLaunchAttribute attr[1] = {pdl_attribute()};
+  cfg.attrs = attr;
+  cfg.numAttrs = 1;
+  return cudaLaunchKernelEx(&cfg, kern, static_cast<Args&&>(args)...);
+}
+
 enum ProfCategory { kProfGemm = 0, kProfDepthwise = 1, kProfAttention = 2, kProfScoreFilter = 3, kProfOther = 4, kProfCategories = 5 };
 struct ProfScope {
   ProfScope(int category, double flops, double bytes, cudaStream_t stream);
diff --git a/visiondk_b200/csrc/vdk_ptx.cuh b/visiondk_b200/csrc/vdk_ptx.cuh
--- a/visiondk_b200/csrc/vdk_ptx.cuh
+++ b/visiondk_b200/csrc/vdk_ptx.cuh
@@ -195,6 +195,8 @@
   asm volatile("barrier.cluster.wait.acquire.aligned;" ::: "memory");
 }
 
+__device__ __forceinline__ void grid_dep_wait() { asm volatile("griddepcontrol.wait;" ::: "memory"); }
+
 __device__ __forceinline__ float2 ffma2(float2 a, float2 b, float2 c) {
   return make_float2(fmaf(a.x, b.x, c.x), fmaf(a.y, b.y, c.y));
 }
```

New measurement: 2484, median of 6. 2.5% higher.
